# ZhengdiYu/Arbitrary-Hands-3D-Reconstruction

Hardware: AMD Instinct MI355X
Metric: frames/sec (2-hand mesh) at 512x512 batch-64; vertex L2 vs ref (higher is better)
Workload: dtype f32; 1 GPU; configs[2]: synthetic 512x512 RGB batch=64 per GPU, HRNet-W32 backbone, fp32; frames_per_gpu=64, global_batch=64, parallelism=frame-sharded x1, gather=none (one rank), contexts_in_turn=2

## Files before the change

arbitrary-hands-3d-reconstruction_amd/_lib.py:

```python
import ctypes as C
import os

HERE = os.path.dirname(os.path.abspath(__file__))
LIB_PATH = os.environ.get('ACRMI_LIB') or os.path.join(HERE, 'libacrmi.so')

OP_U8NORM, OP_CONV, OP_FUSESUM, OP_BILINEAR2X, OP_POW11, OP_ATTPOOL, OP_PAREBIAS, OP_COORDFILL, OP_POINTHEADS, OP_STEM = range(1, 11)
OP_MAXPOOL, OP_PAIR1X1 = 11, 12
MODE_BOTH, MODE_DENSE, MODE_POINT = 0, 1, 2
CONV_BIAS_MAP = 8
CONV_SPLITK = 16
CONV_DUAL = 32
OPT_POINT_HEADS, OPT_LANES, OPT_CENTER_IDX, OPT_TEMPORAL, OPT_CONF_THRESH, OPT_SMOOTH_COEFF, OPT_MANO_FP16 = 1, 2, 3, 4, 5, 6, 7
OPT_LANE_PLAN = 8
OPT_BATCH_PRIOR = 9
OPT_POINT_HEADS_MULTI = 10
VERSION = 303
DT_F32, DT_F16, DT_BF16 = 0, 1, 2
SLOT = 176
MAX_HAND = 8
ASSOC_STATE = 41
SLOT_FLAG, SLOT_FLATIND, SLOT_SCORE, SLOT_CAM, SLOT_POSES, SLOT_BETAS, SLOT_PARAMS = 0, 1, 2, 3, 6, 54, 64
E_INVAL, E_HIP, E_STATE, E_NOMEM, E_RANGE = -1, -2, -3, -4, -5
OVERLAY_SKELETON, OVERLAY_CENTERMAP = 0, 1
SEGM_NONE = 255


class BufferDesc(C.Structure):
    _fields_ = [('h', C.c_int32), ('w', C.c_int32), ('cs', C.c_int32), ('persistent', C.c_int32), ('dtype', C.c_int32)]


class Op(C.Structure):
    _fields_ = [('kind', C.c_int32),
                ('in_buf', C.c_int32), ('out_buf', C.c_int32), ('res_buf', C.c_int32),
                ('in_coff', C.c_int32), ('out_coff', C.c_int32), ('res_coff', C.c_int32),
                ('cin', C.c_int32), ('cout', C.c_int32),
                ('ksize', C.c_int32), ('stride', C.c_int32), ('relu', C.c_int32), ('groups', C.c_int32),
                ('w_off', C.c_int64), ('b_off', C.c_int64),
                ('bias_per_frame', C.c_int32), ('aux_buf', C.c_int32), ('nterms', C.c_int32),
                ('term_buf', C.c_int32 * 4), ('term_coff', C.c_int32 * 4), ('term_shift', C.c_int32 * 4),
                ('w_off2', C.c_int64), ('b_off2', C.c_int64), ('w_off3', C.c_int64),
                ('flags', C.c_int32), ('mode', C.c_int32)]


class Frame(C.Structure):
    _fields_ = [('bgr_dev', C.c_void_p), ('H', C.c_int32), ('W', C.c_int32)]


class NV12Frame(C.Structure):
    _fields_ = [('y_dev', C.c_void_p), ('uv_dev', C.c_void_p), ('H', C.c_int32), ('W', C.c_int32),
                ('y_pitch', C.c_int32), ('uv_pitch', C.c_int32)]


class NV12Surface(C.Structure):
    _fields_ = NV12Frame._fields_


class Roi(C.Structure):
    _fields_ = [('frame', C.c_int32), ('l', C.c_int32), ('t', C.c_int32), ('r', C.c_int32), ('b', C.c_int32)]


NV12_MATRICES = {'cv601': 0, 'bt601': 1, 'bt601-full': 2, 'bt709': 3, 'bt709-full': 4}


class HeadLayout(C.Structure):
    _fields_ = [('center_buf', C.c_int32 * 2), ('params_buf', C.c_int32 * 2), ('prior_buf', C.c_int32 * 2),
                ('segm_buf', C.c_int32), ('backbone_buf', C.c_int32)]


class ConvProblem(C.Structure):
    _fields_ = [('in_', C.c_void_p), ('w_packed', C.c_void_p), ('bias', C.c_void_p), ('res', C.c_void_p), ('out', C.c_void_p)] + \
               [(k, C.c_int32) for k in ('B', 'H', 'W', 'in_cs', 'in_coff', 'cin', 'bias_frame_stride', 'res_cs', 'res_coff', 'out_cs',
                                         'out_coff', 'cout', 'ksize', 'stride', 'relu', 'groups', 'algo', 'reserved')]


EXPORTS = ['acrmi_version', 'acrmi_last_error', 'acrmi_create', 'acrmi_destroy', 'acrmi_load_weights',
           'acrmi_set_program', 'acrmi_load_mano', 'acrmi_backbone_heads', 'acrmi_buffer_ptr', 'acrmi_decode',
           'acrmi_decode_maps', 'acrmi_mano', 'acrmi_forward', 'acrmi_conv2d', 'acrmi_u8norm', 'acrmi_bilinear2x',
           'acrmi_fuse_sum', 'acrmi_attpool', 'acrmi_attpool_ws_floats', 'acrmi_stem_conv', 'acrmi_stream_create', 'acrmi_stream_destroy', 'acrmi_profile_ops', 'acrmi_tune', 'acrmi_preprocess', 'acrmi_cam_trans',
           'acrmi_set_option', 'acrmi_point_heads', 'acrmi_set_option_f', 'acrmi_smooth', 'acrmi_smooth_reset',
           'acrmi_comm_unique_id', 'acrmi_comm_init', 'acrmi_comm_destroy', 'acrmi_allgather', 'acrmi_parebias',
           'acrmi_buffer_dtype', 'acrmi_conv2d_h16', 'acrmi_conv2d_splitk', 'acrmi_conv2d_splitk_workspace',
           'acrmi_decode_gated', 'acrmi_decode_maps_gated', 'acrmi_share_weights', 'acrmi_mano_rotmat', 'acrmi_heads',
           'acrmi_backbone_channels', 'acrmi_check_range', 'acrmi_prior_gate', 'acrmi_preprocess_frames',
           'acrmi_mesh_topology', 'acrmi_render_workspace', 'acrmi_rasterize', 'acrmi_load_faces', 'acrmi_render',
           'acrmi_overlay_tables', 'acrmi_draw_skeletons', 'acrmi_draw_heatmaps', 'acrmi_overlay',
           'acrmi_streams_create', 'acrmi_streams_destroy', 'acrmi_streams_reset', 'acrmi_smooth_streams',
           'acrmi_forward_streams', 'acrmi_nv12_matrix', 'acrmi_preprocess_nv12', 'acrmi_nv12_to_rgb',
           'acrmi_roi_offsets', 'acrmi_preprocess_rois', 'acrmi_preprocess_rois_nv12', 'acrmi_track_box', 'acrmi_track_boxes',
           'acrmi_preprocess_rois_dev', 'acrmi_preprocess_rois_nv12_dev', 'acrmi_nv12_out_matrix', 'acrmi_rgb_to_nv12',
           'acrmi_nv12_compose', 'acrmi_rasterize_views', 'acrmi_draw_region_heatmaps', 'acrmi_render_regions',
           'acrmi_overlay_regions', 'acrmi_decode_multi', 'acrmi_decode_maps_multi', 'acrmi_forward_multi',
           'acrmi_tracks_create', 'acrmi_tracks_destroy', 'acrmi_tracks_reset', 'acrmi_associate', 'acrmi_forward_tracks',
           'acrmi_assoc_step', 'acrmi_point_heads_multi', 'acrmi_contact_workspace', 'acrmi_mesh_contact', 'acrmi_contact',
           'acrmi_conv2d_group', 'acrmi_program_groups', 'acrmi_surface_contact_workspace', 'acrmi_mesh_surface_contact',
           'acrmi_surface_contact', 'acrmi_score_board_bytes', 'acrmi_score_pair_bytes', 'acrmi_pose_errors',
           'acrmi_score_accumulate', 'acrmi_score_hands', 'acrmi_vertex_colors', 'acrmi_contact_values',
           'acrmi_rasterize_colored', 'acrmi_render_colored', 'acrmi_render_regions_colored', 'acrmi_segm_tables',
           'acrmi_segm_labels', 'acrmi_segm_stats_ws_ints', 'acrmi_segm_stats', 'acrmi_segment', 'acrmi_match_board_bytes',
           'acrmi_match_hands', 'acrmi_match_gather', 'acrmi_match_accumulate', 'acrmi_mano_backward']

_lib = None


class AcrmiError(RuntimeError):
    pass


class AcrmiRangeError(AcrmiError, OverflowError):
    """ACRMI_ERANGE: an 'fp16x3' program met an activation outside the f16 range (acrmi_check_range); the results since the
    last check are invalid (and were written as NaN)."""


def lib():
    global _lib
    if _lib is not None:
        return _lib
    if not os.path.exists(LIB_PATH):
        raise AcrmiError('libacrmi.so not built: run `python __graft_entry__.py build` (needs hipcc). '
                         'The ACR path has no CPU fallback.')
    L = C.CDLL(LIB_PATH)
    vp, i32, f32p, u8p = C.c_void_p, C.c_int, C.c_void_p, C.c_void_p
    L.acrmi_version.restype = C.c_int
    if L.acrmi_version() != VERSION:
        raise AcrmiError('%s is ABI version %d, this package binds version %d: rebuild it (`python __graft_entry__.py build`)'
                         % (LIB_PATH, L.acrmi_version(), VERSION))
    L.acrmi_last_error.restype = C.c_char_p
    L.acrmi_last_error.argtypes = [vp]
    L.acrmi_create.argtypes = [C.POINTER(vp), i32]
    L.acrmi_destroy.argtypes = [vp]
    L.acrmi_destroy.restype = None
    L.acrmi_load_weights.argtypes = [vp, vp, C.c_size_t]
    L.acrmi_set_program.argtypes = [vp, C.POINTER(BufferDesc), i32, C.POINTER(Op), i32, C.POINTER(HeadLayout), i32]
    L.acrmi_load_mano.argtypes = [vp, i32, vp, vp, vp, vp, vp, vp]
    L.acrmi_backbone_heads.argtypes = [vp, u8p, i32, vp]
    L.acrmi_buffer_ptr.argtypes = [vp, i32, C.POINTER(i32), C.POINTER(i32), C.POINTER(i32)]
    L.acrmi_buffer_ptr.restype = vp
    L.acrmi_decode.argtypes = [vp, i32, f32p, vp]
    L.acrmi_decode_maps.argtypes = [f32p, f32p, i32, f32p, f32p, i32, f32p, f32p, i32, i32, C.c_float, f32p, vp]
    L.acrmi_decode_gated.argtypes = [vp, i32, vp, f32p, vp]
    L.acrmi_share_weights.argtypes = [vp, vp]
    L.acrmi_decode_maps_gated.argtypes = [f32p, f32p, i32, f32p, f32p, i32, f32p, f32p, i32, i32, C.c_float, vp, f32p, vp]
    L.acrmi_mano.argtypes = [vp, f32p, i32, f32p, i32, vp, i32, i32, f32p, f32p, f32p, f32p, i32, f32p, f32p, f32p,
                             f32p, vp]
    L.acrmi_mano_rotmat.argtypes = [vp, f32p, f32p, i32, vp, i32, i32, f32p, f32p, f32p, vp]
    L.acrmi_mano_backward.argtypes = [vp, f32p, i32, f32p, i32, vp, i32, i32, f32p, f32p, f32p, f32p, f32p, vp]
    L.acrmi_heads.argtypes = [vp, f32p, i32, vp]
    L.acrmi_backbone_channels.argtypes = [vp]
    L.acrmi_check_range.argtypes = [vp, vp]
    L.acrmi_prior_gate.argtypes = [vp, f32p, i32, vp, vp]
    L.acrmi_preprocess_frames.argtypes = [C.POINTER(Frame), i32, vp, vp, vp]
    L.acrmi_nv12_matrix.argtypes = [i32, vp]
    L.acrmi_preprocess_nv12.argtypes = [C.POINTER(NV12Frame), i32, vp, vp, vp, vp]
    L.acrmi_nv12_to_rgb.argtypes = [C.POINTER(NV12Frame), i32, vp, i32, C.POINTER(vp), vp]
    L.acrmi_nv12_out_matrix.argtypes = [i32, vp]
    L.acrmi_rgb_to_nv12.argtypes = [C.POINTER(vp), C.POINTER(NV12Surface), i32, vp, i32, vp]
    L.acrmi_nv12_compose.argtypes = [C.POINTER(NV12Frame), C.POINTER(vp), C.POINTER(NV12Surface), i32, vp, vp, i32, vp]
    L.acrmi_roi_offsets.argtypes = [i32, i32, C.POINTER(Roi), vp, vp]
    L.acrmi_preprocess_rois.argtypes = [C.POINTER(Frame), i32, C.POINTER(Roi), i32, vp, vp, vp]
    L.acrmi_preprocess_rois_nv12.argtypes = [C.POINTER(NV12Frame), i32, C.POINTER(Roi), i32, vp, vp, vp, vp]
    L.acrmi_track_box.argtypes = [f32p, i32, i32, i32, C.c_double, i32, vp]
    L.acrmi_track_boxes.argtypes = [f32p, f32p, vp, i32, C.c_double, i32, vp, vp]
    L.acrmi_preprocess_rois_dev.argtypes = [C.POINTER(Frame), i32, vp, vp, i32, vp, vp, vp, vp]
    L.acrmi_preprocess_rois_nv12_dev.argtypes = [C.POINTER(NV12Frame), i32, vp, vp, i32, vp, vp, vp, vp, vp]
    L.acrmi_forward.argtypes = [vp, u8p, i32, f32p, f32p, f32p, f32p, f32p, f32p, f32p, vp]
    L.acrmi_conv2d.argtypes = [f32p, i32, i32, i32, i32, i32, i32, f32p, f32p, i32, f32p, i32, i32, f32p, i32, i32,
                               i32, i32, i32, i32, i32, i32, vp]
    L.acrmi_conv2d_h16.argtypes = [vp, i32, i32, i32, i32, i32, i32, vp, f32p, i32, vp, i32, i32, vp, i32, i32,
                                   i32, i32, i32, i32, i32, i32, i32, vp]
    L.acrmi_conv2d_splitk.argtypes = [f32p, i32, i32, i32, i32, i32, i32, i32, f32p, f32p, f32p, i32, i32, f32p, i32, i32,
                                      i32, i32, vp, C.c_size_t, vp]
    L.acrmi_conv2d_splitk_workspace.argtypes = [i32, i32, i32, i32, i32]
    L.acrmi_conv2d_splitk_workspace.restype = C.c_size_t
    L.acrmi_buffer_dtype.argtypes = [vp, i32]
    L.acrmi_u8norm.argtypes = [u8p, i32, f32p, vp]
    L.acrmi_bilinear2x.argtypes = [f32p, i32, i32, i32, i32, i32, f32p, i32, vp]
    L.acrmi_fuse_sum.argtypes = [i32, C.POINTER(vp), C.POINTER(i32), C.POINTER(i32), i32, i32, i32, i32, f32p, i32,
                                 i32, vp]
    L.acrmi_attpool.argtypes = [f32p, i32, f32p, i32, i32, i32, f32p, f32p, vp]
    L.acrmi_attpool_ws_floats.argtypes = [i32, i32]
    L.acrmi_stream_create.argtypes = [i32, C.POINTER(C.c_void_p)]
    L.acrmi_stream_destroy.argtypes = [vp]
    L.acrmi_stem_conv.argtypes = [vp, i32, i32, i32, f32p, f32p, f32p, i32, i32, i32, vp]
    L.acrmi_attpool_ws_floats.restype = C.c_size_t
    L.acrmi_profile_ops.argtypes = [vp, u8p, i32, vp, i32, vp]
    L.acrmi_tune.argtypes = [i32, i32]
    L.acrmi_conv2d_group.argtypes = [C.POINTER(ConvProblem), i32, vp]
    L.acrmi_program_groups.argtypes = [vp, i32]
    L.acrmi_preprocess.argtypes = [u8p, i32, i32, i32, u8p, vp, vp]
    L.acrmi_cam_trans.argtypes = [f32p, f32p, i32, C.c_float, C.c_float, f32p, vp]
    L.acrmi_set_option.argtypes = [vp, i32, i32]
    L.acrmi_point_heads.argtypes = [vp, i32, vp]
    L.acrmi_point_heads_multi.argtypes = [vp, i32, i32, vp]
    L.acrmi_set_option_f.argtypes = [vp, i32, C.c_float]
    L.acrmi_smooth.argtypes = [vp, f32p, i32, vp]
    L.acrmi_smooth_reset.argtypes = [vp, vp]
    L.acrmi_streams_create.argtypes = [C.POINTER(vp), i32, i32]
    L.acrmi_streams_destroy.argtypes = [vp]
    L.acrmi_streams_destroy.restype = None
    L.acrmi_streams_reset.argtypes = [vp, vp, i32, vp]
    L.acrmi_smooth_streams.argtypes = [vp, vp, f32p, i32, vp, vp]
    L.acrmi_forward_streams.argtypes = [vp, vp, vp, u8p, i32, f32p, f32p, f32p, f32p, f32p, f32p, f32p, vp]
    L.acrmi_comm_unique_id.argtypes = [vp]
    L.acrmi_comm_init.argtypes = [vp, i32, i32, vp]
    L.acrmi_comm_destroy.argtypes = [vp]
    L.acrmi_allgather.argtypes = [vp, vp, f32p, f32p, C.c_size_t, vp]
    L.acrmi_parebias.argtypes = [f32p, i32, i32, f32p, f32p, f32p, f32p, f32p, i32, f32p, i32, vp]
    L.acrmi_mesh_topology.argtypes = [vp, i32, i32, vp, i32]
    L.acrmi_render_workspace.argtypes = [i32, i32]
    L.acrmi_render_workspace.restype = C.c_size_t
    L.acrmi_rasterize.argtypes = [f32p, f32p, i32, i32, i32, vp, vp, vp, vp, f32p, f32p, C.c_float, C.c_float, u8p, u8p, i32,
                                  i32, i32, vp, vp, vp]
    L.acrmi_load_faces.argtypes = [vp, i32, vp, i32]
    L.acrmi_render.argtypes = [vp, f32p, f32p, f32p, i32, f32p, vp, C.c_float, C.c_float, u8p, u8p, i32, i32, vp, vp]
    L.acrmi_overlay_tables.argtypes = [i32, u8p, u8p]
    L.acrmi_draw_skeletons.argtypes = [f32p, vp, i32, u8p, i32, i32, i32, u8p, u8p, i32, i32, i32, vp]
    L.acrmi_draw_heatmaps.argtypes = [f32p, f32p, C.c_longlong, i32, i32, i32, f32p, C.c_float, u8p, i32, u8p, u8p, u8p, i32,
                                      i32, vp]
    L.acrmi_overlay.argtypes = [vp, i32, f32p, f32p, i32, f32p, i32, u8p, u8p, u8p, i32, i32, vp]
    L.acrmi_rasterize_views.argtypes = list(L.acrmi_rasterize.argtypes)
    L.acrmi_draw_region_heatmaps.argtypes = [f32p, f32p, C.c_longlong, i32, i32, i32, f32p, vp, C.c_float, u8p, i32, u8p, u8p,
                                             u8p, i32, i32, i32, vp]
    L.acrmi_render_regions.argtypes = [vp, f32p, f32p, f32p, i32, f32p, vp, vp, C.c_float, C.c_float, u8p, u8p, i32, i32, i32,
                                       vp, vp]
    L.acrmi_overlay_regions.argtypes = [vp, i32, f32p, f32p, i32, f32p, vp, i32, u8p, u8p, u8p, i32, i32, i32, vp]
    L.acrmi_decode_multi.argtypes = [vp, i32, i32, f32p, vp]
    L.acrmi_decode_maps_multi.argtypes = [f32p, f32p, i32, f32p, f32p, i32, f32p, f32p, i32, i32, i32, C.c_float, f32p, vp]
    L.acrmi_forward_multi.argtypes = [vp, u8p, i32, i32, f32p, f32p, f32p, f32p, f32p, f32p, f32p, vp]
    L.acrmi_tracks_create.argtypes = [C.POINTER(vp), i32, i32, i32, i32, i32]
    L.acrmi_tracks_destroy.argtypes = [vp]
    L.acrmi_tracks_destroy.restype = None
    L.acrmi_tracks_reset.argtypes = [vp, vp, i32, vp]
    L.acrmi_associate.argtypes = [vp, vp, f32p, i32, i32, vp, i32, vp, vp, vp]
    L.acrmi_forward_tracks.argtypes = [vp, vp, vp, i32, u8p, i32, i32, f32p, f32p, f32p, f32p, f32p, f32p, f32p, vp, vp]
    L.acrmi_assoc_step.argtypes = [i32, i32, i32, vp, i32, vp, vp, vp, vp]
    L.acrmi_contact_workspace.argtypes = [i32, i32]
    L.acrmi_contact_workspace.restype = C.c_size_t
    L.acrmi_mesh_contact.argtypes = [f32p, f32p, i32, i32, i32, vp, vp, vp, vp, vp, i32, C.c_float, C.c_float, vp, f32p, f32p,
                                     f32p, vp, vp, vp]
    L.acrmi_contact.argtypes = [vp, f32p, f32p, f32p, i32, i32, vp, C.c_float, C.c_float, vp, f32p, f32p, f32p, vp, vp]
    L.acrmi_surface_contact_workspace.argtypes = [i32, i32, i32]
    L.acrmi_surface_contact_workspace.restype = C.c_size_t
    L.acrmi_mesh_surface_contact.argtypes = [f32p, f32p, i32, i32, i32, vp, vp, vp, vp, i32, C.c_float, C.c_float, vp, f32p, f32p,
                                             vp, f32p, vp, vp, vp]
    L.acrmi_surface_contact.argtypes = [vp, f32p, f32p, f32p, i32, i32, C.c_float, C.c_float, vp, f32p, f32p, vp, f32p, vp, vp]
    L.acrmi_score_board_bytes.argtypes = [i32, i32, i32]
    L.acrmi_score_board_bytes.restype = C.c_size_t
    L.acrmi_score_pair_bytes.argtypes = [i32]
    L.acrmi_score_pair_bytes.restype = C.c_size_t
    L.acrmi_pose_errors.argtypes = [f32p, f32p, u8p, i32, i32, i32, f32p, f32p, f32p, vp, i32, f32p, f32p, f32p, f32p, vp, f32p, f32p, vp]
    L.acrmi_score_accumulate.argtypes = [f32p, f32p, i32, i32, vp, i32, f32p, f32p, i32, C.c_double, vp, vp, vp]
    L.acrmi_score_hands.argtypes = [vp, f32p, f32p, f32p, f32p, f32p, f32p, u8p, vp, i32, i32, i32, i32, C.c_double, vp,
                                    f32p, f32p, f32p, vp, f32p, f32p, f32p, vp, f32p, vp]
    L.acrmi_vertex_colors.argtypes = [f32p, vp, f32p, i32, i32, C.c_float, C.c_float, i32, f32p, u8p, i32, f32p, vp]
    L.acrmi_contact_values.argtypes = [f32p, f32p, vp, i32, i32, i32, C.c_float, f32p, vp, vp]
    L.acrmi_rasterize_colored.argtypes = [f32p, f32p, i32, i32, i32, vp, vp, vp, vp, f32p, f32p, f32p, i32, C.c_float, C.c_float,
                                          u8p, u8p, i32, i32, i32, vp, vp, vp]
    L.acrmi_render_colored.argtypes = [vp, f32p, f32p, f32p, i32, f32p, vp, f32p, C.c_float, C.c_float, u8p, u8p, i32, i32, vp, vp]
    L.acrmi_render_regions_colored.argtypes = [vp, f32p, f32p, f32p, i32, f32p, vp, vp, f32p, C.c_float, C.c_float, u8p, u8p, i32,
                                               i32, i32, vp, vp]
    L.acrmi_segm_tables.argtypes = [i32, i32, u8p]
    L.acrmi_segm_labels.argtypes = [f32p, C.c_longlong, i32, i32, i32, i32, i32, f32p, f32p, C.c_float, u8p, i32, u8p, u8p, u8p,
                                    i32, i32, vp]
    L.acrmi_segm_stats_ws_ints.argtypes = [i32, i32, i32]
    L.acrmi_segm_stats_ws_ints.restype = C.c_size_t
    L.acrmi_segm_stats.argtypes = [u8p, vp, i32, i32, i32, i32, i32, vp, vp, vp, vp, vp]
    L.acrmi_segment.argtypes = [vp, i32, f32p, C.c_float, u8p, i32, u8p, u8p, u8p, i32, i32, vp]
    L.acrmi_match_board_bytes.argtypes = []
    L.acrmi_match_board_bytes.restype = C.c_size_t
    L.acrmi_match_hands.argtypes = [f32p, f32p, u8p, u8p, f32p, i32, f32p, vp, i32, i32, i32, i32, i32, C.c_float, i32, vp, vp, f32p,
                                    vp, vp, vp]
    L.acrmi_match_gather.argtypes = [f32p, vp, i32, i32, i32, i32, f32p, vp]
    L.acrmi_match_accumulate.argtypes = [vp, f32p, i32, i32, vp, vp]
    for name in EXPORTS:
        fn = getattr(L, name)
        if name not in ('acrmi_last_error', 'acrmi_destroy', 'acrmi_buffer_ptr', 'acrmi_attpool_ws_floats',
                        'acrmi_render_workspace', 'acrmi_streams_destroy', 'acrmi_tracks_destroy', 'acrmi_contact_workspace',
                        'acrmi_surface_contact_workspace', 'acrmi_score_board_bytes', 'acrmi_score_pair_bytes',
                        'acrmi_segm_stats_ws_ints', 'acrmi_match_board_bytes'):
            fn.restype = C.c_int
    _lib = L
    return L


def check(rc, ctx=None):
    if rc >= 0:
        return rc
    msg = lib().acrmi_last_error(ctx)
    msg = msg.decode() if msg else 'acrmi error %d' % rc
    if rc == E_INVAL:
        raise ValueError(msg)
    if rc == E_RANGE:
        raise AcrmiRangeError(msg)
    raise AcrmiError(msg)
```

arbitrary-hands-3d-reconstruction_amd/csrc/acrmi.hip:

```cpp
#include "acrmi_ctx.h"
#include "score_plan.h"
#include "surface_contact_plan.h"
#include "vertex_color_plan.h"

#include <initializer_list>
#include <type_traits>

std::string g_err;

int fail(acrmi_ctx* c, int code, const char* fmt, ...) {
  char buf[512];
  va_list ap;
  va_start(ap, fmt);
  vsnprintf(buf, sizeof buf, fmt, ap);
  va_end(ap);
  if (c) c->err = buf; else g_err = buf;
  return code;
}

void release_weights(acrmi_ctx* c) {
  if (c->weights_ref && c->weights_ref->fetch_sub(1) == 1) {
    (void)hipFree(c->weights);
    delete c->weights_ref;
  }
// ... 395 lines not shown
                             shared, stream);
  if (!r) *out = t;
  return r;
}

int acrmi_streams_create(acrmi_streams** out, int device, int capacity) { return streams_create(out, device, capacity, true, nullptr); }

void acrmi_streams_destroy(acrmi_streams* t) { table_destroy(t); }

int acrmi_streams_reset(acrmi_streams* t, const int32_t* ids, int n, void* stream) {
  return table_reset("acrmi_streams_reset", t, ids, n,
                     [](StateTable* t, const SmoothIds& k, int m, hipStream_t s) { return launch_smooth_reset(k, m, t->init, s); },
                     (hipStream_t)stream);
}

static void smooth_coefficients(SmoothArgs& a, float smooth_coeff) {
  a.mincutoff = smooth_coeff; a.mincutoff_betas = 0.6f; a.beta = 0.7f; a.freq = 30.f;
  const double te = 1.0 / 30.0, tau = 1.0 / (2 * M_PI * 1.0), alpha_d = 1.0 / (1.0 + tau / te);
  a.alpha_d = (float)alpha_d; a.one_minus_alpha_d = (float)(1.0 - alpha_d);
  a.two_pi = (float)(2 * M_PI); a.te = (float)te;
}

static int smooth_on(acrmi_ctx* c, acrmi_streams* t, float* slots, int B, const int32_t* ids, hipStream_t stream) {
  SmoothArgs a{};
  a.state = t->state;
  a.init = t->init;
  smooth_coefficients(a, c->smooth_coeff);
  TableOrder ord(t, stream);
  hipError_t e = ord.err;
  for (int f0 = 0; e == hipSuccess && f0 < B; f0 += SMOOTH_FRAMES_PER_LAUNCH) {
    const int m = B - f0 < SMOOTH_FRAMES_PER_LAUNCH ? B - f0 : SMOOTH_FRAMES_PER_LAUNCH;
    const int n_streams = smooth_plan(ids ? ids + f0 : nullptr, m, &a.b, t->last.data());
    if (!n_streams) continue;
    a.slots = slots + (size_t)f0 * 2 * ACRMI_SLOT;
    e = launch_smooth(a, n_streams, stream);
  }
  e = ord.done(e);
  return e == hipSuccess ? ACRMI_OK : fail(c, ACRMI_EHIP, "smoothing: %s", hipGetErrorString(e));
}

static int check_streams(acrmi_ctx* c, const acrmi_streams* t, const int32_t* ids, int B, const char* who) {
  if (!t || !ids || B <= 0) return fail(c, ACRMI_EINVAL, "%s: bad arguments", who);
  return check_table(c, t, ids, B, who);
}

int acrmi_smooth_streams(acrmi_ctx* c, acrmi_streams* t, float* slots, int B, const int32_t* ids, void* stream) {
  if (!c || !slots) return fail(c, ACRMI_EINVAL, "acrmi_smooth_streams: bad arguments");
  const int r = check_streams(c, t, ids, B, "acrmi_smooth_streams");
  if (r) return r;
  ON_DEVICE(c);
  return smooth_on(c, t, slots, B, ids, (hipStream_t)stream);
}

int acrmi_smooth_reset(acrmi_ctx* c, void* stream) {
  if (!c) return fail(c, ACRMI_EINVAL, "acrmi_smooth_reset: ctx is NULL");
  if (!c->own_streams)
    return from_global(c, streams_create(&c->own_streams, c->device, 1, false, (hipStream_t)stream));
  return from_global(c, acrmi_streams_reset(c->own_streams, nullptr, 0, stream));
}

int acrmi_smooth(acrmi_ctx* c, float* slots, int B, void* stream) {
  if (!c || !slots || B <= 0) return fail(c, ACRMI_EINVAL, "acrmi_smooth: bad arguments");
  ON_DEVICE(c);
  if (!c->own_streams) {
    int r = acrmi_smooth_reset(c, stream);
    if (r) return r;
  }
  return smooth_on(c, c->own_streams, slots, B, nullptr, (hipStream_t)stream);
}

int acrmi_tracks_create(acrmi_tracks** out, int device, int capacity, int max_hand, int gate, int max_miss) {
  if (!out) return fail(nullptr, ACRMI_EINVAL, "acrmi_tracks_create: out is NULL");
  if (!assoc_params_ok(max_hand, gate, max_miss))
    return fail(nullptr, ACRMI_EINVAL, "acrmi_tracks_create: max_hand %d outside 1..%d, gate %d outside 0..%d or max_miss %d < -1",
                max_hand, ASSOC_MAX_HAND, gate, ASSOC_GATE_ANY, max_miss);
  if (capacity < 1 || (long long)capacity * max_hand > ASSOC_MAX_TRACKS)
    return fail(nullptr, ACRMI_EINVAL, "acrmi_tracks_create: capacity %d x max_hand %d outside 1..%d hands per side", capacity,
                max_hand, ASSOC_MAX_TRACKS);
  acrmi_tracks* t = new acrmi_tracks();
  t->max_hand = max_hand; t->gate = gate; t->max_miss = max_miss;
  const size_t hands = (size_t)capacity * max_hand * 2;
  const size_t state_bytes = hands * 3 * 64 * sizeof(float), init_bytes = hands * sizeof(int);
  const int r = table_create("acrmi_tracks_create", t, device, capacity, state_bytes,
                             state_bytes + init_bytes + (size_t)capacity * 2 * sizeof(AssocSide), true, nullptr);
  if (r) return r;
  t->meta = reinterpret_cast<AssocSide*>(reinterpret_cast<char*>(t->init) + init_bytes);
  *out = t;
  return ACRMI_OK;
}

void acrmi_tracks_destroy(acrmi_tracks* t) { table_destroy(t); }

int acrmi_tracks_reset(acrmi_tracks* t, const int32_t* ids, int n, void* stream) {
  return table_reset("acrmi_tracks_reset", t, ids, n,
                     [](StateTable* st, const SmoothIds& k, int m, hipStream_t s) {
                       acrmi_tracks* t = static_cast<acrmi_tracks*>(st);
                       return launch_assoc_reset(k, m, t->max_hand, t->meta, t->init, s);
                     },
                     (hipStream_t)stream);
}

static int check_tracks(acrmi_ctx* c, const acrmi_tracks* t, const int32_t* ids, int B, int max_hand, const char* who) {
  if (!t || !ids || B <= 0) return fail(c, ACRMI_EINVAL, "%s: bad arguments", who);
  if (max_hand < 1 || max_hand > ACRMI_MAX_HAND) return fail(c, ACRMI_EINVAL, "%s: max_hand %d outside 1..%d", who, max_hand, ACRMI_MAX_HAND);
  if (max_hand != t->max_hand) return fail(c, ACRMI_EINVAL, "%s: max_hand %d, the table holds %d slots per side", who, max_hand, t->max_hand);
  return check_table(c, t, ids, B, who);
}

static int associate_on(acrmi_ctx* c, acrmi_tracks* t, float* slots, int B, const int32_t* ids, int smooth, int32_t* track_ids,
                        int32_t* perm, hipStream_t stream) {
  AssocArgs a{};
  a.s.state = t->state;
  a.s.init = t->init;
  smooth_coefficients(a.s, c ? c->smooth_coeff : 4.0f );
  a.meta = t->meta;
  a.K = t->max_hand; a.gate = t->gate; a.max_miss = t->max_miss; a.smooth = smooth ? 1 : 0;
  const size_t frame_rows = (size_t)2 * t->max_hand;
  TableOrder ord(t, stream);
  hipError_t e = ord.err;
  for (int f0 = 0; e == hipSuccess && f0 < B; f0 += SMOOTH_FRAMES_PER_LAUNCH) {
    const int m = B - f0 < SMOOTH_FRAMES_PER_LAUNCH ? B - f0 : SMOOTH_FRAMES_PER_LAUNCH;
    const int n_streams = smooth_plan(ids + f0, m, &a.s.b, t->last.data());
    bool any_loose = false;
    memset(a.loose, 0, sizeof a.loose);
    for (int i = 0; i < m; ++i)
      if (ids[f0 + i] < 0) { a.loose[i >> 5] |= 1u << (i & 31); any_loose = true; }
    a.m = m;
    a.s.slots = slots + (size_t)f0 * frame_rows * ACRMI_SLOT;
    a.track_ids = track_ids + (size_t)f0 * frame_rows;
    a.perm = perm ? perm + (size_t)f0 * frame_rows : nullptr;
    e = launch_associate(a, n_streams, any_loose, stream);
  }
  e = ord.done(e);
  return e == hipSuccess ? ACRMI_OK : fail(c, ACRMI_EHIP, "association: %s", hipGetErrorString(e));
}

int acrmi_associate(acrmi_ctx* c, acrmi_tracks* t, float* slots, int B, int max_hand, const int32_t* ids, int smooth,
                    int32_t* track_ids, int32_t* perm, void* stream) {
  if (!slots || !track_ids) return fail(c, ACRMI_EINVAL, "acrmi_associate: bad arguments");
  const int r = check_tracks(c, t, ids, B, max_hand, "acrmi_associate");
  if (r) return r;
  DeviceGuard guard_(t->device);
  if (guard_.err != hipSuccess) return fail(c, ACRMI_EHIP, "hipSetDevice(%d): %s", t->device, hipGetErrorString(guard_.err));
  return associate_on(c, t, slots, B, ids, smooth, track_ids, perm, (hipStream_t)stream);
}

int acrmi_program_groups(acrmi_ctx* c, int B) {
  if (!c) return fail(c, ACRMI_EINVAL, "acrmi_program_groups: bad arguments");
  if (!c->have_program) return fail(c, ACRMI_ESTATE, "no program");
  if (B <= 0 || B > c->max_batch) return fail(c, ACRMI_EINVAL, "batch %d outside 1..%d", B, c->max_batch);
  return c->sched[c->point_heads ? 1 : 0][B > AUTO_SMALL_BATCH ? 1 : 0].n_groups;
}

int acrmi_profile_ops(acrmi_ctx* c, const uint8_t* img, int B, float* ms_out, int n_ms, void* stream) {
  if (!c || !img || !ms_out) return fail(c, ACRMI_EINVAL, "acrmi_profile_ops: bad arguments");
  if (!c->have_program) return fail(c, ACRMI_ESTATE, "no program");
  const int n = (int)c->ops.size();
  if (n_ms < n) return fail(c, ACRMI_EINVAL, "ms_out too small (%d < %d)", n_ms, n);
  ON_DEVICE(c);
  hipStream_t s = (hipStream_t)stream;
  const bool point = c->point_heads;
  int r = run_program(c, img, B, stream, point);
  if (r) return r;
  std::vector<hipEvent_t> ev(n + 1, nullptr);
  auto cleanup = [&]() {
    for (auto& e : ev)
      if (e) (void)hipEventDestroy(e);
  };
  hipError_t he = hipSuccess;
  for (auto& e : ev)
    if ((he = hipEventCreate(&e)) != hipSuccess) break;
  if (he == hipSuccess) he = hipEventRecord(ev[0], s);
  for (int i = 0; i < n && he == hipSuccess && r == ACRMI_OK; ++i) {
    if (op_active(c->ops[i], point)) r = run_op(c, c->ops[i], img, B, s);
    if (r == ACRMI_OK) he = hipEventRecord(ev[i + 1], s);
  }
  if (he == hipSuccess && r == ACRMI_OK) he = hipStreamSynchronize(s);
  for (int i = 0; i < n && he == hipSuccess && r == ACRMI_OK; ++i) he = hipEventElapsedTime(&ms_out[i], ev[i], ev[i + 1]);
  cleanup();
  if (r) return r;
  if (he != hipSuccess) return fail(c, ACRMI_EHIP, "acrmi_profile_ops: %s", hipGetErrorString(he));
  if (B <= AUTO_SMALL_BATCH) {
    c->op_ms[point ? 1 : 0].assign(ms_out, ms_out + n);
    build_schedule(c, point, false);
  }
  return n;
}

void* acrmi_buffer_ptr(acrmi_ctx* c, int buf, int* h, int* w, int* cs) {
  if (!c || !c->have_program || buf < 0 || buf >= (int)c->bufs.size()) return nullptr;
  if (h) *h = c->bufs[buf].h;
  if (w) *w = c->bufs[buf].w;
  if (cs) *cs = c->bufs[buf].cs;
  return c->buf_ptr[buf];
}

int acrmi_buffer_dtype(acrmi_ctx* c, int buf) {
  if (!c || !c->have_program || buf < 0 || buf >= (int)c->bufs.size()) return -1;
  return c->bufs[buf].dtype;
}

static int decode_ctx(acrmi_ctx* c, const char* who, int B, const int32_t* prior_gate, bool top_k, int max_hand, float* slots,
                      void* stream) {
  if (!c || !slots) return fail(c, ACRMI_EINVAL, "%s: bad arguments", who);
  if (top_k && (max_hand < 1 || max_hand > ACRMI_MAX_HAND))
    return fail(c, ACRMI_EINVAL, "%s: max_hand %d outside 1..%d", who, max_hand, ACRMI_MAX_HAND);
  if (!c->have_program) return fail(c, ACRMI_ESTATE, "%s: no program", who);
  if (B <= 0 || B > c->max_batch) return fail(c, ACRMI_EINVAL, "batch %d outside 1..%d", B, c->max_batch);
  ON_DEVICE(c);
  const acrmi_head_layout& h = c->heads;
  return from_global(c, decode_maps_impl(c->buf_ptr[h.center_buf[0]], c->buf_ptr[h.center_buf[1]], c->bufs[h.center_buf[0]].cs,
                                         c->buf_ptr[h.params_buf[0]], c->buf_ptr[h.params_buf[1]], c->bufs[h.params_buf[0]].cs,
                                         c->buf_ptr[h.prior_buf[0]], c->buf_ptr[h.prior_buf[1]], c->bufs[h.prior_buf[0]].cs, B,
                                         c->conf_thresh, prior_gate, c->range_flag, slots, stream, top_k ? max_hand : 0));
}

int acrmi_decode(acrmi_ctx* c, int B, float* slots, void* stream) { return acrmi_decode_gated(c, B, nullptr, slots, stream); }

int acrmi_decode_gated(acrmi_ctx* c, int B, const int32_t* prior_gate, float* slots, void* stream) {
  return decode_ctx(c, "acrmi_decode", B, prior_gate, false, 0, slots, stream);
}

int acrmi_decode_multi(acrmi_ctx* c, int B, int max_hand, float* slots, void* stream) {
  return decode_ctx(c, "acrmi_decode_multi", B, nullptr, true, max_hand, slots, stream);
}

int acrmi_prior_gate(acrmi_ctx* c, const float* slots, int B, int32_t* gate, void* stream) {
  if (!slots || !gate || B <= 0) return fail(c, ACRMI_EINVAL, "acrmi_prior_gate: bad arguments");
  if (c) {
    ON_DEVICE(c);
    return from_global(c, acrmi_prior_gate(nullptr, slots, B, gate, stream));
  }
  HIPCHK(c, launch_prior_gate(slots, B, gate, (hipStream_t)stream));
  return ACRMI_OK;
}

int acrmi_check_range(acrmi_ctx* c, void* stream) {
  if (!c) return fail(c, ACRMI_EINVAL, "acrmi_check_range: ctx is NULL");
  if (!c->range_flag) return ACRMI_OK;
  ON_DEVICE(c);
  unsigned v = 0;
  HIPCHK(c, hipStreamSynchronize((hipStream_t)stream));
  HIPCHK(c, hipMemcpy(&v, c->range_flag, sizeof(v), hipMemcpyDeviceToHost));
  if (!v) return ACRMI_OK;
  HIPCHK(c, hipMemsetAsync(c->range_flag, 0, sizeof(v), (hipStream_t)stream));
  HIPCHK(c, hipStreamSynchronize((hipStream_t)stream));
  return fail(c, ACRMI_ERANGE, "an activation of the 'fp16x3' program left the f16 range (|x| > 65504): its split halves are "
                               "inf / -inf and the results since the last check are invalid (slots and meshes were written as "
                               "NaN); use precision 'bf16x3' or 'fp32' for this checkpoint");
}

static int mano_rows(acrmi_ctx* c, const char* who, ManoArgs& m, const float* betas, int beta_stride, const int32_t* side, int H,
                     int center_idx, float* verts, float* joints, float* center, void* stream) {
  if (!c) return fail(c, ACRMI_EINVAL, "%s: ctx is NULL", who);
  if (H == 0) return ACRMI_OK;
  if (H < 0 || !m.poses || !betas || !verts || !joints || center_idx >= 21) return fail(c, ACRMI_EINVAL, "%s: bad arguments", who);
  if (!c->have_mano[0] && !c->have_mano[1]) return fail(c, ACRMI_ESTATE, "%s: MANO tables not loaded", who);
  ON_DEVICE(c);
  m.t[0] = c->have_mano[0] ? c->mano[0] : c->mano[1];
  m.t[1] = c->have_mano[1] ? c->mano[1] : c->mano[0];
  m.betas = betas; m.beta_stride = beta_stride;
  m.side = side; m.H = H; m.center_idx = center_idx;
  m.verts = verts; m.joints = joints; m.center = center;
  m.off_div = 1;
  m.lbs_f16 = c->mano_f16;
  HIPCHK(c, launch_mano(m, (hipStream_t)stream));
  return ACRMI_OK;
}

int acrmi_mano(acrmi_ctx* c, const float* poses, int pose_stride, const float* betas, int beta_stride,
               const int32_t* side, int H, int center_idx, float* verts, float* joints, float* center,
               const float* cam, int cam_stride, const float* offsets, float* verts_camed, float* pj2d,
               float* pj2d_org, void* stream) {
  ManoArgs m{};
  m.poses = poses; m.pose_stride = pose_stride;
  m.cam = cam; m.cam_stride = cam_stride; m.offsets = offsets;
  m.verts_camed = verts_camed; m.pj2d = pj2d; m.pj2d_org = pj2d_org;
  return mano_rows(c, "acrmi_mano", m, betas, beta_stride, side, H, center_idx, verts, joints, center, stream);
}

int acrmi_mano_rotmat(acrmi_ctx* c, const float* rotmats, const float* betas, int beta_stride, const int32_t* side, int H,
                      int center_idx, float* verts, float* joints, float* center, void* stream) {
  ManoArgs m{};
  m.poses = rotmats; m.pose_stride = 144; m.pose_rotmat = 1;
  return mano_rows(c, "acrmi_mano_rotmat", m, betas, beta_stride, side, H, center_idx, verts, joints, center, stream);
}

int acrmi_mano_backward(acrmi_ctx* c, const float* poses, int pose_stride, const float* betas, int beta_stride,
                        const int32_t* side, int H, int center_idx, const float* g_verts, const float* g_joints,
                        const float* g_center, float* g_poses, float* g_betas, void* stream) {
  if (!c) return fail(c, ACRMI_EINVAL, "acrmi_mano_backward: ctx is NULL");
  if (H < 0 || center_idx < -1 || center_idx > 20 || pose_stride < 48 || beta_stride < 10)
    return fail(c, ACRMI_EINVAL, "acrmi_mano_backward: bad arguments (H >= 0, center_idx -1..20, pose_stride >= 48, beta_stride >= 10)");
  if (H == 0) return ACRMI_OK;
  if (!poses || !betas || !g_poses || !g_betas) return fail(c, ACRMI_EINVAL, "acrmi_mano_backward: NULL poses, betas or outputs");
  if (!c->have_mano[0] && !c->have_mano[1]) return fail(c, ACRMI_ESTATE, "acrmi_mano_backward: MANO tables not loaded");
  ON_DEVICE(c);
  if (!g_verts && !g_joints && !g_center) {
    HIPCHK(c, hipMemsetAsync(g_poses, 0, (size_t)H * 48 * sizeof(float), (hipStream_t)stream));
    HIPCHK(c, hipMemsetAsync(g_betas, 0, (size_t)H * 10 * sizeof(float), (hipStream_t)stream));
    return ACRMI_OK;
  }
  ManoGradArgs m{};
  m.t[0] = c->have_mano[0] ? c->mano[0] : c->mano[1];
  m.t[1] = c->have_mano[1] ? c->mano[1] : c->mano[0];
  m.poses = poses; m.pose_stride = pose_stride;
// ... 318 lines not shown
  if (what == ACRMI_OVERLAY_SKELETON ? (!slots || !kps) : (!out2 || out2 == out || out2 == img_in))
    return fail(c, ACRMI_EINVAL, "%s: bad arguments", who);
  if (!c->have_program || c->last_batch <= 0) return fail(c, ACRMI_ESTATE, "%s: no program has run", who);
  return ACRMI_OK;
}

static hipError_t skeleton_launch(const float* kps, const float* slots, const int32_t* hand_frame, int normalized, int n_hands,
                                  int n_frames, int H, int W, int bgr, const uint8_t* img_in, uint8_t* out, hipStream_t stream) {
  SkeletonArgs a{};
  a.kps = kps; a.hand_frame = hand_frame; a.normalized = normalized;
  if (slots) { a.slots = slots; a.slot_stride = ACRMI_SLOT; a.flag_at = ACRMI_SLOT_FLAG; }
  a.n_hands = n_hands; a.n_frames = n_frames; a.H = H; a.W = W; a.line_width = 3; a.circle_rad = 3;
  a.img_in = img_in; a.img_out = out;
  skeleton_default_colors(bgr != 0, a.colors);
  return launch_skeleton(a, stream);
}

static int heatmap_fill(acrmi_ctx* c, const char* who, HeatmapBase& a, int n, const float* offsets, int bgr, const uint8_t* img_in,
                        uint8_t* out, uint8_t* out2, int H, int W) {
  if (n != c->last_batch)
    return fail(c, ACRMI_ESTATE, "%s: the resident centre maps are those of a batch of %d, not %d", who, c->last_batch, n);
  const acrmi_head_layout& hl = c->heads;
  const acrmi_buffer_desc& d = c->bufs[hl.center_buf[0]];
  a.maps[0] = c->buf_ptr[hl.center_buf[0]]; a.maps[1] = c->buf_ptr[hl.center_buf[1]];
  a.pix_stride = d.cs; a.frame_stride = (long long)d.h * d.w * d.cs; a.dtype = d.dtype;
  a.n = n; a.h = d.h; a.w = d.w; a.H = H; a.W = W; a.offsets = offsets; a.weight = 0.7f;
  a.img_in = img_in; a.out[0] = out; a.out[1] = out2;
  heatmap_default_lut(bgr != 0, a.lut);
  return ACRMI_OK;
}

int acrmi_overlay(acrmi_ctx* c, int what, const float* slots, const float* pj2d, int B, const float* offsets, int bgr,
                  const uint8_t* img_in, uint8_t* out, uint8_t* out2, int H, int W, void* stream) {
  if (int r = check_overlay(c, "acrmi_overlay", what, slots, pj2d, B, img_in, out, out2, B, H, W)) return r;
  ON_DEVICE(c);
  hipError_t e;
  if (what == ACRMI_OVERLAY_SKELETON) {
    e = skeleton_launch(pj2d, slots, nullptr, offsets ? 0 : 1, 2 * B, B, H, W, bgr, img_in, out, (hipStream_t)stream);
  } else {
    HeatmapArgs a{};
    if (int r = heatmap_fill(c, "acrmi_overlay", a, B, offsets, bgr, img_in, out, out2, H, W)) return r;
    e = launch_heatmap(a, (hipStream_t)stream);
  }
  return e == hipSuccess ? ACRMI_OK : fail(c, ACRMI_EHIP, "overlay: %s", hipGetErrorString(e));
}

int acrmi_segment(acrmi_ctx* c, int B, const float* offsets, float weight, const uint8_t* colors_host, int bgr,
                  const uint8_t* img_in, uint8_t* out, uint8_t* labels, int H, int W, void* stream) {
  const char* who = "acrmi_segment";
  if (!c) return fail(c, ACRMI_EINVAL, "%s: ctx is NULL", who);
  if (B <= 0) return fail(c, ACRMI_EINVAL, "%s: B = %d", who, B);
  if (!c->have_program || c->last_batch <= 0) return fail(c, ACRMI_ESTATE, "%s: no program has run", who);
  if (B != c->last_batch)
    return fail(c, ACRMI_ESTATE, "%s: the resident segmentation is that of a batch of %d, not %d", who, c->last_batch, B);
  const int id = c->heads.segm_buf;
  const acrmi_buffer_desc& d = c->bufs[id];
  if (d.dtype != ACRMI_DT_F32) return fail(c, ACRMI_ESTATE, "%s: the segmentation buffer is not fp32", who);
  ON_DEVICE(c);
  return segm_labels_call(c, who, (const float*)c->buf_ptr[id], (long long)d.h * d.w * d.cs, d.cs, B, d.h, d.w, 33, nullptr, offsets,
                          weight, colors_host, bgr, img_in, out, labels, H, W, stream);
}

static int render_regions_call(acrmi_ctx* c, const char* who, bool colored, const float* vcol, const float* verts,
                               const float* cam_trans, const float* slots, int n, const float* offsets, const int32_t* region_frame,
                               const float* colors_host, float focal, float visible_weight, const uint8_t* img_in, uint8_t* img_out,
                               int n_frames, int H, int W, int32_t* ids_out, void* stream) {
  if ((colored && (!vcol || n <= 0 || !vertex_color_sizes_ok(2ll * n, 778))) || !c || !verts || !cam_trans || !slots || !offsets || !region_frame || !img_in || !img_out || n <= 0 || n_frames <= 0 ||
      n_frames > OVERLAY_MAX_FRAMES || H <= 0 || W <= 0 || H > OVERLAY_MAX_DIM || W > OVERLAY_MAX_DIM || !(focal > 0.f) ||
      !(visible_weight >= 0.f && visible_weight <= 1.f) || n > 0x3fffffff || (c->n_faces[0] > 0 && 2ll * n * c->n_faces[0] > 0x7fffffffll))
    return fail(c, ACRMI_EINVAL, "%s: bad arguments", who);
  if (!c->faces_topo[0] || !c->faces_topo[1]) return fail(c, ACRMI_ESTATE, "%s: MANO faces not loaded (acrmi_load_faces)", who);
  ON_DEVICE(c);
  RenderScratch sc;
  if (int r = render_scratch(c, n, &sc)) return r;
  hipError_t e = launch_render_region_prep(slots, offsets, region_frame, n, n_frames, H, W, ACRMI_SLOT, ACRMI_SLOT_FLAG,
                                           colors_host ? colors_host : kHandColors, sc.mesh_frame, sc.mesh_topo, sc.rgb, sc.view,
                                           (hipStream_t)stream);
  if (e != hipSuccess) return fail(c, ACRMI_EHIP, "render region prep: %s", hipGetErrorString(e));
  e = render_launch(c, sc, verts, cam_trans, nullptr, sc.view, focal, visible_weight, img_in, img_out, ids_out, 2 * n, n_frames, H, W,
                    (hipStream_t)stream, vcol);
  return e == hipSuccess ? ACRMI_OK : fail(c, ACRMI_EHIP, "render regions: %s", hipGetErrorString(e));
}

int acrmi_render_regions(acrmi_ctx* c, const float* verts, const float* cam_trans, const float* slots, int n, const float* offsets,
                         const int32_t* region_frame, const float* colors_host, float focal, float visible_weight,
                         const uint8_t* img_in, uint8_t* img_out, int n_frames, int H, int W, int32_t* ids_out, void* stream) {
  return render_regions_call(c, "acrmi_render_regions", false, nullptr, verts, cam_trans, slots, n, offsets, region_frame, colors_host,
                             focal, visible_weight, img_in, img_out, n_frames, H, W, ids_out, stream);
}

int acrmi_render_regions_colored(acrmi_ctx* c, const float* verts, const float* cam_trans, const float* slots, int n,
                                 const float* offsets, const int32_t* region_frame, const float* colors_host, const float* vcol,
                                 float focal, float visible_weight, const uint8_t* img_in, uint8_t* img_out, int n_frames, int H,
                                 int W, int32_t* ids_out, void* stream) {
  return render_regions_call(c, "acrmi_render_regions_colored", true, vcol, verts, cam_trans, slots, n, offsets, region_frame,
                             colors_host, focal, visible_weight, img_in, img_out, n_frames, H, W, ids_out, stream);
}

int acrmi_overlay_regions(acrmi_ctx* c, int what, const float* slots, const float* pj2d_org, int n, const float* offsets,
                          const int32_t* region_frame, int bgr, const uint8_t* img_in, uint8_t* out, uint8_t* out2, int n_frames,
                          int H, int W, void* stream) {
  if (!offsets || !region_frame || n > 0x3fffffff) return fail(c, ACRMI_EINVAL, "acrmi_overlay_regions: bad arguments");
  if (int r = check_overlay(c, "acrmi_overlay_regions", what, slots, pj2d_org, n, img_in, out, out2, n_frames, H, W)) return r;
  ON_DEVICE(c);
  hipError_t e;
  if (what == ACRMI_OVERLAY_SKELETON) {
    if (n > c->region_hand_cap) {
      if (c->region_hand_frame) {
        HIPCHK(c, hipDeviceSynchronize());
        (void)hipFree(c->region_hand_frame);
        c->region_hand_frame = nullptr;
        c->region_hand_cap = 0;
      }
      HIPCHK(c, hipMalloc(&c->region_hand_frame, sizeof(int32_t) * 2 * (size_t)n));
      c->region_hand_cap = n;
    }
    e = launch_render_region_prep(slots, offsets, region_frame, n, n_frames, H, W, ACRMI_SLOT, ACRMI_SLOT_FLAG, nullptr,
                                  c->region_hand_frame, nullptr, nullptr, nullptr, (hipStream_t)stream);
    if (e != hipSuccess) return fail(c, ACRMI_EHIP, "overlay region prep: %s", hipGetErrorString(e));
    e = skeleton_launch(pj2d_org, nullptr, c->region_hand_frame, 0, 2 * n, n_frames, H, W, bgr, img_in, out, (hipStream_t)stream);
  } else {
    RegionHeatmapArgs a{};
    if (int r = heatmap_fill(c, "acrmi_overlay_regions", a, n, offsets, bgr, img_in, out, out2, H, W)) return r;
    a.n_frames = n_frames; a.region_frame = region_frame;
    e = launch_region_heatmap(a, (hipStream_t)stream);
  }
  return e == hipSuccess ? ACRMI_OK : fail(c, ACRMI_EHIP, "overlay regions: %s", hipGetErrorString(e));
}

int acrmi_stream_create(int device, void** stream) {
  if (!stream) return fail(nullptr, ACRMI_EINVAL, "acrmi_stream_create: null argument");
  int prev = 0;
  if (hipGetDevice(&prev) != hipSuccess || hipSetDevice(device) != hipSuccess)
    return fail(nullptr, ACRMI_EHIP, "acrmi_stream_create: cannot select device %d", device);
  hipStream_t st = nullptr;
  const hipError_t e = hipStreamCreateWithFlags(&st, hipStreamNonBlocking);
  (void)hipSetDevice(prev);
  if (e != hipSuccess) return fail(nullptr, ACRMI_EHIP, "hipStreamCreate: %s", hipGetErrorString(e));
  *stream = st;
  return ACRMI_OK;
}

int acrmi_stream_destroy(void* stream) {
  if (!stream) return ACRMI_OK;
  const hipError_t e = hipStreamDestroy((hipStream_t)stream);
  return e == hipSuccess ? ACRMI_OK : fail(nullptr, ACRMI_EHIP, "hipStreamDestroy: %s", hipGetErrorString(e));
}

int acrmi_tune(int key, int value) {
  if (key == 0) { conv_force_cfg(value); return ACRMI_OK; }
  if (key == 3) { conv_set_phase_delay(value); return ACRMI_OK; }
  if (key == 4) { conv_set_xcd_swizzle(value); return ACRMI_OK; }
  if (key == 5) { program_set_grouping(value != 0); return ACRMI_OK; }
  static long long* dbg = nullptr;
  if (key == 1) {
    if (value && !dbg) { if (hipMalloc(&dbg, 128 * sizeof(long long)) != hipSuccess) return ACRMI_EHIP; }
    if (dbg) (void)hipMemset(dbg, 0, 128 * sizeof(long long));
    conv_set_debug(value ? dbg : nullptr);
    return ACRMI_OK;
  }
  if (key == 2) {
    if (!dbg) return ACRMI_OK;
    long long h[128];
    if (hipDeviceSynchronize() != hipSuccess) return ACRMI_EHIP;
    if (hipMemcpy(h, dbg, sizeof h, hipMemcpyDeviceToHost) != hipSuccess) return ACRMI_EHIP;
    const int n = (int)h[63];
    printf("conv stamps (%d):", n);
    for (int i = 1; i < n && i < 60; ++i) printf(" %lld", h[i] - h[i - 1]);
    printf("\n");
    const int nl = (int)h[127];
    if (nl > 0) {
      printf("loader stamps (%d):", nl);
      for (int i = 1; i < nl && i < 60; ++i) printf(" %lld", h[64 + i] - h[64 + i - 1]);
      printf("\n");
    }
    return ACRMI_OK;
  }
  return fail(nullptr, ACRMI_EINVAL, "acrmi_tune: unknown key %d", key);
}

}
```

arbitrary-hands-3d-reconstruction_amd/csrc/acrmi_ctx.h:

```cpp
#pragma once
#include "../../include/acrmi.h"
#include "kernels.h"

#include <dlfcn.h>

#include <atomic>
#include <cmath>
#include <cstdarg>
#include <cstdio>
#include <algorithm>
#include <cstdlib>
#include <cstring>
#include <mutex>
#include <optional>
#include <string>
#include <vector>

using namespace acrmi;

constexpr int MAX_LANES = 8;
constexpr int AUTO_LANES_SMALL = 4, AUTO_LANES_LARGE = 2, AUTO_SMALL_BATCH = 32;
struct Schedule {
  std::vector<int> order;
  std::vector<std::vector<int>> deps;
  std::vector<char> leaf;
  int n_lanes = 0;
  std::vector<int> lane;
  std::vector<std::vector<int>> wait;
  std::vector<char> signal;
  std::vector<int> leader;
  int n_groups = 0;
};
struct StateTable {
  int device = 0;
  int capacity = 0;
  float* state = nullptr;
  int* init = nullptr;
  size_t reset_bytes = 0;
  hipEvent_t order = nullptr;
  std::mutex mu;
  std::vector<int32_t> last;
  virtual ~StateTable() = default;
};

struct acrmi_streams : StateTable {};

struct acrmi_tracks : StateTable {
  int max_hand = 0, gate = 0, max_miss = 0;
  AssocSide* meta = nullptr;
};

struct acrmi_ctx {
  int device = 0;
  std::string err;
  float* weights = nullptr;
  size_t n_weights = 0;
  std::atomic<int>* weights_ref = nullptr;
  std::vector<acrmi_buffer_desc> bufs;
  std::vector<float*> buf_ptr;
  std::vector<acrmi_op> ops;
  acrmi_head_layout heads{};
  bool have_program = false;
  int max_batch = 0;
  bool grouping = false;
  float* att_ws = nullptr;
  size_t att_ws_floats = 0;
  int* picks = nullptr;
  int* gate_buf = nullptr;
  bool batch_prior = false;
  unsigned* range_flag = nullptr;
  bool point_heads = false;
  bool point_heads_multi = false;
  Schedule sched[2][2];
  int want_lanes = 0;
  bool lane_plan = false;
  std::vector<float> op_ms[2];
  hipStream_t lanes[MAX_LANES] = {};
  hipEvent_t fork_ev = nullptr, join_ev[MAX_LANES] = {};
  std::vector<hipEvent_t> op_ev;
  float* split_ws[MAX_LANES] = {};
  unsigned* split_cnt[MAX_LANES] = {};
  size_t split_ws_floats = 0, split_counters = 0;
  ManoTables mano[2]{};
  bool have_mano[2] = {false, false};
  float* mano_allocs[2][11] = {};
  bool mano_f16 = false;
  float conf_thresh = 0.35f;
  int center_idx = 9;
  bool temporal = false;
  float smooth_coeff = 4.0f;
  acrmi_streams* own_streams = nullptr;
  int32_t* faces_topo[2] = {nullptr, nullptr};
  int n_faces[2] = {0, 0};
  char* render_ws = nullptr;
  int render_ws_frames = 0;
  int32_t* region_hand_frame = nullptr;
  int region_hand_cap = 0;
  std::vector<float> v_template_host[2];
  std::vector<int32_t> faces_host[2];
  int contact_sign[2] = {1, 1};
  struct ContactScratch {
    char* ws = nullptr;
    long long hands = 0;
    int faces = 0;
  };
  ContactScratch contact_ws, surface_ws;
  int last_batch = 0;
  void* comm = nullptr;
  int comm_ranks = 0;
};

struct DeviceGuard {
  int prev = -1;
  bool switched = false;
  hipError_t err = hipSuccess;
  explicit DeviceGuard(int dev) {
    err = hipGetDevice(&prev);
    if (err == hipSuccess && prev != dev) {
      err = hipSetDevice(dev);
      switched = err == hipSuccess;
    }
  }
  ~DeviceGuard() {
    if (switched) (void)hipSetDevice(prev);
  }
};

extern std::string g_err;
int fail(acrmi_ctx* c, int code, const char* fmt, ...);
#define ON_DEVICE(c)                                                                                   \
  DeviceGuard guard_((c)->device);                                                                     \
  if (guard_.err != hipSuccess) return fail(c, ACRMI_EHIP, "hipSetDevice(%d): %s", (c)->device, hipGetErrorString(guard_.err))
#define HIPCHK(c, expr)                                                                      \
  do {                                                                                       \
    hipError_t e_ = (expr);                                                                  \
    if (e_ != hipSuccess) return fail(c, ACRMI_EHIP, "%s: %s", #expr, hipGetErrorString(e_)); \
  } while (0)


void free_program(acrmi_ctx* c);
void release_weights(acrmi_ctx* c);
void comm_destroy(acrmi_ctx* c);
PointArgs point_args(const acrmi_ctx* c, const acrmi_op& op, int B);
int run_op(acrmi_ctx* c, const acrmi_op& op, const uint8_t* img, int B, hipStream_t s, int lane = 0, int point_hands = 1);
bool op_active(const acrmi_op& op, bool point);
void build_schedule(acrmi_ctx* c, bool point, bool large);
void program_set_grouping(bool on);
int run_program(acrmi_ctx* c, const uint8_t* img, int B, void* stream, bool point, int first_op = 0, int point_hands = 1);
int decode_maps_impl(const float* l_center, const float* r_center, int center_cs, const float* l_params, const float* r_params,
                     int params_cs, const float* l_prior, const float* r_prior, int prior_cs, int B, float conf_thresh,
                     const int32_t* prior_gate, const unsigned* poison, float* slots, void* stream,
                     int max_hand = 0 );
int segm_labels_call(acrmi_ctx* c, const char* who, const float* logits, long long frame_stride, int pix_stride, int n, int h, int w,
                     int C, const float* view, const float* offsets, float weight, const uint8_t* colors_host, int bgr,
                     const uint8_t* img_in, uint8_t* out, uint8_t* labels, int H, int W, void* stream);
```

arbitrary-hands-3d-reconstruction_amd/csrc/acrmi_program.hip:

```cpp
#include "acrmi_ctx.h"
#include "conv_frame.h"
#include "group_plan.h"

void free_program(acrmi_ctx* c) {
  for (hipEvent_t e : c->op_ev)
    if (e) (void)hipEventDestroy(e);
  c->op_ev.clear();
  for (float* p : c->buf_ptr)
    if (p) (void)hipFree(p);
  c->buf_ptr.clear();
  c->bufs.clear();
  c->ops.clear();
  for (int l = 0; l < MAX_LANES; ++l) {
    if (c->split_ws[l]) (void)hipFree(c->split_ws[l]);
    if (c->split_cnt[l]) (void)hipFree(c->split_cnt[l]);
    c->split_ws[l] = nullptr; c->split_cnt[l] = nullptr;
  }
  c->split_ws_floats = c->split_counters = 0;
  if (c->att_ws) (void)hipFree(c->att_ws);
  c->att_ws = nullptr;
  if (c->picks) (void)hipFree(c->picks);
  c->picks = nullptr;
  if (c->gate_buf) (void)hipFree(c->gate_buf);
  c->gate_buf = nullptr;
  if (c->range_flag) (void)hipFree(c->range_flag);
  c->range_flag = nullptr;
  c->have_program = false;
  c->last_batch = 0;
}

static ConvArgs conv_geometry(const acrmi_op& op, const acrmi_buffer_desc* bufs, int B) {
  const auto& di = bufs[op.in_buf];
  const auto& dout = bufs[op.out_buf];
  ConvArgs a{};
  a.B = B; a.H = di.h; a.W = di.w;
  a.in_cs = di.cs; a.in_coff = op.in_coff; a.Cin = op.cin;
  a.out_cs = dout.cs; a.out_coff = op.out_coff; a.Cout = op.cout;
  a.res_cs = op.res_buf >= 0 ? bufs[op.res_buf].cs : 0; a.res_coff = op.res_coff;
  a.splitk = (op.flags & ACRMI_CONV_SPLITK) != 0;
  if (op.flags & ACRMI_CONV_BIAS_MAP) {
    a.res_cs = (op.groups * op.cout + 3) / 4 * 4; a.res_coff = 0; a.res_bcast = 1;
  }
  a.ks = op.ksize; a.stride = op.stride; a.relu = op.relu; a.groups = op.groups;
  a.bias_fstride = op.bias_per_frame ? bufs[op.aux_buf].cs : 0;
  a.nxt = op.nterms;
  for (int t = 0; t < op.nterms && t < 3; ++t) {
    a.xt_cs[t] = bufs[op.term_buf[t]].cs; a.xt_coff[t] = op.term_coff[t]; a.xt_shift[t] = op.term_shift[t];
  }
  if (op.flags & ACRMI_CONV_DUAL) a.out2_cs = bufs[op.aux_buf].cs;
  a.algo = op.flags & 7;
  a.dtype = di.dtype;
  a.out_f32 = di.dtype != ACRMI_DT_F32 && dout.dtype == ACRMI_DT_F32;
  conv_derive(a);
  return a;
}

PointArgs point_args(const acrmi_ctx* c, const acrmi_op& op, int B) {
  auto ptr = [&](int id) -> float* { return c->buf_ptr[id]; };
  auto desc = [&](int id) -> const acrmi_buffer_desc& { return c->bufs[id]; };
  const acrmi_head_layout& h = c->heads;
  const int side = op.flags & 1;
  PointArgs p{};
  p.x34 = ptr(op.in_buf); p.x_cs = desc(op.in_buf).cs;
  p.center[0] = ptr(h.center_buf[0]); p.center[1] = ptr(h.center_buf[1]); p.center_cs = desc(h.center_buf[0]).cs;
  p.w = c->weights + op.w_off;
  p.mix_w = c->weights + op.w_off2;
  p.bias = ptr(op.aux_buf); p.bias_stride = desc(op.aux_buf).cs;
  p.p109 = ptr(op.res_buf); p.p109_cs = desc(op.res_buf).cs;
  p.prior = ptr(h.prior_buf[side]); p.prior_cs = desc(h.prior_buf[side]).cs;
  p.final_ = ptr(op.out_buf); p.final_cs = desc(op.out_buf).cs;
  p.picks = c->picks; p.side = side; p.B = B; p.thresh = c->conf_thresh;
  p.prior_when_both = c->batch_prior ? 1 : 0;
  return p;
}

static ConvArgs conv_args(const acrmi_ctx* c, const acrmi_op& op, int B, int lane) {
  auto ptr = [&](int id) -> float* { return id >= 0 ? c->buf_ptr[id] : nullptr; };
  ConvArgs a = conv_geometry(op, c->bufs.data(), B);
  a.in = ptr(op.in_buf);
  a.w = c->weights + op.w_off;
  a.bias = op.bias_per_frame ? ptr(op.aux_buf) : c->weights + op.b_off;
  a.res = a.res_bcast ? c->weights + op.w_off2 : ptr(op.res_buf);
  a.out = ptr(op.out_buf);
  if (a.splitk) {
    a.split_ws = c->split_ws[lane]; a.split_cnt = c->split_cnt[lane];
  }
  for (int t = 0; t < op.nterms && t < 3; ++t) a.xt[t] = ptr(op.term_buf[t]);
  if (op.flags & ACRMI_CONV_DUAL) a.out2 = ptr(op.aux_buf);
  a.range_flag = a.algo == 6 ? c->range_flag : nullptr;
  return a;
}

static bool g_grouping = [] {
  const char* e = getenv("ACRMI_GROUP");
  return !(e && atoi(e) == 0);
}();
void program_set_grouping(bool on) { g_grouping = on; }

int run_op(acrmi_ctx* c, const acrmi_op& op, const uint8_t* img, int B, hipStream_t s, int lane, int point_hands) {
  auto ptr = [&](int id) -> float* { return id >= 0 ? c->buf_ptr[id] : nullptr; };
  auto desc = [&](int id) -> const acrmi_buffer_desc& { return c->bufs[id]; };
  auto eptr = [&](int id, int coff) -> float* {
    if (id < 0) return nullptr;
    return reinterpret_cast<float*>(reinterpret_cast<char*>(c->buf_ptr[id]) + (size_t)coff * (c->bufs[id].dtype ? 2 : 4));
  };
  switch (op.kind) {
    case ACRMI_OP_U8NORM: {
      const auto& d = desc(op.out_buf);
      HIPCHK(c, launch_u8norm(img, (long)B * d.h * d.w, ptr(op.out_buf), s));
      return ACRMI_OK;
    }
    case ACRMI_OP_STEM: {
      const auto& d = desc(op.out_buf);
      if (op.ksize == 7) {
        if (d.dtype)
          HIPCHK(c, launch_stem7_h16(img, B, 2 * d.h, 2 * d.w, c->weights + op.w_off, c->weights + op.b_off, ptr(op.out_buf),
                                     d.cs, op.out_coff, op.relu, d.dtype, s));
        else
          HIPCHK(c, launch_stem7(img, B, 2 * d.h, 2 * d.w, c->weights + op.w_off, c->weights + op.b_off, ptr(op.out_buf), d.cs,
                                 op.out_coff, op.relu, s));
        return ACRMI_OK;
      }
      if (d.dtype)
        HIPCHK(c, launch_stem_h16(img, B, 2 * d.h, 2 * d.w, c->weights + op.w_off, c->weights + op.b_off, ptr(op.out_buf),
                                  d.cs, op.out_coff, op.relu, d.dtype, s));
      else
        HIPCHK(c, launch_stem(img, B, 2 * d.h, 2 * d.w, c->weights + op.w_off, c->weights + op.b_off, ptr(op.out_buf), d.cs,
                              op.out_coff, op.relu, s));
      return ACRMI_OK;
    }
    case ACRMI_OP_CONV: {
      HIPCHK(c, launch_conv(conv_args(c, op, B, lane), s));
      return ACRMI_OK;
    }
    case ACRMI_OP_FUSESUM: {
      const auto& dout = desc(op.out_buf);
      FuseArgs f{};
      f.nterms = op.nterms; f.B = B; f.H = dout.h; f.W = dout.w; f.C = op.cout; f.out_cs = dout.cs; f.relu = op.relu;
      f.out = eptr(op.out_buf, op.out_coff);
      for (int t = 0; t < op.nterms; ++t) {
        f.term[t] = eptr(op.term_buf[t], op.term_coff[t]);
        f.cs[t] = desc(op.term_buf[t]).cs;
        f.shift[t] = op.term_shift[t];
      }
      if (dout.dtype) HIPCHK(c, launch_fuse_sum_h16(f, dout.dtype, s));
      else HIPCHK(c, launch_fuse_sum(f, s));
      return ACRMI_OK;
    }
    case ACRMI_OP_BILINEAR2X: {
      const auto& di = desc(op.in_buf);
      if (di.dtype)
        HIPCHK(c, launch_bilinear2x_h16(ptr(op.in_buf), B, di.h, di.w, di.cs, op.in_coff, op.cin, ptr(op.out_buf),
                                        desc(op.out_buf).cs, op.out_coff, di.dtype, s));
      else
        HIPCHK(c, launch_bilinear2x(ptr(op.in_buf), B, di.h, di.w, di.cs, op.in_coff, op.cin, ptr(op.out_buf),
                                    desc(op.out_buf).cs, op.out_coff, s));
      return ACRMI_OK;
    }
    case ACRMI_OP_PAIR1X1: {
      const auto& di = desc(op.in_buf);
      HIPCHK(c, launch_pair1x1(ptr(op.in_buf), di.cs, op.in_coff, ptr(op.res_buf), desc(op.res_buf).cs, op.res_coff, ptr(op.out_buf),
                               desc(op.out_buf).cs, op.out_coff, ptr(op.aux_buf), desc(op.aux_buf).cs, 0, c->weights + op.w_off,
                               (long)B * di.h * di.w, s));
      return ACRMI_OK;
    }
    case ACRMI_OP_MAXPOOL: {
      const auto& di = desc(op.in_buf);
      if (di.dtype)
        HIPCHK(c, launch_maxpool3s2_h16(ptr(op.in_buf), B, di.h, di.w, di.cs, op.in_coff, op.cin, ptr(op.out_buf),
                                        desc(op.out_buf).cs, op.out_coff, di.dtype, s));
      else
        HIPCHK(c, launch_maxpool3s2(ptr(op.in_buf), B, di.h, di.w, di.cs, op.in_coff, op.cin, ptr(op.out_buf),
                                    desc(op.out_buf).cs, op.out_coff, s));
      return ACRMI_OK;
    }
    case ACRMI_OP_POW11: {
      const auto& d = desc(op.out_buf);
      if (d.dtype) HIPCHK(c, launch_pow11_h16(ptr(op.out_buf), (long)B * d.h * d.w, d.cs, op.out_coff, d.dtype, s));
      else HIPCHK(c, launch_pow11(ptr(op.out_buf), (long)B * d.h * d.w, d.cs, op.out_coff, s));
      return ACRMI_OK;
    }
    case ACRMI_OP_ATTPOOL: {
      const auto& ds = desc(op.in_buf);
      const auto& df = desc(op.res_buf);
      HIPCHK(c, launch_attpool(ptr(op.in_buf), ds.cs, eptr(op.res_buf, op.res_coff), df.cs, op.cin, B, df.h, df.w,
                               c->att_ws, ptr(op.out_buf), s, df.dtype));
      return ACRMI_OK;
    }
    case ACRMI_OP_PAREBIAS: {
      PareArgs p{};
      p.pooled = ptr(op.in_buf);
      p.lc_w = c->weights + op.w_off;
      p.lin_w = c->weights + op.w_off2;
      p.lin_b = c->weights + op.b_off2;
      p.mix_wp = c->weights + op.w_off3;
      p.mix_b = c->weights + op.b_off;
      p.out = ptr(op.out_buf);
      p.B = B; p.C = op.cin; p.part0 = op.flags; p.out_stride = desc(op.out_buf).cs;
      HIPCHK(c, launch_parebias(p, s));
      return ACRMI_OK;
    }
    case ACRMI_OP_COORDFILL: {
      const auto& d = desc(op.out_buf);
      if (d.dtype) HIPCHK(c, launch_coordfill_h16(ptr(op.out_buf), c->max_batch, d.h, d.w, d.cs, op.out_coff, d.dtype, s));
      else HIPCHK(c, launch_coordfill(ptr(op.out_buf), c->max_batch, d.h, d.w, d.cs, op.out_coff, s));
      return ACRMI_OK;
    }
    case ACRMI_OP_POINTHEADS: {
      const PointArgs p = point_args(c, op, B);
      if (point_hands > 1) HIPCHK(c, launch_point_heads_multi(p, point_hands, s));
      else HIPCHK(c, launch_point_heads(p, s));
      return ACRMI_OK;
    }
    default:
      return fail(c, ACRMI_EINVAL, "unknown op kind %d", op.kind);
  }
}

bool op_active(const acrmi_op& op, bool point) {
  return op.kind != ACRMI_OP_COORDFILL && op.mode != (point ? ACRMI_MODE_DENSE : ACRMI_MODE_POINT);
}

static void op_rw(const acrmi_ctx* c, const acrmi_op& op, std::vector<int>& R, std::vector<int>& W) {
  R.clear(); W.clear();
  const int n_bufs = (int)c->bufs.size();
  auto r = [&](int id) { if (id >= 0) R.push_back(id); };
  auto w = [&](int id) { if (id >= 0) W.push_back(id); };
  switch (op.kind) {
    case ACRMI_OP_U8NORM: case ACRMI_OP_STEM: w(op.out_buf); break;
    case ACRMI_OP_CONV:
      r(op.in_buf); r(op.res_buf); if (op.bias_per_frame) r(op.aux_buf);
      for (int t = 0; t < op.nterms; ++t) r(op.term_buf[t]);
      w(op.out_buf);
      if (op.flags & ACRMI_CONV_DUAL) w(op.aux_buf);
      break;
    case ACRMI_OP_FUSESUM: for (int t = 0; t < op.nterms; ++t) r(op.term_buf[t]); w(op.out_buf); break;
    case ACRMI_OP_BILINEAR2X: case ACRMI_OP_MAXPOOL: r(op.in_buf); w(op.out_buf); break;
    case ACRMI_OP_PAIR1X1: r(op.in_buf); r(op.res_buf); w(op.out_buf); w(op.aux_buf); break;
    case ACRMI_OP_POW11: r(op.out_buf); w(op.out_buf); break;
    case ACRMI_OP_ATTPOOL: r(op.in_buf); r(op.res_buf); w(op.out_buf); w(n_bufs); break;
    case ACRMI_OP_PAREBIAS: r(op.in_buf); w(op.out_buf); break;
    case ACRMI_OP_POINTHEADS:
      r(op.in_buf); r(op.aux_buf); r(c->heads.center_buf[0]); r(c->heads.center_buf[1]);
      w(op.res_buf); w(op.out_buf); w(c->heads.prior_buf[op.flags & 1]); w(n_bufs + 1);
      break;
    default: break;
  }
}

void build_schedule(acrmi_ctx* c, bool point, bool large) {
  Schedule& S = c->sched[point ? 1 : 0][large ? 1 : 0];
  const int n = (int)c->ops.size(), nb = (int)c->bufs.size() + 2;
  S = Schedule();
  S.deps.assign(n, std::vector<int>());
  S.leaf.assign(n, 1);
  std::vector<std::vector<int>> reads(n), writes(n);
  for (int j = 0; j < n; ++j) {
    if (!op_active(c->ops[j], point)) continue;
    S.order.push_back(j);
    op_rw(c, c->ops[j], reads[j], writes[j]);
  }
  S.deps = hazard_deps(S.order, reads, writes, n, nb);
  for (int j : S.order)
    for (int d : S.deps[j]) S.leaf[d] = 0;
  const int want = c->want_lanes > 0 ? c->want_lanes : (large ? AUTO_LANES_LARGE : AUTO_LANES_SMALL);
  const int max_lanes = std::max(1, std::min(want, MAX_LANES));
  S.lane.assign(n, 0);
  S.wait.assign(n, std::vector<int>());
  S.signal.assign(n, 0);
  std::vector<int> lane_tail(max_lanes, -1);
  const std::vector<float>& ms = c->op_ms[point ? 1 : 0];
  const bool planned = c->lane_plan && !large && max_lanes > 1 && (int)ms.size() == n;
  constexpr float SYNC_MS = 0.002f, EVENT_MS = 0.002f;
  static const float WAIT_MS = experiment_env("ACRMI_PLAN_WAIT_US") ? 1e-3f * (float)atof(experiment_env("ACRMI_PLAN_WAIT_US")) : 0.016f;
  std::vector<float> fin(planned ? n : 0, 0.f), lane_free(max_lanes, 0.f);
  static const bool rank_order = !(experiment_env("ACRMI_PLAN_RANK") && atoi(experiment_env("ACRMI_PLAN_RANK")) == 0);
  if (planned && rank_order) {
    std::vector<float> ru(n, 0.f);
    std::vector<std::vector<int>> succ(n);
    for (int j : S.order)
      for (int d : S.deps[j]) succ[d].push_back(j);
    for (int k = (int)S.order.size() - 1; k >= 0; --k) {
      const int j = S.order[k];
      float m = 0.f;
      for (int s2 : succ[j]) m = std::max(m, ru[s2]);
      ru[j] = m + std::max(ms[j], 1e-4f);
    }
    std::stable_sort(S.order.begin(), S.order.end(), [&](int x, int y) { return ru[x] > ru[y]; });
  }
  S.leader.assign(n, 0);
  for (int j = 0; j < n; ++j) S.leader[j] = j;
  S.n_groups = 0;
  if (c->grouping && c->max_batch >= 16) {
    std::vector<ConvArgs> ca(n);
    std::vector<char> is_conv(n, 0);
    for (int j : S.order)
      if (c->ops[j].kind == ACRMI_OP_CONV) { ca[j] = conv_args(c, c->ops[j], c->max_batch, 0); is_conv[j] = 1; }
    S.leader = plan_groups(S.order, S.deps, n, [&](int x, int y) { return is_conv[x] && is_conv[y] && conv_can_group(ca[x], ca[y]); },
                           CONV_GROUP_MAX);
    for (int j : S.order) S.n_groups += S.leader[j] != j;
  }
  std::vector<int> pos(n, -1);
  for (int k = 0; k < (int)S.order.size(); ++k) pos[S.order[k]] = k;
  for (int j : S.order) {
    int lane = -1;
    if (S.leader[j] != j) {
      lane = S.lane[S.leader[j]];
      if (planned) fin[j] = fin[S.leader[j]] = lane_free[lane] = lane_free[lane] + std::max(ms[j] - EVENT_MS, 0.002f);
    } else if (planned) {
      float best = 0.f;
      bool best_prod = false;
      for (int l = 0; l < max_lanes; ++l) {
        float start = lane_free[l];
        unsigned others = 0;
        bool prod = false;
        for (int d : S.deps[j]) {
          if (S.lane[d] == l) { prod = true; continue; }
          others |= 1u << S.lane[d];
          start = std::max(start, fin[d] + WAIT_MS);
        }
        start += SYNC_MS * (float)__builtin_popcount(others);
        if (lane < 0 || start < best - 1e-6f || (start < best + 1e-6f && prod && !best_prod)) { lane = l; best = start; best_prod = prod; }
      }
      fin[j] = best + std::max(ms[j] - EVENT_MS, 0.002f);
      lane_free[lane] = fin[j] + 0.5f * SYNC_MS;
      S.n_lanes = std::max(S.n_lanes, lane + 1);
    } else {
      for (int d : S.deps[j])
        if (lane_tail[S.lane[d]] == d) { lane = S.lane[d]; break; }
      if (lane < 0) {
        if (S.n_lanes < max_lanes) lane = S.n_lanes++;
        else lane = (int)(std::min_element(lane_tail.begin(), lane_tail.end()) - lane_tail.begin());
      }
    }
    S.lane[j] = lane;
    std::vector<int> latest(max_lanes, -1);
    for (int d : S.deps[j])
      if (S.lane[d] != lane && (latest[S.lane[d]] < 0 || pos[d] > pos[latest[S.lane[d]]])) latest[S.lane[d]] = d;
    for (int l = 0; l < max_lanes; ++l)
      if (latest[l] >= 0) { S.wait[j].push_back(latest[l]); S.signal[latest[l]] = 1; }
    lane_tail[lane] = j;
  }
  if (getenv("ACRMI_DEBUG_SCHED")) {
    std::vector<int> depth(n, 0);
    int edges = 0, maxd = 0;
    for (int j : S.order) {
      for (int d : S.deps[j]) depth[j] = std::max(depth[j], depth[d] + 1);
      edges += (int)S.deps[j].size();
      maxd = std::max(maxd, depth[j] + 1);
    }
    int waits = 0;
    for (int j : S.order) waits += (int)S.wait[j].size();
    fprintf(stderr, "[acrmi] schedule(%s, %s batches, %s): %zu ops, %d edges, critical path %d ops; %d lanes, %d cross-lane waits, "
                    "%d grouped launches\n",
            point ? "point" : "dense", large ? "large" : "small", planned ? "planned from measured op times" : "structural",
            S.order.size(), edges, maxd, S.n_lanes, waits, S.n_groups);
  }
}


extern "C" {

int acrmi_set_program(acrmi_ctx* c, const acrmi_buffer_desc* bufs, int n_bufs, const acrmi_op* ops, int n_ops,
                      const acrmi_head_layout* heads, int max_batch) {
  if (!c || !bufs || !ops || !heads || n_bufs <= 0 || n_ops <= 0 || max_batch <= 0)
    return fail(c, ACRMI_EINVAL, "acrmi_set_program: bad arguments");
  if (!c->weights) return fail(c, ACRMI_ESTATE, "acrmi_set_program: load weights first");
  ON_DEVICE(c);
  int prog_dt = ACRMI_DT_F32;
  for (int i = 0; i < n_bufs; ++i) {
    const auto& d = bufs[i];
    if (d.dtype < ACRMI_DT_F32 || d.dtype > ACRMI_DT_BF16) return fail(c, ACRMI_EINVAL, "buffer %d: unknown dtype %d", i, d.dtype);
    if (d.h <= 0 || d.w <= 0 || d.cs <= 0 || d.cs % (d.dtype ? 8 : 4)) return fail(c, ACRMI_EINVAL, "buffer %d: bad geometry", i);
    if (d.dtype) {
      if (prog_dt && prog_dt != d.dtype) return fail(c, ACRMI_EINVAL, "buffer %d: f16 and bf16 buffers in one program", i);
      prog_dt = d.dtype;
    }
  }
  auto bdt = [&](int id) { return id >= 0 ? bufs[id].dtype : (int)ACRMI_DT_F32; };
  auto buf_ok = [&](int id) { return id >= 0 && id < n_bufs; };
  auto w_ok = [&](long long off, long long n) { return off >= 0 && n >= 0 && (unsigned long long)(off + n) <= c->n_weights; };
  {
    const int hb[8] = {heads->center_buf[0], heads->center_buf[1], heads->params_buf[0], heads->params_buf[1],
                       heads->prior_buf[0], heads->prior_buf[1], heads->segm_buf, heads->backbone_buf};
    for (int id : hb)
      if (!buf_ok(id)) return fail(c, ACRMI_EINVAL, "head layout references buffer %d of %d", id, n_bufs);
    for (int k = 0; k < 7; ++k)
      if (bufs[hb[k]].dtype != ACRMI_DT_F32) return fail(c, ACRMI_EINVAL, "head layout: head maps must be fp32 buffers");
    if (bufs[heads->params_buf[0]].cs < 109 || bufs[heads->params_buf[1]].cs < 109 || bufs[heads->prior_buf[0]].cs < 106 ||
        bufs[heads->prior_buf[1]].cs < 106)
      return fail(c, ACRMI_EINVAL, "head layout: params/prior buffers are too narrow");
    for (int k = 0; k < 6; ++k)
      if (bufs[hb[k]].h != 64 || bufs[hb[k]].w != 64) return fail(c, ACRMI_EINVAL, "head layout: head maps must be 64x64");
  }
  for (int i = 0; i < n_ops; ++i) {
    const acrmi_op& op = ops[i];
    const int ids[4] = {op.in_buf, op.out_buf, op.res_buf, op.aux_buf};
    for (int id : ids)
      if (id >= n_bufs || id < -1) return fail(c, ACRMI_EINVAL, "op %d references buffer %d of %d", i, id, n_bufs);
    if (op.mode < ACRMI_MODE_BOTH || op.mode > ACRMI_MODE_POINT) return fail(c, ACRMI_EINVAL, "op %d: bad mode", i);
    bool need_in = false, need_out = true;
    switch (op.kind) {
      case ACRMI_OP_U8NORM: case ACRMI_OP_POW11: case ACRMI_OP_COORDFILL: case ACRMI_OP_STEM: break;
      case ACRMI_OP_CONV: case ACRMI_OP_BILINEAR2X: case ACRMI_OP_MAXPOOL: case ACRMI_OP_PAIR1X1: case ACRMI_OP_ATTPOOL: case ACRMI_OP_PAREBIAS: case ACRMI_OP_POINTHEADS:
        need_in = true;
        break;
      case ACRMI_OP_FUSESUM: break;
      default: return fail(c, ACRMI_EINVAL, "op %d: unknown kind %d", i, op.kind);
    }
    if ((need_in && !buf_ok(op.in_buf)) || (need_out && !buf_ok(op.out_buf)))
      return fail(c, ACRMI_EINVAL, "op %d (kind %d): missing input/output buffer", i, op.kind);
    if (op.in_coff < 0 || op.out_coff < 0 || op.res_coff < 0) return fail(c, ACRMI_EINVAL, "op %d: negative channel offset", i);
    if (op.kind == ACRMI_OP_CONV) {
      const int idt = bufs[op.in_buf].dtype, odt = bufs[op.out_buf].dtype;
      if (op.in_coff % (idt ? 8 : 4) || (op.ksize != 1 && op.ksize != 3) || op.stride < 1 || op.stride > 2 || op.cin <= 0 || op.cout <= 0 ||
          op.groups <= 0)
        return fail(c, ACRMI_EINVAL, "op %d: unsupported conv geometry", i);
      const int algo = op.flags & 7;
      if (algo > 7) return fail(c, ACRMI_EINVAL, "op %d: unknown conv algo %d", i, algo);
      if (idt ? (algo != 0 || (odt != idt && odt != ACRMI_DT_F32) || (odt == ACRMI_DT_F32 && op.stride != 1) ||
                 (op.groups > 1 && op.cin % 2))
              : odt != ACRMI_DT_F32)
        return fail(c, ACRMI_EINVAL, "op %d: conv buffer types do not fit (in %d, out %d, algo %d)", i, idt, odt, algo);
      if (op.res_buf >= 0 && bufs[op.res_buf].dtype != odt)
        return fail(c, ACRMI_EINVAL, "op %d: the residual must have the type of the output", i);
      const bool splitk = (op.flags & ACRMI_CONV_SPLITK) != 0;
      if (op.flags & ACRMI_CONV_BIAS_MAP) {
        const long long mcs = (op.groups * op.cout + 3) / 4 * 4;
        if (splitk || op.res_buf >= 0 || idt || algo == 3 || !w_ok(op.w_off2, (long long)bufs[op.out_buf].h * bufs[op.out_buf].w * mcs))
          return fail(c, ACRMI_EINVAL, "op %d: a position-bias map needs an fp32 conv without a residual buffer (not algo 3) and "
                      "[Ho][Wo][round4(groups*Cout)] floats inside the blob at w_off2", i);
      }
      const bool dual = (op.flags & ACRMI_CONV_DUAL) != 0;
      if (dual && (algo != 3 || op.nterms < 1 || op.bias_per_frame || !buf_ok(op.aux_buf) || bufs[op.aux_buf].dtype != ACRMI_DT_F32 ||
                   bufs[op.aux_buf].h != bufs[op.out_buf].h || bufs[op.aux_buf].w != bufs[op.out_buf].w || bufs[op.aux_buf].cs % 4 ||
                   bufs[op.aux_buf].cs < op.cout || op.aux_buf == op.out_buf || op.aux_buf == op.in_buf || op.aux_buf == op.res_buf))
        return fail(c, ACRMI_EINVAL, "op %d: a second output needs algo 3, 1..3 terms and an fp32 map of the output's size in aux_buf", i);
      if (op.nterms) {
        const int ho_ = bufs[op.out_buf].h, wo_ = bufs[op.out_buf].w;
        if (op.nterms < 0 || op.nterms > 3 || (op.flags & ACRMI_CONV_BIAS_MAP))
          return fail(c, ACRMI_EINVAL, "op %d: 1..3 extra residual terms, and no position-bias map beside them", i);
        for (int t = 0; t < op.nterms; ++t) {
          const int tb = op.term_buf[t];
          if (!buf_ok(tb) || bufs[tb].dtype != ACRMI_DT_F32 || op.term_coff[t] < 0 || op.term_coff[t] % 4 || bufs[tb].cs % 4 ||
              op.term_shift[t] < 0 || op.term_shift[t] > 3 || op.term_coff[t] + op.groups * op.cout > bufs[tb].cs ||
              (bufs[tb].h << op.term_shift[t]) != ho_ || (bufs[tb].w << op.term_shift[t]) != wo_ || tb == op.out_buf ||
              (dual && tb == op.aux_buf))
            return fail(c, ACRMI_EINVAL, "op %d: residual term %d does not fit the output", i, t);
        }
      }
      if (op.bias_per_frame && (!buf_ok(op.aux_buf) || bufs[op.aux_buf].dtype != ACRMI_DT_F32 || bufs[op.aux_buf].cs < op.groups * op.cout))
        return fail(c, ACRMI_EINVAL, "op %d: per-frame bias buffer missing, too narrow or not fp32", i);
      const int ogroups = splitk ? 1 : op.groups;
      if (op.in_coff + op.groups * op.cin > bufs[op.in_buf].cs || op.out_coff + ogroups * op.cout > bufs[op.out_buf].cs ||
          (op.res_buf >= 0 && op.res_coff + ogroups * op.cout > bufs[op.res_buf].cs) ||
          (op.groups > 1 && op.cin % (bufs[op.in_buf].dtype == ACRMI_DT_F32 ? 4 : 8)))
        return fail(c, ACRMI_EINVAL, "op %d: channel slice outside its buffer's channel stride", i);
      const int ho = conv_out_size(bufs[op.in_buf].h, op.ksize, op.stride), wo = conv_out_size(bufs[op.in_buf].w, op.ksize, op.stride);
      if (ho != bufs[op.out_buf].h || wo != bufs[op.out_buf].w ||
          (op.res_buf >= 0 && (bufs[op.res_buf].h != ho || bufs[op.res_buf].w != wo)))
        return fail(c, ACRMI_EINVAL, "op %d: output/residual buffer geometry does not match the convolution", i);
      ConvShape cs = conv_shape(conv_geometry(op, bufs, max_batch));
      cs.has_res = op.res_buf >= 0 || cs.res_bcast; cs.out2 = dual;
      if (const char* why = conv_algo_reject(algo, cs)) return fail(c, ACRMI_EINVAL, "op %d (algo %d): %s", i, algo, why);
      const long long wn = conv_weight_floats(algo, op.groups, op.ksize, op.cin, op.cout, idt);
      if (!w_ok(op.w_off, wn)) return fail(c, ACRMI_EINVAL, "op %d: packed weights outside the blob", i);
      if (!op.bias_per_frame && !w_ok(op.b_off, (long long)op.groups * conv_n_tiles(op.cout) * 32))
        return fail(c, ACRMI_EINVAL, "op %d: bias outside the blob", i);
    }
    if (op.kind == ACRMI_OP_STEM) {
      if (bufs[op.out_buf].dtype && (bufs[op.out_buf].cs % 8 || op.out_coff % 8))
        return fail(c, ACRMI_EINVAL, "op %d: a 16-bit stem output needs channel stride / offset in multiples of 8", i);
      if (op.ksize != 3 && op.ksize != 7) return fail(c, ACRMI_EINVAL, "op %d: the stem kernels are 3x3 and 7x7 (stride 2)", i);
      const bool ok = op.ksize == 7 ? stem7_shape_ok(2 * bufs[op.out_buf].h, 2 * bufs[op.out_buf].w, bufs[op.out_buf].cs, op.out_coff)
                                    : stem_shape_ok(2 * bufs[op.out_buf].h, 2 * bufs[op.out_buf].w, bufs[op.out_buf].cs, op.out_coff);
      if (op.cout != 64 || !ok)
        return fail(c, ACRMI_EINVAL, "op %d: the stem kernel needs 64 output channels and a map of 8x64-pixel strips", i);
      if (!w_ok(op.w_off, (op.ksize == 7 ? 74 : 14) * 2 * 64) || !w_ok(op.b_off, 64))
        return fail(c, ACRMI_EINVAL, "op %d: stem weights outside the blob", i);
    }
    if (op.kind == ACRMI_OP_FUSESUM) {
      const int vq = bufs[op.out_buf].dtype ? 8 : 4;
      if (op.nterms < 1 || op.nterms > 4 || op.cout <= 0 || op.cout % vq || op.out_coff % vq || op.out_coff + op.cout > bufs[op.out_buf].cs)
        return fail(c, ACRMI_EINVAL, "op %d: bad fuse-sum geometry", i);
      for (int t = 0; t < op.nterms; ++t) {
        if (!buf_ok(op.term_buf[t]) || op.term_coff[t] < 0 || bufs[op.term_buf[t]].dtype != bufs[op.out_buf].dtype ||
            op.term_coff[t] % vq || op.term_shift[t] < 0 || op.term_shift[t] > 3 ||
            op.term_coff[t] + op.cout > bufs[op.term_buf[t]].cs ||
            (bufs[op.term_buf[t]].h << op.term_shift[t]) != bufs[op.out_buf].h ||
            (bufs[op.term_buf[t]].w << op.term_shift[t]) != bufs[op.out_buf].w)
          return fail(c, ACRMI_EINVAL, "op %d: fuse-sum term %d does not fit the output", i, t);
      }
    }
    if (op.kind == ACRMI_OP_PAIR1X1) {
      if (!buf_ok(op.res_buf) || !buf_ok(op.aux_buf) || op.cin != 64 || op.cout != 256)
        return fail(c, ACRMI_EINVAL, "op %d: the 1x1 pair is 64 -> 256 (+ residual) -> 64 with in, res, out and aux buffers", i);
      const int ids4[4] = {op.in_buf, op.res_buf, op.out_buf, op.aux_buf};
      for (int id : ids4)
        if (bufs[id].dtype != ACRMI_DT_F32 || bufs[id].h != bufs[op.in_buf].h || bufs[id].w != bufs[op.in_buf].w)
          return fail(c, ACRMI_EINVAL, "op %d: the 1x1 pair's buffers must be fp32 maps of one size", i);
      if (op.in_coff % 4 || op.res_coff % 4 || op.out_coff % 4 || op.in_coff + 64 > bufs[op.in_buf].cs ||
          op.res_coff + 256 > bufs[op.res_buf].cs || op.out_coff + 256 > bufs[op.out_buf].cs || bufs[op.aux_buf].cs < 64 ||
          op.out_buf == op.in_buf || op.aux_buf == op.in_buf || op.aux_buf == op.out_buf || op.aux_buf == op.res_buf)
        return fail(c, ACRMI_EINVAL, "op %d: the 1x1 pair's channel slices do not fit / its buffers alias", i);
      if (!w_ok(op.w_off, PAIR1X1_FLOATS)) return fail(c, ACRMI_EINVAL, "op %d: pair weights outside the blob", i);
    }
    if (op.kind == ACRMI_OP_MAXPOOL) {
      const int vq = bufs[op.in_buf].dtype ? 8 : 4;
      if (op.cin <= 0 || bufs[op.in_buf].dtype != bufs[op.out_buf].dtype || op.cin % vq || op.in_coff % vq || op.out_coff % vq ||
          op.in_coff + op.cin > bufs[op.in_buf].cs || op.out_coff + op.cin > bufs[op.out_buf].cs ||
          bufs[op.out_buf].h != (bufs[op.in_buf].h - 1) / 2 + 1 || bufs[op.out_buf].w != (bufs[op.in_buf].w - 1) / 2 + 1)
        return fail(c, ACRMI_EINVAL, "op %d: bad max-pool geometry", i);
    }
    if (op.kind == ACRMI_OP_BILINEAR2X &&
        (op.cin <= 0 || bufs[op.in_buf].dtype != bufs[op.out_buf].dtype || op.cin % (bufs[op.in_buf].dtype ? 8 : 4) ||
         op.in_coff % (bufs[op.in_buf].dtype ? 8 : 4) || op.out_coff % (bufs[op.in_buf].dtype ? 8 : 4) || op.in_coff + op.cin > bufs[op.in_buf].cs ||
         op.out_coff + op.cin > bufs[op.out_buf].cs || bufs[op.out_buf].h != 2 * bufs[op.in_buf].h ||
         bufs[op.out_buf].w != 2 * bufs[op.in_buf].w))
      return fail(c, ACRMI_EINVAL, "op %d: bad bilinear geometry", i);
    if ((op.kind == ACRMI_OP_POW11 && op.out_coff >= bufs[op.out_buf].cs) ||
        (op.kind == ACRMI_OP_COORDFILL && op.out_coff + 2 > bufs[op.out_buf].cs))
      return fail(c, ACRMI_EINVAL, "op %d: channel outside the buffer", i);
    if (op.kind == ACRMI_OP_ATTPOOL) {
      if (buf_ok(op.res_buf) && (bufs[op.in_buf].dtype != ACRMI_DT_F32 || bufs[op.out_buf].dtype != ACRMI_DT_F32 ||
                                 (bufs[op.res_buf].dtype != ACRMI_DT_F32 && op.cin != 256)))
        return fail(c, ACRMI_EINVAL, "op %d: attention pooling reads fp32 logits, writes fp32, and pools 256 channels of a 16-bit map", i);
      if (!buf_ok(op.res_buf) || (op.cin != 32 && op.cin != 64 && op.cin != 256 && op.cin != 320) ||
          op.res_coff + op.cin > bufs[op.res_buf].cs || bufs[op.in_buf].cs < 33 || bufs[op.in_buf].h != 2 * bufs[op.res_buf].h ||
          bufs[op.in_buf].w != 2 * bufs[op.res_buf].w || (long long)bufs[op.out_buf].h * bufs[op.out_buf].w * bufs[op.out_buf].cs < 32LL * op.cin)
        return fail(c, ACRMI_EINVAL, "op %d: bad attention-pool geometry", i);
    }
    if ((op.kind == ACRMI_OP_PAREBIAS || op.kind == ACRMI_OP_POINTHEADS || op.kind == ACRMI_OP_U8NORM) &&
        (bdt(op.in_buf) || bdt(op.out_buf) || bdt(op.res_buf) || bdt(op.aux_buf)))
      return fail(c, ACRMI_EINVAL, "op %d (kind %d): fp32 buffers only", i, op.kind);
    if (op.kind == ACRMI_OP_PAREBIAS) {
      const long long shape_n = (op.cin == 320 ? 64 : 256) * 16;
      if ((op.cin != 256 && op.cin != 320) || (op.flags != 0 && op.flags != 16) || bufs[op.out_buf].cs < 109 || bufs[op.out_buf].cs > 256 ||
          (long long)bufs[op.in_buf].h * bufs[op.in_buf].w * bufs[op.in_buf].cs < 32LL * op.cin || !w_ok(op.w_off, 6 * 256 * 16) ||
          !w_ok(op.w_off2, 10 * shape_n) || !w_ok(op.b_off2, 10) || !w_ok(op.w_off3, 109 * 106) || !w_ok(op.b_off, 109))
        return fail(c, ACRMI_EINVAL, "op %d: bad pare-bias geometry or weights", i);
    }
    if (op.kind == ACRMI_OP_POINTHEADS) {
      const bool ok = buf_ok(op.res_buf) && buf_ok(op.aux_buf) &&
                      bufs[op.in_buf].h == 128 && bufs[op.in_buf].w == 128 && bufs[op.in_buf].cs == 36 &&
                      bufs[op.res_buf].h == 64 && bufs[op.out_buf].h == 64 && bufs[op.res_buf].cs >= 109 &&
                      bufs[op.out_buf].cs >= 109 && bufs[op.aux_buf].cs >= 109 && op.mode == ACRMI_MODE_POINT &&
                      w_ok(op.w_off, 3LL * TP_TOWER_FLOATS) && w_ok(op.w_off2, 109LL * TP_EXIT_N);
      if (!ok) return fail(c, ACRMI_EINVAL, "op %d: unsupported point-heads geometry", i);
    }
  }
  free_program(c);
  c->bufs.assign(bufs, bufs + n_bufs);
  c->ops.assign(ops, ops + n_ops);
  c->heads = *heads;
  c->max_batch = max_batch;
  c->grouping = g_grouping;
  c->buf_ptr.assign(n_bufs, nullptr);
  for (int i = 0; i < n_bufs; ++i) {
    const auto& d = bufs[i];
    const size_t bytes = (size_t)max_batch * d.h * d.w * d.cs * (d.dtype ? 2 : sizeof(float));
    hipError_t e = hipMalloc(&c->buf_ptr[i], bytes);
    if (e != hipSuccess) return fail(c, ACRMI_ENOMEM, "hipMalloc(%zu) for buffer %d: %s", bytes, i, hipGetErrorString(e));
    HIPCHK(c, hipMemset(c->buf_ptr[i], 0, bytes));
  }
  for (int i = 0; i < n_ops; ++i) {
    const acrmi_op& op = ops[i];
    if (op.kind != ACRMI_OP_CONV || !(op.flags & ACRMI_CONV_SPLITK)) continue;
    const auto& d = bufs[op.out_buf];
    c->split_ws_floats = std::max(c->split_ws_floats, conv_splitk_ws_floats(max_batch, d.h, d.w, op.cout, op.groups));
    c->split_counters = std::max(c->split_counters, conv_splitk_counters(max_batch, d.h, d.w, op.cout));
  }
  if (c->split_ws_floats)
    for (int l = 0; l < MAX_LANES; ++l) {
      HIPCHK(c, hipMalloc(&c->split_ws[l], c->split_ws_floats * sizeof(float)));
      HIPCHK(c, hipMalloc(&c->split_cnt[l], c->split_counters * sizeof(unsigned)));
      HIPCHK(c, hipMemset(c->split_cnt[l], 0, c->split_counters * sizeof(unsigned)));
    }
  c->att_ws_floats = attpool_ws_floats(max_batch, 320);
  HIPCHK(c, hipMalloc(&c->att_ws, c->att_ws_floats * sizeof(float)));
  HIPCHK(c, hipMalloc(&c->picks, (size_t)max_batch * POINT_PLAN_INTS * sizeof(int)));
  HIPCHK(c, hipMalloc(&c->gate_buf, (size_t)max_batch * sizeof(int)));
  for (int i = 0; i < n_ops; ++i)
    if (ops[i].kind == ACRMI_OP_CONV && (ops[i].flags & 7) == 6 && !c->range_flag) {
      HIPCHK(c, hipMalloc(&c->range_flag, sizeof(unsigned)));
      HIPCHK(c, hipMemset(c->range_flag, 0, sizeof(unsigned)));
    }
  c->op_ms[0].clear(); c->op_ms[1].clear();
  for (int v = 0; v < 4; ++v) build_schedule(c, v & 1, v & 2);
  c->op_ev.assign(n_ops, nullptr);
  c->have_program = true;
  for (const acrmi_op& op : c->ops)
    if (op.kind == ACRMI_OP_COORDFILL) {
      int r = run_op(c, op, nullptr, max_batch, nullptr);
      if (r) return r;
    }
  HIPCHK(c, hipDeviceSynchronize());
  return ACRMI_OK;
}

}

static unsigned lane_event_flags() {
  static const unsigned f = [] {
    const char* e = experiment_env("ACRMI_EVENT_FLAGS");
    if (e) fprintf(stderr, "[acrmi] WARNING: ACRMI_EVENT_FLAGS=%s - lane events created with non-default flags (experiment)\n", e);
    return hipEventDisableTiming | (e ? (unsigned)strtoul(e, nullptr, 16) : 0u);
  }();
  return f;
}

static int run_program_lanes(acrmi_ctx* c, const uint8_t* img, int B, hipStream_t user, bool point, int point_hands) {
  const Schedule& S = c->sched[point ? 1 : 0][B > AUTO_SMALL_BATCH ? 1 : 0];
  for (int l = 1; l < S.n_lanes; ++l) {
    if (!c->lanes[l]) HIPCHK(c, hipStreamCreateWithFlags(&c->lanes[l], hipStreamNonBlocking));
    if (!c->join_ev[l]) HIPCHK(c, hipEventCreateWithFlags(&c->join_ev[l], lane_event_flags()));
  }
  auto st = [&](int l) { return l == 0 ? user : c->lanes[l]; };
  if (S.n_lanes > 1) {
    if (!c->fork_ev) HIPCHK(c, hipEventCreateWithFlags(&c->fork_ev, lane_event_flags()));
    HIPCHK(c, hipEventRecord(c->fork_ev, user));
  }
  for (int l = 1; l < S.n_lanes; ++l) HIPCHK(c, hipStreamWaitEvent(c->lanes[l], c->fork_ev, 0));
  int r = ACRMI_OK;
  const int n_order = (int)S.order.size();
  for (int k = 0; k < n_order; ++k) {
    const int j = S.order[k];
    if (S.leader[j] != j) continue;
    hipStream_t s = st(S.lane[j]);
    static const int ablate = [] {
      const char* e = experiment_env("ACRMI_ABLATE_LANE_SYNC");
      const int v = e ? atoi(e) : 0;
      if (v) fprintf(stderr, "[acrmi] WARNING: ACRMI_ABLATE_LANE_SYNC=%d - cross-lane synchronisation is DISABLED, results are WRONG "
                             "(timing experiment only)\n", v);
      return v;
    }();
    int members[CONV_GROUP_MAX] = {j}, nm = 1;
    while (nm < CONV_GROUP_MAX && k + nm < n_order && S.leader[S.order[k + nm]] == j && S.order[k + nm] != j) { members[nm] = S.order[k + nm]; ++nm; }
    if (!(ablate & 1))
      for (int m = 0; m < nm; ++m)
        for (int d : S.wait[members[m]]) HIPCHK(c, hipStreamWaitEvent(s, c->op_ev[d], 0));
    if (nm > 1) {
      ConvArgs ga[CONV_GROUP_MAX];
      bool same = true;
      for (int m = 0; m < nm; ++m) {
        ga[m] = conv_args(c, c->ops[members[m]], B, S.lane[j]);
        same = same && conv_can_group(ga[0], ga[m]);
      }
      hipError_t e = hipSuccess;
      if (same) {
        e = launch_conv_group(ga, nm, s);
      } else {
        for (int m = 0; m < nm && e == hipSuccess; ++m) e = launch_conv(ga[m], s);
      }
      if (e != hipSuccess) {
        r = fail(c, ACRMI_EHIP, "grouped conv launch: %s", hipGetErrorString(e));
        break;
      }
    } else {
      r = run_op(c, c->ops[j], img, B, s, S.lane[j], point_hands);
      if (r) break;
    }
    for (int m = 0; m < nm; ++m) {
      const int jm = members[m];
      if (S.signal[jm] && !(ablate & 2)) {
        if (!c->op_ev[jm]) HIPCHK(c, hipEventCreateWithFlags(&c->op_ev[jm], lane_event_flags()));
        HIPCHK(c, hipEventRecord(c->op_ev[jm], s));
      }
    }
  }
  for (int l = 1; l < S.n_lanes; ++l) {
    HIPCHK(c, hipEventRecord(c->join_ev[l], c->lanes[l]));
    HIPCHK(c, hipStreamWaitEvent(user, c->join_ev[l], 0));
  }
  return r;
}

int run_program(acrmi_ctx* c, const uint8_t* img, int B, void* stream, bool point, int first_op, int point_hands) {
  if (!c || (!img && first_op <= 0)) return fail(c, ACRMI_EINVAL, "acrmi_backbone_heads: bad arguments");
  if (!c->have_program) return fail(c, ACRMI_ESTATE, "acrmi_backbone_heads: no program");
  if (B <= 0 || B > c->max_batch) return fail(c, ACRMI_EINVAL, "batch %d outside 1..%d", B, c->max_batch);
  ON_DEVICE(c);
  c->last_batch = B;
  static const bool dbg_sync = getenv("ACRMI_DEBUG_SYNC") != nullptr;
  const Schedule& S = c->sched[point ? 1 : 0][B > AUTO_SMALL_BATCH ? 1 : 0];
  if ((S.n_lanes > 1 || S.n_groups > 0) && !dbg_sync && first_op <= 0)
    return run_program_lanes(c, img, B, (hipStream_t)stream, point, point_hands);
  int i = 0;
  for (const acrmi_op& op : c->ops) {
    ++i;
    if (!op_active(op, point) || i - 1 < first_op) continue;
    if (dbg_sync) fprintf(stderr, "[acrmi] op %d kind %d B %d\n", i - 1, (int)op.kind, B), fflush(stderr);
    int r = run_op(c, op, img, B, (hipStream_t)stream, 0, point_hands);
    if (r) return r;
    if (dbg_sync) HIPCHK(c, hipStreamSynchronize((hipStream_t)stream));
  }
  return ACRMI_OK;
}
```

arbitrary-hands-3d-reconstruction_amd/csrc/kernels.h:

```cpp
#pragma once
#include <hip/hip_runtime.h>
#include <stdint.h>
#include <mutex>

#include <stdlib.h>

#include "conv_rules.h"
#include "nv12_out_plan.h"
#include "smooth_plan.h"
#include "assoc_plan.h"
#include "point_plan.h"

namespace acrmi {

inline const char* experiment_env(const char* name) {
#ifdef ACRMI_EXPERIMENTS
  return getenv(name);
#else
  (void)name;
  return nullptr;
#endif
}

struct ConvArgs {
  const float* in;
  const float* w;
  const float* bias;
  const float* res;
  float* out;
  int B, H, W, Ho, Wo;
  int in_cs, in_coff, Cin;
  int out_cs, out_coff, Cout;
  int res_cs, res_coff;
  int ks, stride, relu, groups;
  int n_tiles;
  int cin8;
  int bias_fstride;
  int algo;
  long long* dbg;
  int phase_delay;
  int xcd_swizzle;
  const float* zeros;
  int dtype;
  int out_f32;
  int res_bcast;
  int in_sub;
  int splitk;
  float* split_ws;
  unsigned* split_cnt;
  int nxt;
  const float* xt[3];
  int xt_cs[3], xt_coff[3], xt_shift[3];
  float* out2;
  int out2_cs, out2_coff;
  unsigned* range_flag;
};
inline void conv_derive(ConvArgs& a) {
  a.Ho = conv_out_size(a.H, a.ks, a.stride);
  a.Wo = conv_out_size(a.W, a.ks, a.stride);
  a.cin8 = conv_ksteps(a.Cin, a.dtype);
  a.n_tiles = conv_n_tiles(a.Cout);
}
inline size_t conv_splitk_groups(int B, int Ho, int Wo, int cout) {
  return (size_t)B * ((Ho + 7) / 8) * ((Wo + 15) / 16) * conv_n_tiles(cout);
}
inline size_t conv_splitk_ws_floats(int B, int Ho, int Wo, int cout, int splits) { return conv_splitk_groups(B, Ho, Wo, cout) * splits * 4096; }
inline size_t conv_splitk_counters(int B, int Ho, int Wo, int cout) { return conv_splitk_groups(B, Ho, Wo, cout) * 4; }

constexpr int MAX_DEVICES = 64;
bool first_use_on_device(unsigned char* flags);
std::recursive_mutex& launch_mutex();

hipError_t launch_conv(ConvArgs a, hipStream_t s);
hipError_t launch_conv_h16(ConvArgs a, hipStream_t s);
bool conv_can_group(const ConvArgs& a, const ConvArgs& b);
hipError_t launch_conv_group(const ConvArgs* a, int n, hipStream_t s);
const char* conv_kernel_name(const ConvArgs& a);
void conv_force_cfg(int cfg);
void conv_set_debug(long long* dbg);
void conv_set_phase_delay(int cycles);
void conv_set_xcd_swizzle(int on);

hipError_t launch_u8norm(const uint8_t* img, long n_pixels, float* out, hipStream_t s);
bool stem_shape_ok(int H, int W, int out_cs, int out_coff);
hipError_t launch_stem(const uint8_t* img, int B, int H, int W, const float* wpk, const float* bias, float* out,
                       int out_cs, int out_coff, int relu, hipStream_t s);
hipError_t launch_pair1x1(const float* t2, int t2_cs, int t2_coff, const float* x, int x_cs, int x_coff, float* y, int y_cs,
                          int y_coff, float* t, int t_cs, int t_coff, const float* wpk, long npix, hipStream_t s);
constexpr long PAIR1X1_FLOATS = 256 * 64 + 64 * 256 + 256 + 64;
bool stem7_shape_ok(int H, int W, int out_cs, int out_coff);
hipError_t launch_stem7(const uint8_t* img, int B, int H, int W, const float* wpk, const float* bias, float* out,
                        int out_cs, int out_coff, int relu, hipStream_t s);
hipError_t launch_stem7_h16(const uint8_t* img, int B, int H, int W, const float* wpk, const float* bias, void* out,
                            int out_cs, int out_coff, int relu, int dtype, hipStream_t s);
hipError_t launch_stem_h16(const uint8_t* img, int B, int H, int W, const float* wpk, const float* bias, void* out,
                           int out_cs, int out_coff, int relu, int dtype, hipStream_t s);
hipError_t launch_bilinear2x(const float* in, int B, int H, int W, int in_cs, int in_coff, int C, float* out,
                             int out_cs, int out_coff, hipStream_t s);
struct FuseArgs {
  const float* term[4];
  int cs[4], shift[4];
  int nterms, B, H, W, C, out_cs, relu;
  float* out;
};
hipError_t launch_fuse_sum(const FuseArgs& a, hipStream_t s);
__device__ inline void cv_cubic_taps(int d, double scale, int& s0, int (&c)[4]) {
  float f = (float)(((double)d + 0.5) * scale - 0.5);
  const float fl = floorf(f);
  s0 = (int)fl;
  f -= fl;
  const float A = -0.75f;
  float k[4];
  k[0] = ((A * (f + 1.f) - 5.f * A) * (f + 1.f) + 8.f * A) * (f + 1.f) - 4.f * A;
  k[1] = ((A + 2.f) * f - (A + 3.f)) * f * f + 1.f;
  k[2] = ((A + 2.f) * (1.f - f) - (A + 3.f)) * (1.f - f) * (1.f - f) + 1.f;
  k[3] = 1.f - k[0] - k[1] - k[2];
#pragma unroll
  for (int i = 0; i < 4; ++i) {
    int v = (int)rintf(k[i] * 2048.f);
    c[i] = v < -32768 ? -32768 : (v > 32767 ? 32767 : v);
  }
}
hipError_t launch_preprocess(const uint8_t* bgr, int n, int H, int W, int out_size, uint8_t* out, hipStream_t s);
constexpr int NV12_FRAMES_PER_LAUNCH = 64;
struct Nv12Coef {
  int cy, cub, cug, cvg, cvr, y_off;
};
struct Nv12DstFrame {
  const uint8_t* y;
  const uint8_t* uv;
  uint8_t* dst;
  int H, W, y_pitch, uv_pitch;
};
struct Nv12DstBatch {
  Nv12DstFrame f[NV12_FRAMES_PER_LAUNCH];
};
static_assert(sizeof(Nv12DstBatch) + sizeof(Nv12Coef) + 8 <= 4096, "NV12 kernel arguments must fit the 4 KB argument block");
hipError_t launch_nv12_to_rgb(const Nv12DstBatch& pb, const Nv12Coef& k, int n, int bgr, hipStream_t s);
__device__ inline int nv12_clamp8(int v) { return v < 0 ? 0 : (v > 255 ? 255 : v); }
__device__ inline void nv12_pixel(const Nv12Coef& k, int Y, int U, int V, int& R, int& G, int& B) {
  int yy = Y - k.y_off;
  yy = (yy < 0 ? 0 : yy) * k.cy;
  const int u = U - 128, v = V - 128, r = 1 << 19;
  R = nv12_clamp8((yy + k.cvr * v + r) >> 20);
  G = nv12_clamp8((yy + k.cug * u + k.cvg * v + r) >> 20);
  B = nv12_clamp8((yy + k.cub * u + r) >> 20);
}
struct Nv12OutFrame {
  const uint8_t* src;
  uint8_t* y;
  uint8_t* uv;
  int H, W, y_pitch, uv_pitch;
};
struct Nv12OutBatch {
  Nv12OutFrame f[NV12_FRAMES_PER_LAUNCH];
};
constexpr int NV12_COMPOSE_FRAMES_PER_LAUNCH = 58;
struct Nv12ComposeFrame {
  const uint8_t* src_y;
  const uint8_t* src_uv;
  const uint8_t* drawn;
  uint8_t* y;
  uint8_t* uv;
  int H, W, src_y_pitch, src_uv_pitch, y_pitch, uv_pitch;
};
struct Nv12ComposeBatch {
  Nv12ComposeFrame f[NV12_COMPOSE_FRAMES_PER_LAUNCH];
};
static_assert(sizeof(Nv12OutBatch) + sizeof(Nv12OutCoef) + 8 + 256 <= 4096 &&
                  sizeof(Nv12ComposeBatch) + sizeof(Nv12Coef) + sizeof(Nv12OutCoef) + 8 + 256 <= 4096,
              "NV12 output kernel arguments must fit the 4 KB argument block");
hipError_t launch_rgb_to_nv12(const Nv12OutBatch& pb, const Nv12OutCoef& k, int n, int bgr, hipStream_t s);
hipError_t launch_nv12_compose(const Nv12ComposeBatch& pb, const Nv12Coef& k6, const Nv12OutCoef& k10, int n, int bgr, hipStream_t s);
constexpr int ROIS_PER_LAUNCH = 64;
struct RoiBgr {
  const uint8_t* src;
  size_t pitch;
  int h, w;
};
struct RoiBgrBatch {
  RoiBgr r[ROIS_PER_LAUNCH];
};
struct RoiNv12 {
  const uint8_t* y;
  const uint8_t* uv;
  int y_pitch, uv_pitch;
  int l, t, h, w;
};
struct RoiNv12Batch {
  RoiNv12 r[ROIS_PER_LAUNCH];
};
static_assert(sizeof(RoiBgrBatch) + 24 <= 4096 && sizeof(RoiNv12Batch) + sizeof(Nv12Coef) + 24 <= 4096,
              "window kernel arguments must fit the 4 KB argument block");
hipError_t launch_preprocess_rois(const RoiBgrBatch& rb, int n, int out_size, uint8_t* out, hipStream_t s);
hipError_t launch_preprocess_rois_nv12(const RoiNv12Batch& rb, const Nv12Coef& k, int n, int out_size, uint8_t* out, hipStream_t s);
struct RoiBgrDev {
  const uint8_t* frame;
  int H, W;
  int box;
};
struct RoiBgrDevBatch {
  RoiBgrDev r[ROIS_PER_LAUNCH];
};
struct RoiNv12Dev {
  const uint8_t* y;
  const uint8_t* uv;
  int y_pitch, uv_pitch;
  int H, W;
  int box;
};
struct RoiNv12DevBatch {
  RoiNv12Dev r[ROIS_PER_LAUNCH];
};
static_assert(sizeof(RoiBgrDevBatch) + 48 <= 4096 && sizeof(RoiNv12DevBatch) + sizeof(Nv12Coef) + 48 <= 4096,
              "window kernel arguments must fit the 4 KB argument block");
hipError_t launch_preprocess_rois_dev(const RoiBgrDevBatch& rb, const int32_t* boxes, int n, int out_size, uint8_t* out,
                                      float* offsets, int32_t* status, hipStream_t s);
hipError_t launch_preprocess_rois_nv12_dev(const RoiNv12DevBatch& rb, const Nv12Coef& k, const int32_t* boxes, int n, int out_size,
                                           uint8_t* out, float* offsets, int32_t* status, hipStream_t s);
hipError_t launch_track_boxes(const float* pj2d_org, const float* slots, const int32_t* frame_hw, int n, int slot_floats,
                              int flag_at, double scale, int min_size, int32_t* boxes, hipStream_t s);
hipError_t launch_pow11(float* buf, long n_pixels, int cs, int ch, hipStream_t s);
hipError_t launch_nchw_to_nhwc(const float* in, int B, int C, int H, int W, float* out, int cs, int coff, hipStream_t s);
hipError_t launch_coordfill(float* buf, int B, int H, int W, int cs, int coff, hipStream_t s);
hipError_t launch_maxpool3s2(const float* in, int B, int H, int W, int in_cs, int in_coff, int C, float* out, int out_cs,
                             int out_coff, hipStream_t s);
hipError_t launch_maxpool3s2_h16(const void* in, int B, int H, int W, int in_cs, int in_coff, int C, void* out, int out_cs,
                                 int out_coff, int dtype, hipStream_t s);
hipError_t launch_bilinear2x_h16(const void* in, int B, int H, int W, int in_cs, int in_coff, int C, void* out, int out_cs,
                                 int out_coff, int dtype, hipStream_t s);
hipError_t launch_fuse_sum_h16(const FuseArgs& a, int dtype, hipStream_t s);
hipError_t launch_pow11_h16(void* buf, long n_pixels, int cs, int ch, int dtype, hipStream_t s);
hipError_t launch_coordfill_h16(void* buf, int B, int H, int W, int cs, int coff, int dtype, hipStream_t s);

hipError_t launch_attpool(const float* segm, int segm_cs, const float* feat, int feat_cs, int C, int B, int H, int W,
                          float* ws, float* pooled, hipStream_t s, int feat_dtype = 0);
size_t attpool_ws_floats(int B, int C);

struct PareArgs {
  const float* pooled;
  const float* lc_w;
// ... 326 lines not shown
```

arbitrary-hands-3d-reconstruction_amd/csrc/pair1x1.hip:

```cpp
#include "conv_frame.h"

namespace acrmi {

constexpr int PR_C1 = 64, PR_C2 = 256, PR_C3 = 64;
constexpr int PR_PIX = 256;
constexpr int PR_MT = 1, PR_WAVES = PR_PIX / (32 * PR_MT);
constexpr int PR_LDS_FLOATS = PR_C2 * PR_C1 + PR_C3 * PR_C2 + PR_C2 + PR_C3;

__global__ __launch_bounds__(PR_WAVES * 64, 1) void pair1x1_kernel(const float* __restrict__ t2, int t2_cs, int t2_coff,
                                                         const float* __restrict__ x, int x_cs, int x_coff,
                                                         float* __restrict__ y, int y_cs, int y_coff,
                                                         float* __restrict__ t, int t_cs, int t_coff,
                                                         const float* __restrict__ wpk, long npix) {
  extern __shared__ f32x4 smem4[];
  const f32x4* a1 = smem4;
  const f32x4* a2 = smem4 + PR_C2 * PR_C1 / 4;
  const f32x4* b3 = a2 + PR_C3 * PR_C2 / 4;
  const f32x4* b1 = b3 + PR_C2 / 4;
  const int tid = threadIdx.x, lane = tid & 63, wave = tid >> 6;
  const int li = lane & 31, lh = lane >> 5;
  for (int i = tid; i < PR_LDS_FLOATS / 4; i += PR_WAVES * 64) smem4[i] = reinterpret_cast<const f32x4*>(wpk)[i];

  const long items = (npix + PR_PIX - 1) / PR_PIX;
  auto pix_of = [&](long item, int p) -> long { return item * PR_PIX + 32 * PR_MT * wave + 32 * p + li; };
  f32x4 bq[PR_MT][8], bn[PR_MT][8];
  auto request_t2 = [&](long item, f32x4 (&dst)[PR_MT][8]) {
#pragma unroll
    for (int p = 0; p < PR_MT; ++p) {
      long px = pix_of(item, p);
      px = px < npix ? px : npix - 1;
      const f32x4* src = reinterpret_cast<const f32x4*>(t2 + (size_t)px * t2_cs + t2_coff + 32 * lh);
#pragma unroll
      for (int q = 0; q < 8; ++q) dst[p][q] = src[q];
    }
  };
  long item = blockIdx.x;
  if (item < items) request_t2(item, bq);
  __syncthreads();
  for (; item < items; item += gridDim.x) {
    const long nitem = item + gridDim.x;
    if (nitem < items) request_t2(nitem, bn);
    long px[PR_MT];
    bool ok[PR_MT];
#pragma unroll
    for (int p = 0; p < PR_MT; ++p) {
      px[p] = pix_of(item, p);
      ok[p] = px[p] < npix;
      px[p] = ok[p] ? px[p] : npix - 1;
    }
    f32x16 acc2[PR_MT][2];
    const f32x16 zero = {0.f, 0.f, 0.f, 0.f, 0.f, 0.f, 0.f, 0.f, 0.f, 0.f, 0.f, 0.f, 0.f, 0.f, 0.f, 0.f};
#pragma unroll 1
    for (int c = 0; c < 8; ++c) {
      f32x4 rv[PR_MT][4];
#pragma unroll
      for (int p = 0; p < PR_MT; ++p) {
        const float* xr = x + (size_t)px[p] * x_cs + x_coff + 32 * c + 4 * lh;
#pragma unroll
        for (int g = 0; g < 4; ++g) rv[p][g] = *reinterpret_cast<const f32x4*>(xr + 8 * g);
      }
      f32x16 acc1[PR_MT];
#pragma unroll
      for (int s4 = 0; s4 < 8; ++s4) {
        const f32x4 af = a1[(c * 8 + s4) * 64 + lane];
#pragma unroll
        for (int e = 0; e < 4; ++e)
#pragma unroll
          for (int p = 0; p < PR_MT; ++p) {
            if (s4 == 0 && e == 0) acc1[p] = __builtin_amdgcn_mfma_f32_32x32x2f32(af[e], bq[p][s4][e], zero, 0, 0, 0);
            else acc1[p] = __builtin_amdgcn_mfma_f32_32x32x2f32(af[e], bq[p][s4][e], acc1[p], 0, 0, 0);
          }
      }
      f32x4 yv[PR_MT][4];
#pragma unroll
      for (int g = 0; g < 4; ++g) {
        const f32x4 bv = b3[(c * 4 + g) * 2 + lh];
#pragma unroll
        for (int p = 0; p < PR_MT; ++p) {
          f32x4 o = f32x4{acc1[p][4 * g], acc1[p][4 * g + 1], acc1[p][4 * g + 2], acc1[p][4 * g + 3]} + bv + rv[p][g];
          o[0] = fmaxf(o[0], 0.f); o[1] = fmaxf(o[1], 0.f); o[2] = fmaxf(o[2], 0.f); o[3] = fmaxf(o[3], 0.f);
          yv[p][g] = o;
          if (ok[p])
            *reinterpret_cast<f32x4*>(y + (size_t)px[p] * y_cs + y_coff + 32 * c + 8 * g + 4 * lh) = o;
        }
      }
#pragma unroll
      for (int nt = 0; nt < 2; ++nt)
#pragma unroll
        for (int g = 0; g < 4; ++g) {
          const f32x4 af = a2[((c * 2 + nt) * 4 + g) * 64 + lane];
#pragma unroll
          for (int e = 0; e < 4; ++e)
#pragma unroll
            for (int p = 0; p < PR_MT; ++p) {
              if (c == 0 && g == 0 && e == 0) acc2[p][nt] = __builtin_amdgcn_mfma_f32_32x32x2f32(af[e], yv[p][g][e], zero, 0, 0, 0);
              else acc2[p][nt] = __builtin_amdgcn_mfma_f32_32x32x2f32(af[e], yv[p][g][e], acc2[p][nt], 0, 0, 0);
            }
        }
    }
#pragma unroll
    for (int nt = 0; nt < 2; ++nt)
#pragma unroll
      for (int g = 0; g < 4; ++g) {
        const f32x4 bv = b1[(nt * 4 + g) * 2 + lh];
#pragma unroll
        for (int p = 0; p < PR_MT; ++p) {
          f32x4 o = f32x4{acc2[p][nt][4 * g], acc2[p][nt][4 * g + 1], acc2[p][nt][4 * g + 2], acc2[p][nt][4 * g + 3]} + bv;
          o[0] = fmaxf(o[0], 0.f); o[1] = fmaxf(o[1], 0.f); o[2] = fmaxf(o[2], 0.f); o[3] = fmaxf(o[3], 0.f);
          if (ok[p])
            *reinterpret_cast<f32x4*>(t + (size_t)px[p] * t_cs + t_coff + 32 * nt + 8 * g + 4 * lh) = o;
        }
      }
#pragma unroll
    for (int p = 0; p < PR_MT; ++p)
#pragma unroll
      for (int q = 0; q < 8; ++q) bq[p][q] = bn[p][q];
  }
}

hipError_t launch_pair1x1(const float* t2, int t2_cs, int t2_coff, const float* x, int x_cs, int x_coff, float* y, int y_cs,
                          int y_coff, float* t, int t_cs, int t_coff, const float* wpk, long npix, hipStream_t s) {
  if (!t2 || !x || !y || !t || !wpk || npix <= 0 || t2_cs % 4 || x_cs % 4 || y_cs % 4 || t_cs % 4 || t2_coff % 4 || x_coff % 4 ||
      y_coff % 4 || t_coff % 4)
    return hipErrorInvalidValue;
  constexpr size_t lds = (size_t)PR_LDS_FLOATS * sizeof(float);
  static_assert(lds <= 160 * 1024, "both weight matrices must fit the LDS");
  std::lock_guard<std::recursive_mutex> lock(launch_mutex());
  static unsigned char init[MAX_DEVICES] = {};
  if (first_use_on_device(init)) {
    hipError_t e = hipFuncSetAttribute(reinterpret_cast<const void*>(pair1x1_kernel), hipFuncAttributeMaxDynamicSharedMemorySize, (int)lds);
    if (e != hipSuccess) return e;
    if ((e = conv_ensure_device_info()) != hipSuccess) return e;
  }
  const long items = (npix + PR_PIX - 1) / PR_PIX;
  const long cus = conv_num_cus();
  const unsigned grid = (unsigned)(items < cus ? items : cus);
  hipLaunchKernelGGL(pair1x1_kernel, dim3(grid), dim3(PR_WAVES * 64), lds, s, t2, t2_cs, t2_coff, x, x_cs, x_coff, y, y_cs, y_coff, t, t_cs,
                     t_coff, wpk, npix);
  return hipGetLastError();
}

}
```

arbitrary-hands-3d-reconstruction_amd/packer.py:

```python
import numpy as np

from . import _lib
from .schema import RESNET50, RESNET50_LAYERS, RESNET50_UP, backbone_channels, stage_cfg, state_dict_schema, width_of

EPS = 1e-5
WINOGRAD = True
WINOGRAD_2D = True


def _np(t):
    if hasattr(t, 'detach'):
        t = t.detach().cpu().numpy()
    return np.asarray(t)


def strip_prefix(sd, prefix='module.'):
    for k in ('model_state_dict', 'state_dict'):
        if k in sd and isinstance(sd[k], dict):
            sd = sd[k]
    out = {}
    for k, v in sd.items():
        out[k[len(prefix):] if k.startswith(prefix) else k] = v
    return out

# ... 416 lines not shown
            wb_list, cin = [(w0[:, s * ks:(s + 1) * ks], b0) for s in range(slices)], ks
        if out is None:
            out = self.buf(ho, wo, (out_c or (cout if slices > 1 else cout * len(wb_list))))
        if self.dt != DT_F32:
            assert self.dtype_of(src) == self.dt, 'conv input must be a 16-bit buffer in a 16-bit program'
            assert res is None or self.dtype_of(res) == self.dtype_of(out)
            algo = 0
            packed = [pack_conv_h16(w, b, self.dt) for (w, b) in wb_list]
            w_off = self.blob.add16(np.concatenate([p[0] for p in packed]))
        else:
            algo = 2 if slices > 1 else conv_algo(k, stride, cin, cout, len(wb_list), ho, wo, bias_buf is not None, self.wino24,
                                                    False if ((terms or fp32_kernel) and stride == 2) else self.split16, even)
            if algo in (6, 7):
                packed = [pack_conv_x3(wb_list, DT_BF16 if algo == 7 else DT_F16)]
            elif algo == 3:
                packed = [pack_wino3(w, b) for (w, b) in wb_list]
            else:
                tr = (lambda t: t, winograd_weights, winograd2d_weights, None, winograd24_weights, polyphase2_weights)[algo]
                packed = [pack_conv(tr(w), b) for (w, b) in wb_list]
            w_off = self.blob.add(np.concatenate([p[0] for p in packed]))
        b_off = self.blob.add(np.concatenate([p[1] for p in packed]))
        flops = 2.0 * ho * wo * flop_cout * cin_w * k * k * (1 if slices > 1 else len(wb_list))
        self._op(name, flops, kind=_lib.OP_CONV, in_buf=src, out_buf=out, res_buf=-1 if res is None else res,
                 in_coff=in_coff, out_coff=out_coff, res_coff=res_coff, cin=cin, cout=cout, ksize=k, stride=stride,
                 relu=int(relu), groups=len(wb_list), w_off=w_off, b_off=b_off, flags=algo,
                 bias_per_frame=0 if bias_buf is None else 1, aux_buf=-1 if bias_buf is None else bias_buf)
        if slices > 1:
            self.ops[-1].flags = algo | _lib.CONV_SPLITK
        if dual:
            out2, terms = dual
            assert algo == 3 and bias_buf is None and self.dims(out2)[:2] == (ho, wo) and out2 != out
            self.ops[-1].flags = algo | _lib.CONV_DUAL
            self.ops[-1].aux_buf = out2
        if terms:
            assert len(terms) <= 3 and self.dt == DT_F32 and len(wb_list) == 1
            assert dual or (k == 3 and stride == 2 and algo in (0, 5))
            op = self.ops[-1]
            op.nterms = len(terms)
            for t, (tb, sh) in enumerate(terms):
                th, tw, tcs = self.dims(tb)
                assert (th << sh, tw << sh) == (ho, wo) and tcs >= cout and tb != out
                op.term_buf[t], op.term_coff[t], op.term_shift[t] = tb, 0, sh
        if bias_map is not None:
            assert res is None and self.dt == DT_F32 and algo != 3
            assert bias_map.shape == (ho, wo, (cout * len(wb_list) + 3) // 4 * 4), bias_map.shape
            self.ops[-1].flags = algo | _lib.CONV_BIAS_MAP
            self.ops[-1].w_off2 = self.blob.add(bias_map)
        self.op_info[-1]['algo'] = ('direct', 'winograd_f23x', 'winograd_f2x2_3x3', 'winograd_f2x2_3x3_lds',
                                    'winograd_f2x4_3x3', 'polyphase_f2x2_s2', 'split_f16x3', 'split_bf16x3')[algo] + ('_splitk%d' % slices if slices > 1 else '')
        ng = len(wb_list)
        esz = lambda b: 4 if self.dtype_of(b) == DT_F32 else 2
        fam = ('conv_ws2_kernel', 'conv_wino_kernel', 'conv_wino2_kernel', 'conv_wino3_kernel', 'conv_wino24_kernel',
               'conv_pp2_kernel', 'conv_x3_kernel', 'conv_x3_kernel')[algo]
        if algo == 4 and wino24b_width(cin, cout, ho, wo):
            fam = 'conv_wino24b_kernel'
        if algo in (6, 7) and k == 1:
            fam = 'conv_x3p_kernel'
        if algo in (6, 7) and stride == 2:
            fam = 'conv_x3s2_kernel'
        if (algo == 0 and k == 1 and stride == 1 and cin % 32 == 0 and cout % 32 == 0 and (ho * wo) % 256 == 0 and
                (WINOGRAD_24 if self.wino24 is None else self.wino24) and
                (ho * wo // 256) * 64 * ng * ((cout // 32) // (2 if cout % 64 == 0 else 1)) >= 512):
            fam = 'conv_p1_kernel'
        if self.dt != DT_F32:
            fam = 'conv_h16_kernel'
        self.op_info[-1]['kernel'] = fam
        self.op_info[-1]['bytes'] = float(h * w_ * cin * ng * esz(src) + ho * wo * (cout if slices > 1 else cout * ng) * esz(out) *
                                          (2 if res is not None else 1) +
                                          sum((ho >> sh) * (wo >> sh) * cout * 4 for (_, sh) in (terms or [])) +
                                          (ho * wo * cout * 4 if dual else 0))
        if self.keep_weights:
            self.op_info[-1]['wb'] = [(np.asarray(w, np.float64), np.asarray(b, np.float64)) for (w, b) in wb_list]
        return out

    def cp(self, c):
        return self.chan_pad.get(c, c)

    def fuse_epilogue_ok(self, cin, cout):
        return FUSE_EPILOGUE and self.dt == DT_F32 and cin > 16 and cin % 8 == 0 and cout % 32 == 0

    def conv_bn(self, src, conv, bn, k, stride, relu, padded=False, **kw):
        w, b = self.folded(conv, bn)
        if padded and (self.cp(w.shape[0]) != w.shape[0] or self.cp(w.shape[1]) != w.shape[1]):
            co, ci = w.shape[:2]
            wp = np.zeros((self.cp(co), self.cp(ci)) + w.shape[2:])
            wp[:co, :ci] = w
            bp = np.zeros(self.cp(co))
            bp[:co] = b
            out = self.conv(conv, src, [(wp, bp)], k, stride, relu, **kw)
            self.op_info[-1]['flops'] *= float(co * ci) / float(wp.shape[0] * wp.shape[1])
            return out
        return self.conv(conv, src, [(w, b)], k, stride, relu, **kw)

    def fuse_sum(self, name, terms, c, relu, out=None, out_coff=0):
        h, w_, _ = self.dims(terms[0][0])
        assert terms[0][1] == 0
        if out is None:
            out = self.buf(h, w_, c)
        op = self._op(name, 0.0, kind=_lib.OP_FUSESUM, out_buf=out, out_coff=out_coff, cout=c, relu=int(relu),
                      nterms=len(terms))
        for t, (b, sh) in enumerate(terms):
            op.term_buf[t], op.term_coff[t], op.term_shift[t] = b, 0, sh
        return out

    def basic_block(self, x, p, dual=None):
        t = self.conv_bn(x, p + '.conv1', p + '.bn1', 3, 1, True, padded=True)
        kw = dict(dual=dual) if dual else {}
        y = self.conv_bn(t, p + '.conv2', p + '.bn2', 3, 1, True, res=x, padded=True, **kw)
        self.release(t, x)
        return y

    def fuse0_ok(self, c, h, w):
        return (FUSE_EPILOGUE and FUSE_FULLRES and self.dt == DT_F32 and not self.splitk and
                conv_algo(3, 1, self.cp(c), self.cp(c), 1, h, w, False, self.wino24, self.split16) == 3)

    def bottleneck(self, x, p, cat=None, stride=1):
        cin = self.sd[p + '.conv1.weight'].shape[1]
        t1 = self.conv_bn(x, p + '.conv1', p + '.bn1', 1, 1, True, cin=cin)
        if cat is not None:
            assert cat == x and stride == 1 and (p + '.downsample.0.weight') in self.sd
            mid = self.sd[p + '.conv2.weight'].shape[0]
            assert mid == cin and self.dims(cat)[2] >= 2 * cin
            self.conv_bn(t1, p + '.conv2', p + '.bn2', 3, 1, True, out=cat, out_coff=cin)
            self.release(t1)
            (wd, bd), (w3, b3) = self.folded(p + '.downsample.0', p + '.downsample.1'), self.folded(p + '.conv3', p + '.bn3')
            y = self.conv(p + '.conv3+downsample', cat, [(np.concatenate([wd, w3], 1), bd + b3)], 1, 1, True)
            self.release(cat)
            return y
        t2 = self.conv_bn(t1, p + '.conv2', p + '.bn2', 3, stride, True)
        self.release(t1)
        if (p + '.downsample.0.weight') in self.sd:
            res = self.conv_bn(x, p + '.downsample.0', p + '.downsample.1', 1, stride, False)
            self.release(x)
        else:
            res = x
        y = self.conv_bn(t2, p + '.conv3', p + '.bn3', 1, 1, True, res=res)
        self.release(t2, res)
        return y

    def bottleneck_chain(self, x, prefix, n, cat=None):
        shapes_ok = all(self.sd['%s.%d.conv3.weight' % (prefix, i)].shape[:2] == (256, 64) and
                        self.sd['%s.%d.conv1.weight' % (prefix, i)].shape[0] == 64 for i in range(n))
        if not (self.pairs and shapes_ok and n >= 2):
            for i in range(n):
                x = self.bottleneck(x, '%s.%d' % (prefix, i), cat=cat if i == 0 else None)
            return x
        t1 = None
        for i in range(n):
            p = '%s.%d' % (prefix, i)
            if t1 is None:
                t1 = self.conv_bn(x, p + '.conv1', p + '.bn1', 1, 1, True, cin=self.sd[p + '.conv1.weight'].shape[1])
            t2 = self.conv_bn(t1, p + '.conv2', p + '.bn2', 3, 1, True)
            self.release(t1)
            if (p + '.downsample.0.weight') in self.sd:
                res = self.conv_bn(x, p + '.downsample.0', p + '.downsample.1', 1, 1, False,
                                   cin=self.sd[p + '.downsample.0.weight'].shape[1])
                self.release(x)
            else:
                res = x
            if i == n - 1:
                y = self.conv_bn(t2, p + '.conv3', p + '.bn3', 1, 1, True, res=res)
                self.release(t2, res)
                return y
            q = '%s.%d' % (prefix, i + 1)
            (w3, b3), (w1, b1) = self.folded(p + '.conv3', p + '.bn3'), self.folded(q + '.conv1', q + '.bn1')
            h, w_, _ = self.dims(t2)
            y, t1 = self.buf(h, w_, 256), self.buf(h, w_, 64)
            self._op(p + '.conv3+' + q + '.conv1', 2.0 * h * w_ * (256 * 64 + 64 * 256), kind=_lib.OP_PAIR1X1, in_buf=t2, res_buf=res,
                     out_buf=y, aux_buf=t1, cin=64, cout=256, ksize=1, stride=1, relu=1, groups=1,
                     w_off=self.blob.add(pack_pair1x1(w3[:, :, 0, 0], b3, w1[:, :, 0, 0], b1)))
            self.op_info[-1]['algo'] = 'pair1x1'
            if self.keep_weights:
                self.op_info[-1]['wb'] = [(np.asarray(w3, np.float64), np.asarray(b3, np.float64)),
                                          (np.asarray(w1, np.float64), np.asarray(b1, np.float64))]
            self.release(t2, res)
            x = y

    def hr_module(self, xs, p, ch, multi_scale=True, final_out=None):
        nb = len(xs)
        xs = list(xs)
        h0, w0, _ = self.dims(xs[0])
        fold0 = nb > 1 and self.fuse0_ok(ch[0], h0, w0)
        for i in range(nb):
            for k in range(3 if (i == 0 and fold0) else 4):
                xs[i] = self.basic_block(xs[i], '%s.branches.%d.%d' % (p, i, k))
        outs = []
        temps = []

        def term(i, j, hosted=None):
            f = '%s.fuse_layers.%d.%d' % (p, i, j)
            if j == i:
                return xs[j], 0
            if j > i:
                t = self.conv_bn(xs[j], f + '.0', f + '.1', 1, 1, False, padded=True)
                temps.append(t)
                return t, j - i
            t = xs[j]
            for k in range(i - j):
                last = k == i - j - 1
                kw = dict(terms=hosted) if (last and hosted) else {}
                if last and j == 0:
                    kw['fp32_kernel'] = True
                t2 = self.conv_bn(t, '%s.%d.0' % (f, k), '%s.%d.1' % (f, k), 3, 2, (not last) or bool(hosted), padded=True, **kw)
                if t is not xs[j]:
                    self.release(t)
                t = t2
            if not hosted:
                temps.append(t)
            return t, 0

        for i in range(nb if multi_scale else 1):
            f0 = '%s.fuse_layers.%d.0' % (p, i)
            if i == 0 and fold0:
                others = [term(0, j) for j in range(1, nb)]
                y0 = final_out if final_out is not None else self.buf(h0, w0, self.cp(ch[0]))
                xs[0] = self.basic_block(xs[0], '%s.branches.0.3' % p, dual=(y0, others))
                self.op_info[-1]['name'] += '+fuse0'
                outs.append(y0)
                continue
            if i >= 1 and final_out is None:
                wl = self.sd['%s.%d.0.weight' % (f0, i - 1)]
                if self.fuse_epilogue_ok(self.cp(wl.shape[1]), self.cp(wl.shape[0])):
                    others = [term(i, j) for j in range(1, nb)]
                    y, _ = term(i, 0, hosted=others)
                    self.op_info[-1]['name'] += '+fuse%d' % i
                    outs.append(y)
                    continue
            terms = [term(i, j) for j in range(nb)]
            if terms[0][1] != 0:
                raise AssertionError('term 0 must be at output resolution')
            if final_out is not None:
                outs.append(self.fuse_sum(p + '.fuse%d' % i, terms, ch[i], True, out=final_out))
            else:
                outs.append(self.fuse_sum(p + '.fuse%d' % i, terms, self.cp(ch[i]), True))
        self.release(*temps)
        self.release(*xs)
        return outs


def point_tower(P, side, k):
    def rows(w, cpad):
        co, ci = w.shape[:2]
        wp = np.zeros((co, cpad, 3, 3))
        wp[:, :ci] = w
        return wp.reshape(co, cpad // 4, 4, 9).transpose(3, 1, 0, 2).reshape(-1)
    pre = '%s_final_layers.%d' % (side, k)
    w, b = P.folded(pre + '.0.0', pre + '.0.1')
    parts = [rows(w, 36), b]
    for blk in range(2):
        for c in (1, 2):
            w, b = P.folded(pre + '.1.%d.0.conv%d' % (blk, c), pre + '.1.%d.0.bn%d' % (blk, c))
            parts += [rows(w, 64), b]
    w, b = P.folded(pre + '.2')
    we = np.zeros((64, 112))
    we[:, :w.shape[0]] = w[:, :, 0, 0].T
    be = np.zeros(112)
    be[:w.shape[0]] = b
    out = np.concatenate([np.asarray(x, np.float64).reshape(-1) for x in parts + [we, be]])
    assert out.size == 9 * 9 * 64 * 4 + 64 + 4 * (9 * 16 * 64 * 4 + 64) + 64 * 112 + 112
    return out


def lower(sd, check=True, point_heads=True, keep_taps=False, precision='fp32', keep_weights=False, keep_all=False,
          wino24=None, splitk=False, pairs=None):
    sd = strip_prefix(sd)
    if check:
        check_state_dict(sd)
    if precision not in PRECISIONS:
        raise ValueError('precision %r: one of %s' % (precision, sorted(PRECISIONS)))
    width = width_of({k: _np(v) for k, v in sd.items() if k in ('backbone.transition1.0.0.weight', 'backbone.layer4.0.conv1.weight')})
    STAGE_CFG = None if width == RESNET50 else stage_cfg(width)
    c0 = backbone_channels(width)
    dt = PRECISIONS[precision]
    point_heads = point_heads and dt == DT_F32 and width == 32
    P = Program(sd, dt, keep_weights, keep_all, wino24, splitk, FUSE_PAIRS and not splitk if pairs is None else pairs,
                split16={'fp16x3': 'fp16', 'bf16x3': 'bf16'}.get(precision, False))
    b = 'backbone.'
    taps = {}
    x34 = None
    if width == RESNET50:
        w, bb = P.folded(b + 'conv1', b + 'bn1')
        x = P.buf(256, 256, 64)
        wp, bp = pack_stem7(w, bb)
        P._op(b + 'conv1', 2.0 * 256 * 256 * 64 * 3 * 49, kind=_lib.OP_STEM, out_buf=x, cin=3, cout=64, ksize=7, stride=2,
              relu=1, groups=1, w_off=P.blob.add(wp), b_off=P.blob.add(bp))
        P.op_info[-1]['algo'] = 'stem7_u8'
        if keep_weights:
            P.op_info[-1]['wb'] = [(np.asarray(w, np.float64), np.asarray(bb, np.float64))]
        if keep_taps:
            taps['stem'] = P.pin(x)
        cat = P.buf(128, 128, 128) if FUSE_PROJECTION else None
        pooled = cat if cat is not None else P.buf(128, 128, 64)
        P._op(b + 'maxpool', 0.0, kind=_lib.OP_MAXPOOL, in_buf=x, out_buf=pooled, cin=64)
        P.release(x)
        x = pooled
        for li, (planes, blocks, stride) in enumerate(RESNET50_LAYERS):
            for i in range(blocks):
                x = P.bottleneck(x, b + 'layer%d.%d' % (li + 1, i), cat=cat if (li == 0 and i == 0) else None,
                                 stride=stride if i == 0 else 1)
        if keep_taps:
            taps['layer4'] = P.pin(x)
        x34 = P.buf(128, 128, c0 + 2, persistent=True)
        P._op('coordfill', 0.0, kind=_lib.OP_COORDFILL, out_buf=x34, out_coff=c0)
        for k, c in enumerate(RESNET50_UP):
            h, w_, cs = P.dims(x)
            cin = P.sd[b + 'deconv_layers.%d.0.weight' % k].shape[1]
            up = P.buf(2 * h, 2 * w_, cin)
            P._op(b + 'deconv_layers.%d.bilinear2x' % k, 0.0, kind=_lib.OP_BILINEAR2X, in_buf=x, out_buf=up, cin=cin)
            P.release(x)
            x = P.conv_bn(up, b + 'deconv_layers.%d.0' % k, b + 'deconv_layers.%d.1' % k, 3, 1, True,
                          out=x34 if k == len(RESNET50_UP) - 1 else None)
            P.release(up)
    else:
        x34 = _lower_hrnet(P, sd, b, STAGE_CFG, c0, keep_taps, keep_weights, taps)
    return _lower_heads(P, sd, b, x34, c0, dt, point_heads, precision, width, taps)


def width_of_sd(sd):
    return width_of({k: v for k, v in sd.items() if k in ('backbone.transition1.0.0.weight', 'backbone.layer4.0.conv1.weight')})


def _lower_hrnet(P, sd, b, STAGE_CFG, c0, keep_taps, keep_weights, taps):
    w, bb = P.folded(b + 'conv1', b + 'bn1')
    if STEM_FUSED:
        x = P.buf(256, 256, 64)
        wp, bp = pack_stem(w, bb)
        P._op(b + 'conv1', 2.0 * 256 * 256 * 64 * 3 * 9, kind=_lib.OP_STEM, out_buf=x, cin=3, cout=64, ksize=3, stride=2,
              relu=1, groups=1, w_off=P.blob.add(wp), b_off=P.blob.add(bp))
# ... 171 lines not shown
```

include/acrmi.h:

```cpp
#ifndef ACRMI_H
#define ACRMI_H

#include <stddef.h>
#include <stdint.h>

#ifdef __cplusplus
extern "C" {
#endif

#define ACRMI_VERSION 303

#define ACRMI_OK 0
#define ACRMI_EINVAL (-1)
#define ACRMI_EHIP (-2)
#define ACRMI_ESTATE (-3)
#define ACRMI_ENOMEM (-4)
#define ACRMI_ERANGE (-5)

typedef struct acrmi_ctx acrmi_ctx;

enum { ACRMI_DT_F32 = 0, ACRMI_DT_F16 = 1, ACRMI_DT_BF16 = 2 };

typedef struct {
  int32_t h, w, cs;
// ... 228 lines not shown
#define ACRMI_OPT_SMOOTH_COEFF 6
int acrmi_set_option_f(acrmi_ctx* ctx, int option, float value);

int acrmi_smooth(acrmi_ctx* ctx, float* slots_dev, int B, void* stream);
int acrmi_smooth_reset(acrmi_ctx* ctx, void* stream);

typedef struct acrmi_streams acrmi_streams;
int acrmi_streams_create(acrmi_streams** out, int device, int capacity);
void acrmi_streams_destroy(acrmi_streams* t);
int acrmi_streams_reset(acrmi_streams* t, const int32_t* ids_host, int n, void* stream);
int acrmi_smooth_streams(acrmi_ctx* ctx, acrmi_streams* t, float* slots_dev, int B, const int32_t* ids_host, void* stream);
int acrmi_forward_streams(acrmi_ctx* ctx, acrmi_streams* t, const int32_t* ids_host, const uint8_t* img_dev, int B,
                          const float* offsets_dev, float* slots_dev, float* verts_dev, float* joints_dev,
                          float* verts_camed_dev, float* pj2d_dev, float* pj2d_org_dev, void* stream);

typedef struct acrmi_tracks acrmi_tracks;
int acrmi_tracks_create(acrmi_tracks** out, int device, int capacity, int max_hand, int gate, int max_miss);
void acrmi_tracks_destroy(acrmi_tracks* t);
int acrmi_tracks_reset(acrmi_tracks* t, const int32_t* ids_host, int n, void* stream);
int acrmi_associate(acrmi_ctx* ctx, acrmi_tracks* t, float* slots_dev, int B, int max_hand, const int32_t* ids_host, int smooth,
                    int32_t* track_ids_dev, int32_t* perm_dev, void* stream);
int acrmi_forward_tracks(acrmi_ctx* ctx, acrmi_tracks* t, const int32_t* ids_host, int smooth, const uint8_t* img_dev, int B,
                         int max_hand, const float* offsets_dev, float* slots_dev, float* verts_dev, float* joints_dev,
                         float* verts_camed_dev, float* pj2d_dev, float* pj2d_org_dev, int32_t* track_ids_dev, void* stream);
#define ACRMI_ASSOC_STATE 41
int acrmi_assoc_step(int max_hand, int gate, int max_miss, const float* rows_host, int row_stride, int32_t* state,
                     int32_t* track_ids, int32_t* perm, int32_t* born);

int acrmi_mesh_topology(const int32_t* faces_host, int n_faces, int n_verts, int32_t* blob_host, int n_ints);
size_t acrmi_render_workspace(int n_meshes, int n_faces);
int acrmi_rasterize(const float* verts_dev, const float* trans_dev, int n_meshes, int n_verts, int n_faces,
                    const int32_t* topo_dev, const int32_t* topo2_dev, const int32_t* mesh_topo_dev,
                    const int32_t* mesh_frame_dev, const float* rgb_dev, const float* view_dev, float focal,
                    float visible_weight, const uint8_t* img_in_dev, uint8_t* img_out_dev, int n_frames, int H, int W,
                    int32_t* ids_out_dev, void* ws_dev, void* stream);
int acrmi_load_faces(acrmi_ctx* ctx, int side, const int32_t* faces_host, int n_faces);
int acrmi_render(acrmi_ctx* ctx, const float* verts_dev, const float* cam_trans_dev, const float* slots_dev, int B,
                 const float* offsets_dev, const float* colors_host, float focal, float visible_weight,
                 const uint8_t* img_in_dev, uint8_t* img_out_dev, int H, int W, int32_t* ids_out_dev, void* stream);

size_t acrmi_contact_workspace(int n_meshes, int n_verts);
int acrmi_mesh_contact(const float* verts_dev, const float* trans_dev, int n_meshes, int n_verts, int n_faces,
                       const int32_t* topo_dev, const int32_t* topo2_dev, const int32_t* mesh_topo_dev, const int32_t* sign_dev,
                       const int32_t* pairs_dev, int n_pairs, float contact_dist, float max_depth, int32_t* nn_dev, float* d2_dev,
                       float* s_dev, float* sum_f_dev, int32_t* sum_i_dev, void* ws_dev, void* stream);
int acrmi_contact(acrmi_ctx* ctx, const float* verts_dev, const float* cam_trans_dev, const float* slots_dev, int B, int K,
                  const int32_t* sign_host, float contact_dist, float max_depth, int32_t* nn_dev, float* d2_dev, float* s_dev,
                  float* sum_f_dev, int32_t* sum_i_dev, void* stream);

size_t acrmi_surface_contact_workspace(int n_meshes, int n_verts, int n_faces);
int acrmi_mesh_surface_contact(const float* verts_dev, const float* trans_dev, int n_meshes, int n_verts, int n_faces,
                               const int32_t* topo_dev, const int32_t* topo2_dev, const int32_t* mesh_topo_dev,
                               const int32_t* pairs_dev, int n_pairs, float contact_dist, float max_depth, int32_t* face_dev,
                               float* d2_dev, float* point_dev, int32_t* cross_dev, float* sum_f_dev, int32_t* sum_i_dev,
                               void* ws_dev, void* stream);
int acrmi_surface_contact(acrmi_ctx* ctx, const float* verts_dev, const float* cam_trans_dev, const float* slots_dev, int B,
                          int K, float contact_dist, float max_depth, int32_t* face_dev, float* d2_dev, float* point_dev,
                          int32_t* cross_dev, float* sum_f_dev, int32_t* sum_i_dev, void* stream);

size_t acrmi_score_board_bytes(int n, int n_groups, int n_bins);
size_t acrmi_score_pair_bytes(int n_groups);
int acrmi_pose_errors(const float* pred_dev, const float* gt_dev, const uint8_t* valid_dev, int N, int n, int root,
                      const float* origin_pred_dev, const float* origin_gt_dev, const float* trans_dev, const int32_t* group_dev,
                      int n_groups, const float* flags_dev, float* e_ra_dev, float* e_pa_dev, float* row_f_dev, int32_t* row_i_dev,
                      float* xform_dev, float* pair_err_dev, void* stream);
int acrmi_score_accumulate(const float* e_ra_dev, const float* e_pa_dev, int N, int n, const int32_t* group_dev, int n_groups,
                           const float* flags_dev, const float* pair_err_dev, int n_bins, double bin_width, void* board_dev,
                           void* pair_board_dev, void* stream);
int acrmi_score_hands(acrmi_ctx* ctx, const float* joints_dev, const float* verts_dev, const float* slots_dev,
                      const float* cam_trans_dev, const float* gt_joints_dev, const float* gt_verts_dev,
                      const uint8_t* joint_valid_dev, const int32_t* group_dev, int B, int K, int n_groups, int n_bins,
                      double bin_width, void* board_dev, float* j_e_ra_dev, float* j_e_pa_dev, float* j_row_f_dev,
                      int32_t* j_row_i_dev, float* v_e_ra_dev, float* v_e_pa_dev, float* v_row_f_dev, int32_t* v_row_i_dev,
                      float* pair_err_dev, void* stream);

size_t acrmi_match_board_bytes(void);
int acrmi_match_hands(const float* pred_dev, const float* truth_dev, const uint8_t* valid_dev, const uint8_t* truth_valid_dev,
                      const float* flags_dev, int flag_stride, const float* trans_dev, const int32_t* group_dev, int B, int K, int G,
                      int n, int D, float gate, int min_points, int32_t* match_dev, int32_t* pred_of_dev, float* cost_dev,
                      int32_t* counts_dev, int32_t* group_out_dev, void* stream);
int acrmi_match_gather(const float* src_dev, const int32_t* index_dev, int B, int Ks, int Kd, int W, float* dst_dev, void* stream);
int acrmi_match_accumulate(const int32_t* counts_dev, const float* cost_dev, int B, int K, void* board_dev, void* stream);

#define ACRMI_OVERLAY_SKELETON 0
#define ACRMI_OVERLAY_CENTERMAP 1
int acrmi_overlay_tables(int bgr, uint8_t* colors_host, uint8_t* lut_host);
int acrmi_draw_skeletons(const float* kps_dev, const int32_t* hand_frame_dev, int n_hands, const uint8_t* colors_host, int bgr,
                         int line_width, int circle_rad, const uint8_t* img_in_dev, uint8_t* img_out_dev, int n_frames, int H,
                         int W, void* stream);
int acrmi_draw_heatmaps(const float* maps_l_dev, const float* maps_r_dev, long long frame_stride, int n, int h, int w,
                        const float* view_dev, float weight, const uint8_t* lut_host, int bgr, const uint8_t* img_in_dev,
                        uint8_t* out_l_dev, uint8_t* out_r_dev, int H, int W, void* stream);
int acrmi_overlay(acrmi_ctx* ctx, int what, const float* slots_dev, const float* pj2d_dev, int B, const float* offsets_dev,
                  int bgr, const uint8_t* img_in_dev, uint8_t* out_dev, uint8_t* out2_dev, int H, int W, void* stream);

int acrmi_rasterize_views(const float* verts_dev, const float* trans_dev, int n_meshes, int n_verts, int n_faces,
                          const int32_t* topo_dev, const int32_t* topo2_dev, const int32_t* mesh_topo_dev,
                          const int32_t* mesh_frame_dev, const float* rgb_dev, const float* view_dev, float focal,
                          float visible_weight, const uint8_t* img_in_dev, uint8_t* img_out_dev, int n_frames, int H, int W,
                          int32_t* ids_out_dev, void* ws_dev, void* stream);
int acrmi_draw_region_heatmaps(const float* maps_l_dev, const float* maps_r_dev, long long frame_stride, int n, int h, int w,
                               const float* offsets_dev, const int32_t* region_frame_dev, float weight,
                               const uint8_t* lut_host, int bgr, const uint8_t* img_in_dev, uint8_t* out_l_dev,
                               uint8_t* out_r_dev, int n_frames, int H, int W, void* stream);
int acrmi_render_regions(acrmi_ctx* ctx, const float* verts_dev, const float* cam_trans_dev, const float* slots_dev, int n,
                         const float* offsets_dev, const int32_t* region_frame_dev, const float* colors_host, float focal,
                         float visible_weight, const uint8_t* img_in_dev, uint8_t* img_out_dev, int n_frames, int H, int W,
                         int32_t* ids_out_dev, void* stream);
int acrmi_overlay_regions(acrmi_ctx* ctx, int what, const float* slots_dev, const float* pj2d_org_dev, int n,
                          const float* offsets_dev, const int32_t* region_frame_dev, int bgr, const uint8_t* img_in_dev,
                          uint8_t* out_dev, uint8_t* out2_dev, int n_frames, int H, int W, void* stream);

int acrmi_vertex_colors(const float* values_dev, const int32_t* flags_dev, const float* base_rgb_dev, int M, int V, float lo,
                        float hi, int reverse, const float* flag_rgb_host, const uint8_t* lut_host, int bgr, float* vcol_dev,
                        void* stream);
int acrmi_contact_values(const float* d2_dev, const float* s_dev, const int32_t* cross_dev, int B, int K, int V, float max_depth,
                         float* value_dev, int32_t* flag_dev, void* stream);
int acrmi_rasterize_colored(const float* verts_dev, const float* trans_dev, int n_meshes, int n_verts, int n_faces,
                            const int32_t* topo_dev, const int32_t* topo2_dev, const int32_t* mesh_topo_dev,
                            const int32_t* mesh_frame_dev, const float* rgb_dev, const float* vcol_dev, const float* view_dev,
                            int view_per_mesh, float focal, float visible_weight, const uint8_t* img_in_dev, uint8_t* img_out_dev,
                            int n_frames, int H, int W, int32_t* ids_out_dev, void* ws_dev, void* stream);
int acrmi_render_colored(acrmi_ctx* ctx, const float* verts_dev, const float* cam_trans_dev, const float* slots_dev, int B,
                         const float* offsets_dev, const float* colors_host, const float* vcol_dev, float focal,
                         float visible_weight, const uint8_t* img_in_dev, uint8_t* img_out_dev, int H, int W, int32_t* ids_out_dev,
                         void* stream);
int acrmi_render_regions_colored(acrmi_ctx* ctx, const float* verts_dev, const float* cam_trans_dev, const float* slots_dev, int n,
                                 const float* offsets_dev, const int32_t* region_frame_dev, const float* colors_host,
                                 const float* vcol_dev, float focal, float visible_weight, const uint8_t* img_in_dev,
                                 uint8_t* img_out_dev, int n_frames, int H, int W, int32_t* ids_out_dev, void* stream);

#define ACRMI_SEGM_NONE 255
int acrmi_segm_tables(int bgr, int C, uint8_t* colors_host);
int acrmi_segm_labels(const float* logits_dev, long long frame_stride, int pix_stride, int n, int h, int w, int C,
                      const float* view_dev, const float* offsets_dev, float weight, const uint8_t* colors_host, int bgr,
                      const uint8_t* img_in_dev, uint8_t* out_dev, uint8_t* labels_dev, int H, int W, void* stream);
size_t acrmi_segm_stats_ws_ints(int n, int H, int W);
int acrmi_segm_stats(const uint8_t* labels_dev, const int32_t* ids_dev, int n_faces, int n, int H, int W, int C,
                     int32_t* counts_dev, int32_t* boxes_dev, int32_t* agree_dev, int32_t* ws_dev, void* stream);
int acrmi_segment(acrmi_ctx* ctx, int B, const float* offsets_dev, float weight, const uint8_t* colors_host, int bgr,
                  const uint8_t* img_in_dev, uint8_t* out_dev, uint8_t* labels_dev, int H, int W, void* stream);

int acrmi_comm_unique_id(void* id128_out);
int acrmi_comm_init(acrmi_ctx* ctx, int n_ranks, int rank, const void* id128);
int acrmi_comm_destroy(acrmi_ctx* ctx);
int acrmi_allgather(acrmi_ctx* ctx, void* nccl_comm, const float* send_dev, float* recv_dev, size_t n_floats,
                    void* stream);

int acrmi_point_heads(acrmi_ctx* ctx, int B, void* stream);
int acrmi_point_heads_multi(acrmi_ctx* ctx, int B, int max_hand, void* stream);

int acrmi_profile_ops(acrmi_ctx* ctx, const uint8_t* img_dev, int B, float* ms_out, int n_ms, void* stream);
int acrmi_program_groups(acrmi_ctx* ctx, int B);

int acrmi_stream_create(int device, void** stream);
int acrmi_stream_destroy(void* stream);

int acrmi_tune(int key, int value);

#ifdef __cplusplus
}
#endif
#endif
```

Measured before the change: 2023 frames/s.

## Absorb bottleneck downsample projection conv into following pair1x1 kernel

Adds a schedule pass that finds a 1x1 64->256 downsample convolution whose output is used only as the residual of the next fused conv3+conv1 pair kernel. It drops that op and computes the projection inside the pair kernel with extra MFMAs, folding the downsample bias into the conv3 bias in LDS. This removes one kernel launch and the write and re-read of a 256-channel residual tensor, at the cost of more registers and MFMA work inside the pair kernel. The packer now keeps the downsample input alive until the pair has run. The pass is on by default for max_batch >= 16, and the program then runs through the lane scheduler.

```diff
diff --git a/arbitrary-hands-3d-reconstruction_amd/_lib.py b/arbitrary-hands-3d-reconstruction_amd/_lib.py
--- a/arbitrary-hands-3d-reconstruction_amd/_lib.py
+++ b/arbitrary-hands-3d-reconstruction_amd/_lib.py
@@ -92,7 +92,7 @@
            'acrmi_overlay_regions', 'acrmi_decode_multi', 'acrmi_decode_maps_multi', 'acrmi_forward_multi',
            'acrmi_tracks_create', 'acrmi_tracks_destroy', 'acrmi_tracks_reset', 'acrmi_associate', 'acrmi_forward_tracks',
            'acrmi_assoc_step', 'acrmi_point_heads_multi', 'acrmi_contact_workspace', 'acrmi_mesh_contact', 'acrmi_contact',
-           'acrmi_conv2d_group', 'acrmi_program_groups', 'acrmi_surface_contact_workspace', 'acrmi_mesh_surface_contact',
+           'acrmi_conv2d_group', 'acrmi_program_groups', 'acrmi_program_absorbed', 'acrmi_surface_contact_workspace', 'acrmi_mesh_surface_contact',
            'acrmi_surface_contact', 'acrmi_score_board_bytes', 'acrmi_score_pair_bytes', 'acrmi_pose_errors',
            'acrmi_score_accumulate', 'acrmi_score_hands', 'acrmi_vertex_colors', 'acrmi_contact_values',
            'acrmi_rasterize_colored', 'acrmi_render_colored', 'acrmi_render_regions_colored', 'acrmi_segm_tables',
@@ -186,6 +186,7 @@
     L.acrmi_tune.argtypes = [i32, i32]
     L.acrmi_conv2d_group.argtypes = [C.POINTER(ConvProblem), i32, vp]
     L.acrmi_program_groups.argtypes = [vp, i32]
+    L.acrmi_program_absorbed.argtypes = [vp, i32]
     L.acrmi_preprocess.argtypes = [u8p, i32, i32, i32, u8p, vp, vp]
     L.acrmi_cam_trans.argtypes = [f32p, f32p, i32, C.c_float, C.c_float, f32p, vp]
     L.acrmi_set_option.argtypes = [vp, i32, i32]
diff --git a/arbitrary-hands-3d-reconstruction_amd/csrc/absorb_plan.h b/arbitrary-hands-3d-reconstruction_amd/csrc/absorb_plan.h
--- /dev/null
+++ b/arbitrary-hands-3d-reconstruction_amd/csrc/absorb_plan.h
@@ -0,0 +1,95 @@
+#pragma once
+#include <cstddef>
+#include <vector>
+
+namespace acrmi {
+
+enum { ABSORB_OTHER = 0, ABSORB_CONV = 1, ABSORB_PAIR = 2 };
+
+struct AbsorbSlice {
+  int buf = -1, coff = 0, c = 0;
+};
+
+struct AbsorbOp {
+  int kind = ABSORB_OTHER;
+  bool proj_ok = false;
+  int in_buf = -1, in_coff = 0;
+  int out_buf = -1, out_coff = 0;
+  int res_buf = -1, res_coff = 0;
+  int aux_buf = -1;
+  int h = 0, w = 0;
+  std::vector<AbsorbSlice> reads, writes;
+};
+
+constexpr int ABSORB_COUT = 256;
+
+inline bool absorb_overlaps(const AbsorbSlice& s, int buf, int coff, int c) {
+  return s.buf == buf && (s.c <= 0 || (s.coff < coff + c && coff < s.coff + s.c));
+}
+inline bool absorb_covers(const AbsorbSlice& s, int buf, int coff, int c) {
+  return s.buf == buf && s.c > 0 && s.coff <= coff && coff + c <= s.coff + s.c;
+}
+
+inline std::vector<int> plan_absorb(const std::vector<AbsorbOp>& ops, const std::vector<int>& order, const std::vector<char>& keep) {
+  std::vector<int> by(ops.size(), -1);
+  auto touches = [](const AbsorbOp& o, int buf) {
+    for (const AbsorbSlice& s : o.reads) if (s.buf == buf) return true;
+    for (const AbsorbSlice& s : o.writes) if (s.buf == buf) return true;
+    return false;
+  };
+  auto writes_buf = [](const AbsorbOp& o, int buf) {
+    for (const AbsorbSlice& s : o.writes) if (s.buf == buf) return true;
+    return false;
+  };
+  for (std::size_t k = 0; k < order.size(); ++k) {
+    const AbsorbOp& D = ops[order[k]];
+    if (D.kind != ABSORB_CONV || !D.proj_ok || D.out_buf < 0 || D.in_buf < 0 || D.in_buf == D.out_buf) continue;
+    if (D.out_buf >= (int)keep.size() || keep[D.out_buf]) continue;
+    std::size_t q = k + 1;
+    bool x_intact = true;
+    for (; q < order.size() && !touches(ops[order[q]], D.out_buf); ++q) x_intact = x_intact && !writes_buf(ops[order[q]], D.in_buf);
+    if (q == order.size() || !x_intact) continue;
+    const AbsorbOp& P = ops[order[q]];
+    if (P.kind != ABSORB_PAIR || P.res_buf != D.out_buf || P.res_coff != D.out_coff || P.h != D.h || P.w != D.w) continue;
+    if (P.in_buf == D.out_buf || P.out_buf == D.out_buf || P.aux_buf == D.out_buf) continue;
+    if (P.out_buf == D.in_buf || P.aux_buf == D.in_buf || writes_buf(P, D.in_buf)) continue;
+    bool dead = false;
+    for (std::size_t r = q + 1; r < order.size() && !dead; ++r) {
+      const AbsorbOp& o = ops[order[r]];
+      bool reads = false, part = false, whole = false;
+      for (const AbsorbSlice& s : o.reads) reads = reads || s.buf == D.out_buf;
+      for (const AbsorbSlice& s : o.writes) {
+        if (absorb_covers(s, D.out_buf, D.out_coff, ABSORB_COUT)) whole = true;
+        else if (absorb_overlaps(s, D.out_buf, D.out_coff, ABSORB_COUT)) part = true;
+      }
+      if (reads || (part && !whole)) break;
+      dead = whole;
+    }
+    if (dead) by[order[k]] = order[q];
+  }
+  return by;
+}
+
+inline const char* check_absorb(const std::vector<AbsorbOp>& ops, const std::vector<int>& order, const std::vector<int>& by) {
+  std::vector<int> pos(ops.size(), -1), taken(ops.size(), 0);
+  for (std::size_t k = 0; k < order.size(); ++k) pos[order[k]] = (int)k;
+  for (std::size_t j = 0; j < ops.size(); ++j) {
+    const int p = by[j];
+    if (p < 0) continue;
+    if (pos[j] < 0 || p >= (int)ops.size() || pos[p] <= pos[j]) return "an absorbed op's pair does not follow it";
+    if (ops[j].kind != ABSORB_CONV || ops[p].kind != ABSORB_PAIR) return "an absorption is not a convolution into a pair";
+    if (ops[p].res_buf != ops[j].out_buf) return "the pair does not take the absorbed op's output as its residual";
+    if (++taken[p] > 1) return "a pair absorbs two ops";
+    for (int q = pos[j] + 1; q < (int)order.size(); ++q) {
+      if (q == pos[p]) continue;
+      for (const AbsorbSlice& s : ops[order[q]].reads)
+        if (s.buf == ops[j].out_buf) return "an op reads the output that is never written";
+      bool whole = false;
+      for (const AbsorbSlice& s : ops[order[q]].writes) whole = whole || absorb_covers(s, ops[j].out_buf, ops[j].out_coff, ABSORB_COUT);
+      if (whole) break;
+    }
+  }
+  return nullptr;
+}
+
+}
diff --git a/arbitrary-hands-3d-reconstruction_amd/csrc/acrmi.hip b/arbitrary-hands-3d-reconstruction_amd/csrc/acrmi.hip
--- a/arbitrary-hands-3d-reconstruction_amd/csrc/acrmi.hip
+++ b/arbitrary-hands-3d-reconstruction_amd/csrc/acrmi.hip
@@ -571,6 +571,13 @@
   return c->sched[c->point_heads ? 1 : 0][B > AUTO_SMALL_BATCH ? 1 : 0].n_groups;
 }
 
+int acrmi_program_absorbed(acrmi_ctx* c, int B) {
+  if (!c) return fail(c, ACRMI_EINVAL, "acrmi_program_absorbed: bad arguments");
+  if (!c->have_program) return fail(c, ACRMI_ESTATE, "no program");
+  if (B <= 0 || B > c->max_batch) return fail(c, ACRMI_EINVAL, "batch %d outside 1..%d", B, c->max_batch);
+  return c->sched[c->point_heads ? 1 : 0][B > AUTO_SMALL_BATCH ? 1 : 0].n_absorbed;
+}
+
 int acrmi_profile_ops(acrmi_ctx* c, const uint8_t* img, int B, float* ms_out, int n_ms, void* stream) {
   if (!c || !img || !ms_out) return fail(c, ACRMI_EINVAL, "acrmi_profile_ops: bad arguments");
   if (!c->have_program) return fail(c, ACRMI_ESTATE, "no program");
@@ -1195,6 +1202,7 @@
   if (key == 3) { conv_set_phase_delay(value); return ACRMI_OK; }
   if (key == 4) { conv_set_xcd_swizzle(value); return ACRMI_OK; }
   if (key == 5) { program_set_grouping(value != 0); return ACRMI_OK; }
+  if (key == 6) { program_set_absorbing(value); return ACRMI_OK; }
   static long long* dbg = nullptr;
   if (key == 1) {
     if (value && !dbg) { if (hipMalloc(&dbg, 128 * sizeof(long long)) != hipSuccess) return ACRMI_EHIP; }
diff --git a/arbitrary-hands-3d-reconstruction_amd/csrc/acrmi_ctx.h b/arbitrary-hands-3d-reconstruction_amd/csrc/acrmi_ctx.h
--- a/arbitrary-hands-3d-reconstruction_amd/csrc/acrmi_ctx.h
+++ b/arbitrary-hands-3d-reconstruction_amd/csrc/acrmi_ctx.h
@@ -30,6 +30,8 @@
   std::vector<char> signal;
   std::vector<int> leader;
   int n_groups = 0;
+  std::vector<int> absorbed_by, absorbs;
+  int n_absorbed = 0;
 };
 struct StateTable {
   int device = 0;
@@ -63,6 +65,7 @@
   bool have_program = false;
   int max_batch = 0;
   bool grouping = false;
+  bool absorbing = false;
   float* att_ws = nullptr;
   size_t att_ws_floats = 0;
   int* picks = nullptr;
@@ -146,6 +149,7 @@
 bool op_active(const acrmi_op& op, bool point);
 void build_schedule(acrmi_ctx* c, bool point, bool large);
 void program_set_grouping(bool on);
+void program_set_absorbing(int value);
 int run_program(acrmi_ctx* c, const uint8_t* img, int B, void* stream, bool point, int first_op = 0, int point_hands = 1);
 int decode_maps_impl(const float* l_center, const float* r_center, int center_cs, const float* l_params, const float* r_params,
                      int params_cs, const float* l_prior, const float* r_prior, int prior_cs, int B, float conf_thresh,
diff --git a/arbitrary-hands-3d-reconstruction_amd/csrc/acrmi_program.hip b/arbitrary-hands-3d-reconstruction_amd/csrc/acrmi_program.hip
--- a/arbitrary-hands-3d-reconstruction_amd/csrc/acrmi_program.hip
+++ b/arbitrary-hands-3d-reconstruction_amd/csrc/acrmi_program.hip
@@ -1,6 +1,7 @@
 #include "acrmi_ctx.h"
 #include "conv_frame.h"
 #include "group_plan.h"
+#include "absorb_plan.h"
 
 void free_program(acrmi_ctx* c) {
   for (hipEvent_t e : c->op_ev)
@@ -96,6 +97,22 @@
   return !(e && atoi(e) == 0);
 }();
 void program_set_grouping(bool on) { g_grouping = on; }
+
+constexpr bool ABSORB_DEFAULT = true;
+static bool absorb_start_value() {
+  const char* e = getenv("ACRMI_ABSORB");
+  return e ? atoi(e) != 0 : ABSORB_DEFAULT;
+}
+static bool g_absorbing = absorb_start_value();
+void program_set_absorbing(int value) { g_absorbing = value < 0 ? absorb_start_value() : value != 0; }
+
+static int run_pair_proj(acrmi_ctx* c, const acrmi_op& op, const acrmi_op& d, int B, hipStream_t s) {
+  const auto& di = c->bufs[op.in_buf];
+  HIPCHK(c, launch_pair1x1_proj(c->buf_ptr[op.in_buf], di.cs, op.in_coff, c->buf_ptr[d.in_buf], c->bufs[d.in_buf].cs, d.in_coff,
+                                c->weights + d.w_off, c->weights + d.b_off, c->buf_ptr[op.out_buf], c->bufs[op.out_buf].cs, op.out_coff,
+                                c->buf_ptr[op.aux_buf], c->bufs[op.aux_buf].cs, 0, c->weights + op.w_off, (long)B * di.h * di.w, s));
+  return ACRMI_OK;
+}
 
 int run_op(acrmi_ctx* c, const acrmi_op& op, const uint8_t* img, int B, hipStream_t s, int lane, int point_hands) {
   auto ptr = [&](int id) -> float* { return id >= 0 ? c->buf_ptr[id] : nullptr; };
@@ -248,6 +265,36 @@
   }
 }
 
+static AbsorbOp absorb_op(const acrmi_ctx* c, const acrmi_op& op) {
+  AbsorbOp a;
+  std::vector<int> R, W;
+  op_rw(c, op, R, W);
+  for (int b : R) a.reads.push_back(AbsorbSlice{b, 0, 0});
+  for (int b : W) a.writes.push_back(AbsorbSlice{b, 0, 0});
+  auto extent = [](std::vector<AbsorbSlice>& v, int buf, int coff, int ch) {
+    for (AbsorbSlice& s : v)
+      if (s.buf == buf && s.c == 0) { s.coff = coff; s.c = ch; return; }
+  };
+  a.in_buf = op.in_buf; a.in_coff = op.in_coff; a.out_buf = op.out_buf; a.out_coff = op.out_coff;
+  a.res_buf = op.res_buf; a.res_coff = op.res_coff; a.aux_buf = op.aux_buf;
+  if (op.out_buf >= 0) { a.h = c->bufs[op.out_buf].h; a.w = c->bufs[op.out_buf].w; }
+  if (op.kind == ACRMI_OP_CONV) {
+    a.kind = ABSORB_CONV;
+    const bool splitk = (op.flags & ACRMI_CONV_SPLITK) != 0;
+    extent(a.writes, op.out_buf, op.out_coff, (splitk ? 1 : op.groups) * op.cout);
+    a.proj_ok = op.ksize == 1 && op.stride == 1 && op.cin == 64 && op.cout == ABSORB_COUT && op.groups == 1 && !op.relu &&
+                op.res_buf < 0 && !op.bias_per_frame && !op.nterms && op.flags == 0 && c->bufs[op.in_buf].dtype == ACRMI_DT_F32 &&
+                c->bufs[op.out_buf].dtype == ACRMI_DT_F32 && op.w_off % 4 == 0 && op.b_off % 4 == 0;
+  } else if (op.kind == ACRMI_OP_PAIR1X1) {
+    a.kind = ABSORB_PAIR;
+    extent(a.writes, op.out_buf, op.out_coff, 256);
+    extent(a.writes, op.aux_buf, 0, 64);
+  } else if (op.kind == ACRMI_OP_FUSESUM) {
+    extent(a.writes, op.out_buf, op.out_coff, op.cout);
+  }
+  return a;
+}
+
 void build_schedule(acrmi_ctx* c, bool point, bool large) {
   Schedule& S = c->sched[point ? 1 : 0][large ? 1 : 0];
   const int n = (int)c->ops.size(), nb = (int)c->bufs.size() + 2;
@@ -259,6 +306,28 @@
     if (!op_active(c->ops[j], point)) continue;
     S.order.push_back(j);
     op_rw(c, c->ops[j], reads[j], writes[j]);
+  }
+  S.absorbed_by.assign(n, -1);
+  S.absorbs.assign(n, -1);
+  if (c->absorbing && c->max_batch >= 16) {
+    std::vector<AbsorbOp> ao(n);
+    std::vector<char> keep(c->bufs.size() + 2, 0);
+    for (size_t b = 0; b < c->bufs.size(); ++b) keep[b] = c->bufs[b].persistent != 0;
+    const int hb[8] = {c->heads.center_buf[0], c->heads.center_buf[1], c->heads.params_buf[0], c->heads.params_buf[1],
+                       c->heads.prior_buf[0], c->heads.prior_buf[1], c->heads.segm_buf, c->heads.backbone_buf};
+    for (int b : hb) keep[b] = 1;
+    for (int j : S.order) ao[j] = absorb_op(c, c->ops[j]);
+    S.absorbed_by = plan_absorb(ao, S.order, keep);
+    for (int d = 0; d < n; ++d) {
+      const int p = S.absorbed_by[d];
+      if (p < 0) continue;
+      S.absorbs[p] = d;
+      ++S.n_absorbed;
+      reads[d].clear(); writes[d].clear();
+      reads[p].erase(std::remove(reads[p].begin(), reads[p].end(), c->ops[p].res_buf), reads[p].end());
+      reads[p].push_back(c->ops[d].in_buf);
+      S.order.erase(std::remove(S.order.begin(), S.order.end(), d), S.order.end());
+    }
   }
   S.deps = hazard_deps(S.order, reads, writes, n, nb);
   for (int j : S.order)
@@ -555,6 +624,7 @@
   c->heads = *heads;
   c->max_batch = max_batch;
   c->grouping = g_grouping;
+  c->absorbing = g_absorbing;
   c->buf_ptr.assign(n_bufs, nullptr);
   for (int i = 0; i < n_bufs; ++i) {
     const auto& d = bufs[i];
@@ -657,7 +727,8 @@
         break;
       }
     } else {
-      r = run_op(c, c->ops[j], img, B, s, S.lane[j], point_hands);
+      r = S.absorbs[j] >= 0 ? run_pair_proj(c, c->ops[j], c->ops[S.absorbs[j]], B, s)
+                            : run_op(c, c->ops[j], img, B, s, S.lane[j], point_hands);
       if (r) break;
     }
     for (int m = 0; m < nm; ++m) {
@@ -683,7 +754,7 @@
   c->last_batch = B;
   static const bool dbg_sync = getenv("ACRMI_DEBUG_SYNC") != nullptr;
   const Schedule& S = c->sched[point ? 1 : 0][B > AUTO_SMALL_BATCH ? 1 : 0];
-  if ((S.n_lanes > 1 || S.n_groups > 0) && !dbg_sync && first_op <= 0)
+  if ((S.n_lanes > 1 || S.n_groups > 0 || S.n_absorbed > 0) && !dbg_sync && first_op <= 0)
     return run_program_lanes(c, img, B, (hipStream_t)stream, point, point_hands);
   int i = 0;
   for (const acrmi_op& op : c->ops) {
diff --git a/arbitrary-hands-3d-reconstruction_amd/csrc/kernels.h b/arbitrary-hands-3d-reconstruction_amd/csrc/kernels.h
--- a/arbitrary-hands-3d-reconstruction_amd/csrc/kernels.h
+++ b/arbitrary-hands-3d-reconstruction_amd/csrc/kernels.h
@@ -87,6 +87,9 @@
                        int out_cs, int out_coff, int relu, hipStream_t s);
 hipError_t launch_pair1x1(const float* t2, int t2_cs, int t2_coff, const float* x, int x_cs, int x_coff, float* y, int y_cs,
                           int y_coff, float* t, int t_cs, int t_coff, const float* wpk, long npix, hipStream_t s);
+hipError_t launch_pair1x1_proj(const float* t2, int t2_cs, int t2_coff, const float* x, int x_cs, int x_coff, const float* wd,
+                               const float* bd, float* y, int y_cs, int y_coff, float* t, int t_cs, int t_coff, const float* wpk,
+                               long npix, hipStream_t s);
 constexpr long PAIR1X1_FLOATS = 256 * 64 + 64 * 256 + 256 + 64;
 bool stem7_shape_ok(int H, int W, int out_cs, int out_coff);
 hipError_t launch_stem7(const uint8_t* img, int B, int H, int W, const float* wpk, const float* bias, float* out,
diff --git a/arbitrary-hands-3d-reconstruction_amd/csrc/pair1x1.hip b/arbitrary-hands-3d-reconstruction_amd/csrc/pair1x1.hip
--- a/arbitrary-hands-3d-reconstruction_amd/csrc/pair1x1.hip
+++ b/arbitrary-hands-3d-reconstruction_amd/csrc/pair1x1.hip
@@ -7,11 +7,13 @@
 constexpr int PR_MT = 1, PR_WAVES = PR_PIX / (32 * PR_MT);
 constexpr int PR_LDS_FLOATS = PR_C2 * PR_C1 + PR_C3 * PR_C2 + PR_C2 + PR_C3;
 
+template <bool PROJ>
 __global__ __launch_bounds__(PR_WAVES * 64, 1) void pair1x1_kernel(const float* __restrict__ t2, int t2_cs, int t2_coff,
                                                          const float* __restrict__ x, int x_cs, int x_coff,
                                                          float* __restrict__ y, int y_cs, int y_coff,
                                                          float* __restrict__ t, int t_cs, int t_coff,
-                                                         const float* __restrict__ wpk, long npix) {
+                                                         const float* __restrict__ wpk, const float* __restrict__ wd,
+                                                         const float* __restrict__ bd, long npix) {
   extern __shared__ f32x4 smem4[];
   const f32x4* a1 = smem4;
   const f32x4* a2 = smem4 + PR_C2 * PR_C1 / 4;
@@ -19,7 +21,12 @@
   const f32x4* b1 = b3 + PR_C2 / 4;
   const int tid = threadIdx.x, lane = tid & 63, wave = tid >> 6;
   const int li = lane & 31, lh = lane >> 5;
-  for (int i = tid; i < PR_LDS_FLOATS / 4; i += PR_WAVES * 64) smem4[i] = reinterpret_cast<const f32x4*>(wpk)[i];
+  constexpr int B3_AT = (PR_C2 * PR_C1 + PR_C3 * PR_C2) / 4;
+  for (int i = tid; i < PR_LDS_FLOATS / 4; i += PR_WAVES * 64) {
+    f32x4 v = reinterpret_cast<const f32x4*>(wpk)[i];
+    if (PROJ && i >= B3_AT && i < B3_AT + PR_C2 / 4) v += reinterpret_cast<const f32x4*>(bd)[i - B3_AT];
+    smem4[i] = v;
+  }
 
   const long items = (npix + PR_PIX - 1) / PR_PIX;
   auto pix_of = [&](long item, int p) -> long { return item * PR_PIX + 32 * PR_MT * wave + 32 * p + li; };
@@ -34,8 +41,15 @@
       for (int q = 0; q < 8; ++q) dst[p][q] = src[q];
     }
   };
+  f32x4 xq[PROJ ? PR_MT : 1][8], wq[8];
+  const f32x4* wd4 = reinterpret_cast<const f32x4*>(wd) + (size_t)(4 * lh) * (PR_C2 / 32) * 64 + li;
+  auto request_wd = [&](int c) {
+#pragma unroll
+    for (int q = 0; q < 8; ++q) wq[q] = wd4[((q >> 1) * (PR_C2 / 32) + c) * 64 + 32 * (q & 1)];
+  };
   long item = blockIdx.x;
   if (item < items) request_t2(item, bq);
+  if (PROJ && item < items) request_wd(0);
   __syncthreads();
   for (; item < items; item += gridDim.x) {
     const long nitem = item + gridDim.x;
@@ -48,16 +62,26 @@
       ok[p] = px[p] < npix;
       px[p] = ok[p] ? px[p] : npix - 1;
     }
+    if (PROJ) {
+#pragma unroll
+      for (int p = 0; p < PR_MT; ++p) {
+        const f32x4* src = reinterpret_cast<const f32x4*>(x + (size_t)px[p] * x_cs + x_coff + 32 * lh);
+#pragma unroll
+        for (int q = 0; q < 8; ++q) xq[p][q] = src[q];
+      }
+    }
     f32x16 acc2[PR_MT][2];
     const f32x16 zero = {0.f, 0.f, 0.f, 0.f, 0.f, 0.f, 0.f, 0.f, 0.f, 0.f, 0.f, 0.f, 0.f, 0.f, 0.f, 0.f};
 #pragma unroll 1
     for (int c = 0; c < 8; ++c) {
-      f32x4 rv[PR_MT][4];
+      f32x4 rv[PROJ ? 1 : PR_MT][4];
+      if (!PROJ) {
 #pragma unroll
-      for (int p = 0; p < PR_MT; ++p) {
-        const float* xr = x + (size_t)px[p] * x_cs + x_coff + 32 * c + 4 * lh;
+        for (int p = 0; p < PR_MT; ++p) {
+          const float* xr = x + (size_t)px[p] * x_cs + x_coff + 32 * c + 4 * lh;
 #pragma unroll
-        for (int g = 0; g < 4; ++g) rv[p][g] = *reinterpret_cast<const f32x4*>(xr + 8 * g);
+          for (int g = 0; g < 4; ++g) rv[p][g] = *reinterpret_cast<const f32x4*>(xr + 8 * g);
+        }
       }
       f32x16 acc1[PR_MT];
 #pragma unroll
@@ -71,13 +95,23 @@
             else acc1[p] = __builtin_amdgcn_mfma_f32_32x32x2f32(af[e], bq[p][s4][e], acc1[p], 0, 0, 0);
           }
       }
+      if (PROJ) {
+#pragma unroll
+        for (int q = 0; q < 8; ++q)
+#pragma unroll
+          for (int e = 0; e < 4; ++e)
+#pragma unroll
+            for (int p = 0; p < PR_MT; ++p) acc1[p] = __builtin_amdgcn_mfma_f32_32x32x2f32(wq[q][e], xq[p][q][e], acc1[p], 0, 0, 0);
+        request_wd((c + 1) & 7);
+      }
       f32x4 yv[PR_MT][4];
 #pragma unroll
       for (int g = 0; g < 4; ++g) {
         const f32x4 bv = b3[(c * 4 + g) * 2 + lh];
 #pragma unroll
         for (int p = 0; p < PR_MT; ++p) {
-          f32x4 o = f32x4{acc1[p][4 * g], acc1[p][4 * g + 1], acc1[p][4 * g + 2], acc1[p][4 * g + 3]} + bv + rv[p][g];
+          f32x4 o = f32x4{acc1[p][4 * g], acc1[p][4 * g + 1], acc1[p][4 * g + 2], acc1[p][4 * g + 3]} + bv;
+          if (!PROJ) o += rv[p][g];
           o[0] = fmaxf(o[0], 0.f); o[1] = fmaxf(o[1], 0.f); o[2] = fmaxf(o[2], 0.f); o[3] = fmaxf(o[3], 0.f);
           yv[p][g] = o;
           if (ok[p])
@@ -118,26 +152,43 @@
   }
 }
 
-hipError_t launch_pair1x1(const float* t2, int t2_cs, int t2_coff, const float* x, int x_cs, int x_coff, float* y, int y_cs,
-                          int y_coff, float* t, int t_cs, int t_coff, const float* wpk, long npix, hipStream_t s) {
+template <bool PROJ>
+static hipError_t launch_pair1x1_form(const float* t2, int t2_cs, int t2_coff, const float* x, int x_cs, int x_coff, float* y, int y_cs,
+                                      int y_coff, float* t, int t_cs, int t_coff, const float* wpk, const float* wd, const float* bd,
+                                      long npix, hipStream_t s) {
   if (!t2 || !x || !y || !t || !wpk || npix <= 0 || t2_cs % 4 || x_cs % 4 || y_cs % 4 || t_cs % 4 || t2_coff % 4 || x_coff % 4 ||
-      y_coff % 4 || t_coff % 4)
+      y_coff % 4 || t_coff % 4 || t2_coff < 0 || x_coff < 0 || y_coff < 0 || t_coff < 0)
     return hipErrorInvalidValue;
+  if (t2_coff + PR_C1 > t2_cs || x_coff + (PROJ ? PR_C1 : PR_C2) > x_cs || y_coff + PR_C2 > y_cs || t_coff + PR_C3 > t_cs)
+    return hipErrorInvalidValue;
+  if (PROJ && (!wd || !bd || (uintptr_t)wd % 16 || (uintptr_t)bd % 16 || x == y || x == t)) return hipErrorInvalidValue;
+  if ((uintptr_t)wpk % 16) return hipErrorInvalidValue;
   constexpr size_t lds = (size_t)PR_LDS_FLOATS * sizeof(float);
   static_assert(lds <= 160 * 1024, "both weight matrices must fit the LDS");
   std::lock_guard<std::recursive_mutex> lock(launch_mutex());
   static unsigned char init[MAX_DEVICES] = {};
   if (first_use_on_device(init)) {
-    hipError_t e = hipFuncSetAttribute(reinterpret_cast<const void*>(pair1x1_kernel), hipFuncAttributeMaxDynamicSharedMemorySize, (int)lds);
+    hipError_t e = hipFuncSetAttribute(reinterpret_cast<const void*>(pair1x1_kernel<PROJ>), hipFuncAttributeMaxDynamicSharedMemorySize, (int)lds);
     if (e != hipSuccess) return e;
     if ((e = conv_ensure_device_info()) != hipSuccess) return e;
   }
   const long items = (npix + PR_PIX - 1) / PR_PIX;
   const long cus = conv_num_cus();
   const unsigned grid = (unsigned)(items < cus ? items : cus);
-  hipLaunchKernelGGL(pair1x1_kernel, dim3(grid), dim3(PR_WAVES * 64), lds, s, t2, t2_cs, t2_coff, x, x_cs, x_coff, y, y_cs, y_coff, t, t_cs,
-                     t_coff, wpk, npix);
+  hipLaunchKernelGGL(pair1x1_kernel<PROJ>, dim3(grid), dim3(PR_WAVES * 64), lds, s, t2, t2_cs, t2_coff, x, x_cs, x_coff, y, y_cs, y_coff, t,
+                     t_cs, t_coff, wpk, wd, bd, npix);
   return hipGetLastError();
 }
 
+hipError_t launch_pair1x1(const float* t2, int t2_cs, int t2_coff, const float* x, int x_cs, int x_coff, float* y, int y_cs,
+                          int y_coff, float* t, int t_cs, int t_coff, const float* wpk, long npix, hipStream_t s) {
+  return launch_pair1x1_form<false>(t2, t2_cs, t2_coff, x, x_cs, x_coff, y, y_cs, y_coff, t, t_cs, t_coff, wpk, nullptr, nullptr, npix, s);
 }
+
+hipError_t launch_pair1x1_proj(const float* t2, int t2_cs, int t2_coff, const float* x, int x_cs, int x_coff, const float* wd,
+                               const float* bd, float* y, int y_cs, int y_coff, float* t, int t_cs, int t_coff, const float* wpk,
+                               long npix, hipStream_t s) {
+  return launch_pair1x1_form<true>(t2, t2_cs, t2_coff, x, x_cs, x_coff, y, y_cs, y_coff, t, t_cs, t_coff, wpk, wd, bd, npix, s);
+}
+
+}
diff --git a/arbitrary-hands-3d-reconstruction_amd/packer.py b/arbitrary-hands-3d-reconstruction_amd/packer.py
--- a/arbitrary-hands-3d-reconstruction_amd/packer.py
+++ b/arbitrary-hands-3d-reconstruction_amd/packer.py
@@ -592,15 +592,16 @@
                 t1 = self.conv_bn(x, p + '.conv1', p + '.bn1', 1, 1, True, cin=self.sd[p + '.conv1.weight'].shape[1])
             t2 = self.conv_bn(t1, p + '.conv2', p + '.bn2', 3, 1, True)
             self.release(t1)
+            held = ()
             if (p + '.downsample.0.weight') in self.sd:
                 res = self.conv_bn(x, p + '.downsample.0', p + '.downsample.1', 1, 1, False,
                                    cin=self.sd[p + '.downsample.0.weight'].shape[1])
-                self.release(x)
+                held = (x,)
             else:
                 res = x
             if i == n - 1:
                 y = self.conv_bn(t2, p + '.conv3', p + '.bn3', 1, 1, True, res=res)
-                self.release(t2, res)
+                self.release(t2, res, *held)
                 return y
             q = '%s.%d' % (prefix, i + 1)
             (w3, b3), (w1, b1) = self.folded(p + '.conv3', p + '.bn3'), self.folded(q + '.conv1', q + '.bn1')
@@ -613,7 +614,7 @@
             if self.keep_weights:
                 self.op_info[-1]['wb'] = [(np.asarray(w3, np.float64), np.asarray(b3, np.float64)),
                                           (np.asarray(w1, np.float64), np.asarray(b1, np.float64))]
-            self.release(t2, res)
+            self.release(t2, res, *held)
             x = y
 
     def hr_module(self, xs, p, ch, multi_scale=True, final_out=None):
diff --git a/include/acrmi.h b/include/acrmi.h
--- a/include/acrmi.h
+++ b/include/acrmi.h
@@ -404,6 +404,7 @@
 
 int acrmi_profile_ops(acrmi_ctx* ctx, const uint8_t* img_dev, int B, float* ms_out, int n_ms, void* stream);
 int acrmi_program_groups(acrmi_ctx* ctx, int B);
+int acrmi_program_absorbed(acrmi_ctx* ctx, int B);
 
 int acrmi_stream_create(int device, void** stream);
 int acrmi_stream_destroy(void* stream);
```

Measured after the change: 2042 frames/s (median of 6 runs). Within noise of the previous version (+0.9%).
